# the-byte-bender/GraphAudio

Hardware: AMD Instinct MI355X
Metric: rendered frames/sec @48kHz, 1024-voice convolver graph (higher is better)
Workload: dtype f32

## Files before the change

graphaudio_amd/_capi.py:

```python
from __future__ import annotations

import ctypes as C
import os

_HERE = os.path.dirname(os.path.abspath(__file__))
LIB_NAME = "libgraphaudio_hip.so"


class GraphAudioLibraryError(ImportError):
    """The native HIP library could not be loaded."""


class ArgumentException(ValueError):
    """System.ArgumentException (OfflineAudioContext.cs:32-51)."""


class ArgumentOutOfRangeException(ArgumentException):
    """System.ArgumentOutOfRangeException (AudioBuffer.cs:18, AudioNodeInput.cs:43)."""


class InvalidOperationException(RuntimeError):
    """System.InvalidOperationException (ConvolverNode.cs:45-49, Nodes/AudioNode.cs:157-160)."""


class ObjectDisposedException(InvalidOperationException):
    """System.ObjectDisposedException (AudioContextBase.cs:54)."""


class NotSupportedException(RuntimeError):
    """The graph uses a feature outside the accelerated path (GA_ERR_UNSUPPORTED)."""


class DeviceException(RuntimeError):
    """HIP runtime / device failure (GA_ERR_DEVICE, GA_ERR_OUT_OF_MEMORY, GA_ERR_NO_DEVICE)."""


_CODE_TO_EXC = {
    -1: ArgumentException,
    -2: ArgumentOutOfRangeException,
    -3: InvalidOperationException,
    -4: ObjectDisposedException,
    -5: InvalidOperationException,
    -6: NotSupportedException,
    -7: DeviceException,
    -8: DeviceException,
    -9: DeviceException,
}


class Stats(C.Structure):
    _fields_ = [
        ("blocks_rendered", C.c_int64),
        ("chunks", C.c_int64),
        ("segments", C.c_int64),
        ("kernel_launches", C.c_int64),
        ("device_ms_total", C.c_double),
        ("mac_launches", C.c_int64),
        ("mac_ms_total", C.c_double),
        ("mac_flops_total", C.c_double),
        ("mac_bytes_total", C.c_double),
        ("fft_ms_total", C.c_double),
        ("other_ms_total", C.c_double),
        ("device_bytes_in_use", C.c_int64),
        ("n_nodes", C.c_int32),
        ("n_conv_rows", C.c_int32),
        ("stage_ms", C.c_double * 16),
        ("stage_launches", C.c_int64 * 16),
        ("stage_bytes", C.c_double * 16),
        ("profiled_chunks", C.c_int64),
        ("coarse_carried_outputs", C.c_int64),
        ("stage_flops", C.c_double * 16),
        ("stage_kernel", (C.c_char * 64) * 16),
        ("coarse_premixed_signals", C.c_int64),
        ("deferred_handovers", C.c_int64),
        ("biquad_split_cascades", C.c_int64),
        ("ref_order_rows", C.c_int64),
        ("sim_replays", C.c_int64),
        ("twin_rows", C.c_int64),
    ]
    STAGES = ("other", "mix", "rfft_fwd", "mac", "rfft_inv", "coarse_fwd", "coarse_mac", "coarse_inv", "coarse_hist", "coarse_section",
              "coarse_premix")

    def as_dict(self):
        d = {}
        for name, _ in self._fields_:
            v = getattr(self, name)
            if name == "stage_kernel":
                d[name] = [bytes(row.value).decode("ascii", "replace") for row in v]
            else:
                d[name] = list(v) if hasattr(v, "__len__") else v
        return d


NODE_SPATIAL_PANNER = 12
SPATIAL_PARAM_COUNT = 17
SPATIAL_DISTANCE_MODEL = 17
SPATIAL_HRIR_AZIMUTHS = 18
LISTENER_OPTIONS = tuple(f"listener_{v}_{a}" for v in ("origin", "right", "up", "ahead") for a in "xyz")

_vp, _i, _i64, _f, _d = C.c_void_p, C.c_int, C.c_int64, C.c_float, C.c_double
_pp = C.POINTER(C.c_void_p)

SIGNATURES = {
    "strerror": (C.c_char_p, [_i]),
    "version": (C.c_char_p, []),
    "device_count": (_i, []),
    "context_create": (_i, [_i, _i, C.POINTER(_vp)]),
    "context_destroy": (_i, [_vp]),
    "last_error": (C.c_char_p, [_vp]),
    "current_time": (_d, [_vp]),
    "current_block": (_i64, [_vp]),
    "set_option": (_i, [_vp, C.c_char_p, _d]),
    "get_stats": (_i, [_vp, C.POINTER(Stats)]),
    "buffer_create": (_i, [_vp, _pp, _i, _i64, _i, C.POINTER(_i)]),
    "buffer_release": (_i, [_vp, _i]),
    "node_create": (_i, [_vp, _i, C.POINTER(_i)]),
    "node_create_ex": (_i, [_vp, _i, _d, C.POINTER(_i)]),
    "node_dispose": (_i, [_vp, _i]),
    "node_connect": (_i, [_vp, _i, _i, _i, _i]),
    "node_disconnect": (_i, [_vp, _i, _i, _i, _i]),
    "node_connect_param": (_i, [_vp, _i, _i, _i, _i]),
    "node_disconnect_param": (_i, [_vp, _i, _i, _i, _i]),
    "node_has_ended": (_i, [_vp, _i]),
    "poll_ended": (_i, [_vp, C.POINTER(_i), _i]),
    "input_set_channel_count": (_i, [_vp, _i, _i, _i]),
    "input_set_channel_count_mode": (_i, [_vp, _i, _i, _i]),
    "input_set_channel_interpretation": (_i, [_vp, _i, _i, _i]),
    "destination_set_channel_count": (_i, [_vp, _i]),
    "destination_output_channels": (_i, [_vp]),
    "param_set_value": (_i, [_vp, _i, _i, _f]),
    "param_get_value": (_i, [_vp, _i, _i, C.POINTER(_f)]),
    "param_set_value_at_time": (_i, [_vp, _i, _i, _f, _d]),
    "param_linear_ramp_to_value_at_time": (_i, [_vp, _i, _i, _f, _d]),
    "param_exponential_ramp_to_value_at_time": (_i, [_vp, _i, _i, _f, _d]),
    "param_set_target_at_time": (_i, [_vp, _i, _i, _f, _d, _d]),
    "param_cancel_scheduled_values": (_i, [_vp, _i, _i, _d]),
    "source_set_buffer": (_i, [_vp, _i, _i]),
    "source_set_loop": (_i, [_vp, _i, _i, _d, _d]),
    "source_start": (_i, [_vp, _i, _d, _d, _d]),
    "source_stop": (_i, [_vp, _i, _d]),
    "oscillator_set_type": (_i, [_vp, _i, _i]),
    "biquad_set_type": (_i, [_vp, _i, _i]),
    "convolver_set_normalize": (_i, [_vp, _i, _i]),
    "convolver_set_enable_true_stereo": (_i, [_vp, _i, _i]),
    "convolver_set_buffer": (_i, [_vp, _i, _i]),
    "render": (_i, [_vp, _pp, _i, _i64, _i64]),
    "render_device": (_i, [_vp, _pp, _i, _i64, _i64]),
    "process_blocks": (_i, [_vp, _pp, _i, _i64, _i]),
    "process_blocks_interleaved": (_i, [_vp, C.POINTER(C.c_float), _i, _i64, _i]),
    "context_set_stream": (_i, [_vp, _vp]),
    "synchronize": (_i, [_vp]),
    "stream_queue_buffer": (_i, [_vp, _i, _i]),
    "stream_set_state": (_i, [_vp, _i, _i]),
    "stream_dequeue_processed": (_i, [_vp, _i, C.POINTER(_i)]),
    "stream_queued_count": (_i, [_vp, _i]),
    "stream_processed_count": (_i, [_vp, _i]),
    "comm_unique_id": (_i, [_vp]),
    "comm_init": (_i, [_vp, _vp, _i, _i]),
    "comm_destroy": (_i, [_vp]),
    "comm_info": (_i, [_vp, C.POINTER(_i), C.POINTER(_i), C.POINTER(_i)]),
    "shard_range": (_i, [_i64, _i, _i, C.POINTER(_i64), C.POINTER(_i64)]),
# ... 60 lines not shown
```

graphaudio_amd/csrc/ga_api.cpp:

```cpp
#include <algorithm>
#include <cstring>

#include <execinfo.h>
#include <signal.h>
#include <unistd.h>

#include "ga_engine.hpp"

using namespace ga;

static void ga_segv_handler(int sig) {
  void* frames[64];
  int n = backtrace(frames, 64);
  const char msg[] = "\n[graphaudio_hip] fatal signal, native backtrace:\n";
  (void)!write(2, msg, sizeof(msg) - 1);
  backtrace_symbols_fd(frames, n, 2);
  signal(sig, SIG_DFL);
  raise(sig);
}
__attribute__((constructor)) static void ga_install_handler() {
  const char* e = getenv("GA_BACKTRACE");
  if (e && e[0] == '1') signal(SIGSEGV, ga_segv_handler);
}

// ... 258 lines not shown
  stats.device_bytes_in_use = devBytes;
}

extern "C" {

const char* ga_strerror(int code) {
  switch (code) {
    case GA_OK: return "ok";
    case GA_ERR_INVALID_ARGUMENT: return "invalid argument";
    case GA_ERR_OUT_OF_RANGE: return "argument out of range";
    case GA_ERR_INVALID_OPERATION: return "invalid operation";
    case GA_ERR_DISPOSED: return "object disposed";
    case GA_ERR_CYCLE: return "audio graph cycle detected";
    case GA_ERR_UNSUPPORTED: return "unsupported on the device path";
    case GA_ERR_DEVICE: return "HIP device error";
    case GA_ERR_OUT_OF_MEMORY: return "out of memory";
    case GA_ERR_NO_DEVICE: return "no HIP device";
    default: return "unknown error code";
  }
}
const char* ga_version(void) { return "graphaudio-hip 0.1 (gfx950)"; }
int ga_device_count(void) {
  int n = 0;
  if (hipGetDeviceCount(&n) != hipSuccess) return 0;
  return n;
}

int ga_context_create(int sample_rate, int device_ordinal, ga_context** out) {
  if (!out) return GA_ERR_INVALID_ARGUMENT;
  if (sample_rate <= 0) return GA_ERR_OUT_OF_RANGE;
  ga_context* h = nullptr;
  try {
    h = new ga_context(sample_rate);
    h->c.init_device(device_ordinal);
    auto d = std::make_unique<NodeS>();
    d->id = 0;
    d->type = GA_NODE_DESTINATION;
    d->inputs.resize(1);
    d->inputs[0].channelCount = 2;
    h->c.nodes.push_back(std::move(d));
    *out = h;
    return GA_OK;
  } catch (const Err& e) {
    delete h;
    return e.code;
  } catch (...) {
    delete h;
    return GA_ERR_DEVICE;
  }
}
int ga_context_destroy(ga_context* ctx) {
  delete ctx;
  return GA_OK;
}
const char* ga_last_error(ga_context* ctx) { return ctx ? ctx->c.lastError.c_str() : ""; }
double ga_current_time(ga_context* ctx) { return ctx ? ctx->c.currentTime : 0.0; }
int64_t ga_current_block(ga_context* ctx) { return ctx ? ctx->c.currentBlock : 0; }
int ga_set_option(ga_context* ctx, const char* key, double value) {
  return guard(ctx, [&](Context& c) {
    std::string k = key ? key : "";
    if (k == "max_chunk_blocks") c.maxChunkBlocks = std::max<int64_t>(1, std::min<int64_t>(32768, (int64_t)value));
    else if (k == "profile") c.profile = value != 0;
    else if (k == "profile_every") c.profileEvery = (int)std::max<int64_t>(1, value);
    else if (k == "time_fft") c.useTimeFft = value != 0;
    else if (k == "fft64") c.fft64 = value != 0;
    else if (k == "tconv_radix16") c.useRadix16 = value != 0;
    else if (k == "async") {
      if (c.asyncMode && value == 0) c.synchronize();
      c.asyncMode = value != 0;
    }
    else if (k == "coarse") c.useCoarse = value != 0;
    else if (k == "coarse_overlap") c.coarseOverlap = value != 0;
    else if (k == "coarse_carry") c.coarseCarry = value != 0;
    else if (k == "coarse_tail") c.coarseTail = value != 0;
    else if (k == "coarse_tail_private") c.coarseTailPrivate = value != 0;
    else if (k == "sim_replay") c.simReplay = value != 0;
    else if (k == "twin_channels") c.twinChannels = value != 0;
    else if (k == "cycle_delay_split") c.cycleDelaySplit = value != 0;
    else if (k == "resample_fast") c.resampleFast = value != 0;
    else if (k == "rate_mod_walk") c.rateModWalk = value != 0;
    else if (k == "conv_reference_order") c.convRefOrder = (int)std::min(2.0, std::max(0.0, value));
    else if (k == "conv_ref_min_deviation") c.convRefMinDeviation = std::max(0.0, value);
    else if (k == "coarse_premix") c.coarsePremix = value != 0;
    else if (k == "coarse_long") c.coarseLong = value != 0;
    else if (k == "coarse_ext_history") c.coarseExtHist = value != 0;
    else if (k == "coarse_wide") c.coarseWide = value != 0;
    else if (k == "gain_pass_through") c.gainPassThrough = value != 0;
    else if (k == "gain_fold") c.gainFold = value != 0;
    else if (k == "coarse_mfma") c.coarseMfma = value != 0;
    else if (k == "biquad_time_split") c.biquadTimeSplit = (int)std::min(2.0, std::max(0.0, value));
    else if (k == "biquad_split_max_deviation") c.biquadSplitMaxDeviation = std::max(0.0, value);
    else if (k == "biquad_split_min_frames") c.biquadSplitMinFrames = std::max<int64_t>(2048, (int64_t)value);
    else if (k == "host_direct") c.hostDirect = value != 0;
    else if (k == "host_defer") c.hostDefer = value != 0;
    else if (k == "table_upload_kernel") c.tableUploadKernel = value != 0;
    else if (k == "comm_timeout_s") c.commTimeoutS = std::max(1.0, value);
    else if (k == "host_copy_stream") c.hostCopyStream = value != 0;
    else if (k == "coarse_min_blocks") c.coarseMinBlocks = std::max<int64_t>(1, (int64_t)value);
    else if (k == "debug_tconv_n2") c.debugTconvN2 = (int)value;
    else if (k == "mem_budget_fraction") c.memBudgetFraction = std::min(0.95, std::max(0.05, value));
    else if (k.rfind("listener_", 0) == 0) {
      static const char* const vec[4] = {"origin", "right", "up", "ahead"};
      int slot = -1;
      for (int v = 0; v < 4 && slot < 0; v++)
        for (int a = 0; a < 3 && slot < 0; a++)
          if (k == std::string("listener_") + vec[v] + "_" + "xyz"[a]) slot = v * 3 + a;
      if (slot < 0) fail(GA_ERR_INVALID_ARGUMENT, "unknown option " + k);
      c.listener[slot] = (float)value;
    }
    else fail(GA_ERR_INVALID_ARGUMENT, "unknown option " + k);
  });
}
int ga_get_stats(ga_context* ctx, ga_stats* out) {
  return guardRO(ctx, [&](Context& c) {
    if (!out) fail(GA_ERR_INVALID_ARGUMENT, "null pointer");
    c.harvestProfile(true);
    c.stats.device_bytes_in_use = c.devBytes;
    c.stats.n_nodes = (int)c.nodes.size();
    int rows = 0;
    for (auto& g : c.groups) rows += (int)g->rows.size();
    c.stats.n_conv_rows = rows;
    *out = c.stats;
  });
}
int ga_synchronize(ga_context* ctx) {
  return guardRO(ctx, [&](Context& c) { c.synchronize(); });
}
int ga_context_set_stream(ga_context* ctx, void* hip_stream) {
  return guard(ctx, [&](Context& c) {
    c.flushHandOver();
    GA_HIP(hipStreamSynchronize(c.stream));
    c.waitHostCopies();
    if (c.ownStream && c.stream) (void)hipStreamDestroy(c.stream);
    c.stream = (hipStream_t)hip_stream;
    c.ownStream = false;
  });
}

int ga_buffer_create(ga_context* ctx, const float* const* planar, int channels, int64_t frames, int sample_rate, int* out_id) {
  return guard(ctx, [&](Context& c) {
    if (!planar || !out_id) fail(GA_ERR_INVALID_ARGUMENT, "null pointer");
    if (channels < 1 || channels > 4096) fail(GA_ERR_OUT_OF_RANGE, "Channel count must be between 1 and 4096 (1 .. 32 for audio, more for an HRIR set)");
    if (frames < 0) fail(GA_ERR_OUT_OF_RANGE, "Length must be non-negative");
    if (sample_rate <= 0) fail(GA_ERR_OUT_OF_RANGE, "Sample rate must be positive");
    auto b = std::make_unique<PlayBuf>();
    b->channels = channels;
    b->length = frames;
    b->sampleRate = sample_rate;
    b->stride = (frames + 8 + 63) / 64 * 64;
    b->host.resize(channels);
    GA_HIP(hipSetDevice(c.device));
    size_t bytes = (size_t)b->stride * channels * sizeof(float);
    b->dev = c.dallocSkewed(bytes, &b->devBase, &b->devBytes);
    GA_HIP(hipMemsetAsync(b->dev, 0, bytes, c.stream));
    for (int i = 0; i < channels; i++) {
      if (!planar[i]) fail(GA_ERR_INVALID_ARGUMENT, "null channel pointer");
      b->host[i].assign(planar[i], planar[i] + frames);
      if (frames)
        GA_HIP(hipMemcpyAsync(b->dev + (size_t)i * b->stride, planar[i], sizeof(float) * frames, hipMemcpyHostToDevice, c.stream));
    }
    GA_HIP(hipStreamSynchronize(c.stream));
    c.buffers.push_back(std::move(b));
    c.bufVersion++;
    *out_id = (int)c.buffers.size() - 1;
  });
}
// ... 572 lines not shown
```

graphaudio_amd/csrc/ga_chunk.cpp:

```cpp
#include "ga_chunk_internal.hpp"

namespace ga {

float* getSlab(Context& c) {
  if (c.slabFree.empty()) {
    size_t slabBytes = (size_t)c.slabFrames * sizeof(float);
    size_t count = std::max<size_t>(8, std::min<size_t>(1024, ((size_t)1 << 30) / slabBytes));
    char* blk = (char*)c.dalloc(slabBytes * count);
    c.slabBlocks.push_back(blk);
    for (size_t i = 0; i < count; i++) {
      float* p = (float*)(blk + i * slabBytes);
      c.slabAll.push_back(p);
      c.slabFree.push_back(p);
    }
  }
  float* p = c.slabFree.back();
  c.slabFree.pop_back();
  return p;
}

void resetSlabs(Context& c, int64_t frames) {
  int64_t need = roundup(frames, 256);
  if (need > c.slabFrames) {
    GA_HIP(hipStreamSynchronize(c.stream));
// ... 573 lines not shown
    }
    nd.delayW.assign(rings, 0);
    nd.delayR.assign(rings, 0);
  }

  if (r.stage != 2) resetSlabs(*this, frames);
  if (zerosLen < frames) {
    if (zeros) {
      GA_HIP(hipStreamSynchronize(stream));
      dfree(zeros, (size_t)zerosLen * 4);
    }
    zerosLen = roundup(frames, 4096);
    zeros = (float*)dalloc((size_t)zerosLen * 4);
    GA_HIP(hipMemsetAsync(zeros, 0, (size_t)zerosLen * 4, stream));
  }
  if (busCapFrames < frames) {
    GA_HIP(hipStreamSynchronize(stream));
    for (float* p : busSlabs) dfree(p, (size_t)busCapFrames * 4);
    busSlabs.clear();
    busCapFrames = roundup(frames, 4096);
  }
  while ((int)busSlabs.size() < 32 && (int)busSlabs.size() < std::max(destOutCh, 2)) busSlabs.push_back((float*)dalloc((size_t)busCapFrames * 4));
  {
    int mx = 0;
    for (auto& sg : segs)
      if (r.stage != 1) mx = std::max(mx, sg.nodes.back().outCh);
    while ((int)busSlabs.size() < mx) busSlabs.push_back((float*)dalloc((size_t)busCapFrames * 4));
  }

}

void Context::chunkExecute(ChunkRun& r) {
  Context& c_ = *this; (void)c_;
  int& maxDepth = r.maxDepth; int& maxLevel = r.maxLevel; (void)maxDepth; (void)maxLevel;
  int64_t& n = r.n; (void)n;
  std::vector<double>& bt = r.bt; (void)bt;
  std::vector<int>& srcIds = r.srcIds; (void)srcIds;
  std::vector<SrcPlanOut>& srcPlans = r.srcPlans; (void)srcPlans;
  std::vector<Segment>& segs = r.segs; (void)segs;
  const int64_t frames = r.n * kBlock; (void)frames;
  int& bHistMax = r.bHistMax; (void)bHistMax;
  Exec& ex = *r.ex;
  r.tmPlan = nowMs();
  if (!pendingHandOver.empty()) {
    std::vector<HandOver> hv;
    hv.swap(pendingHandOver);
    hipStream_t st = stream;
    ex.plan.launches.insert(ex.plan.launches.begin(), Plan::L{[hv, st](uint8_t*) {
      for (const HandOver& h : hv) GA_HIP(hipMemcpyAsync(h.dst_host, h.src, sizeof(float) * (size_t)h.n, hipMemcpyDeviceToHost, st));
    }, LK_OTHER, 0.0, 0.0});
  }
  ex.trajOffFinal = ex.plan.putv(ex.traj);
  ex.spatialJobsOff = ex.plan.putv(ex.spatialJobs);
  size_t tbytes = ex.plan.host.size();
  const int slot = asyncMode ? (int)(chunkSeq & 1) : 0;
  void*& thost = slot ? tablesHostB : tablesHost;
  size_t& thostBytes = slot ? tablesHostBBytes : tablesHostBytes;
  if (asyncMode && chunkDone[slot]) GA_HIP(hipEventSynchronize(chunkDone[slot]));
  if (thostBytes < tbytes) {
    if (thost) {
      GA_HIP(hipStreamSynchronize(stream));
      (void)hipHostFree(thost);
    }
    thostBytes = (tbytes + tbytes / 4 + 4096 + 15) & ~(size_t)15;
    GA_HIP(hipHostMalloc(&thost, thostBytes, hipHostMallocDefault));
  }
  ensure(tables, std::max(tablesHostBytes, tablesHostBBytes));
  std::memcpy(thost, ex.plan.host.data(), tbytes);
  if (tableUploadKernel) launch_table_upload(stream, tables.p, thost, tbytes);
  else GA_HIP(hipMemcpyAsync(tables.p, thost, tbytes, hipMemcpyHostToDevice, stream));
  uint8_t* base = (uint8_t*)tables.p;

  std::vector<std::pair<hipEvent_t, hipEvent_t>> evs;
  std::vector<int> evKind;
  std::vector<double> evBytes;
  hipEvent_t evBegin = nullptr, evEnd = nullptr;
  const bool profile = profileNow;
  if (profile) {
    GA_HIP(hipEventCreate(&evBegin));
    GA_HIP(hipEventCreate(&evEnd));
    GA_HIP(hipEventRecord(evBegin, stream));
  }
  for (auto& l : ex.plan.launches) {
    hipEvent_t e0 = nullptr, e1 = nullptr;
    if (profile) {
      GA_HIP(hipEventCreate(&e0));
      GA_HIP(hipEventCreate(&e1));
      GA_HIP(hipEventRecord(e0, stream));
    }
    l.fn(base);
    if (profile) {
      GA_HIP(hipEventRecord(e1, stream));
      evs.push_back({e0, e1});
      evKind.push_back(l.kind);
      evBytes.push_back(l.bytes);
    }
    if (l.kind == GA_STAGE_COARSE_SECTION) continue;
    stats.kernel_launches++;
    if (l.kind >= 0 && l.kind < 16) {
      stats.stage_launches[l.kind]++;
      stats.stage_bytes[l.kind] += l.bytes;
      stats.stage_flops[l.kind] += l.flops;
    }
  }
  for (auto& x : extraProf) {
    evs.push_back({x.e0, x.e1});
    evKind.push_back(x.kind);
    evBytes.push_back(x.bytes);
  }
  extraProf.clear();
  if (profile) GA_HIP(hipEventRecord(evEnd, stream));
  GA_HIP(hipGetLastError());
  r.tmLaunch = nowMs();
  if (profileNow) pendingProf.push_back(ProfBatch{evBegin, evEnd, std::move(evs), std::move(evKind), std::move(evBytes)});
  if (asyncMode) {
    if (!chunkDone[slot]) GA_HIP(hipEventCreateWithFlags(&chunkDone[slot], hipEventDisableTiming));
    GA_HIP(hipEventRecord(chunkDone[slot], stream));
    harvestProfile(false);
  } else {
    GA_HIP(hipStreamSynchronize(stream));
    harvestProfile(true);
  }
  chunkSeq++;
  if (gaTiming)
    fprintf(stderr, "[ga]   host detail: topo %.2f, sources %.2f, sim %.2f | resources %.2f, params %.2f, exec %.2f ms\n", r.tmTopo - r.tm0,
            r.tmSrc - r.tmTopo, r.tmSim - r.tmSrc, r.tmRes - r.tmSim, r.tmPre - r.tmRes, r.tmPlan - r.tmPre);
  if (gaTiming)
    fprintf(stderr, "[ga] chunk %lld blocks: sim %.2f ms, plan %.2f ms, enqueue %.2f ms, wait %.2f ms\n", (long long)n, r.tmSim - r.tm0,
            r.tmPlan - r.tmSim, r.tmLaunch - r.tmPlan, nowMs() - r.tmLaunch);

}

void Context::chunkCommit(ChunkRun& r) {
  Context& c_ = *this; (void)c_;
  int& maxDepth = r.maxDepth; int& maxLevel = r.maxLevel; (void)maxDepth; (void)maxLevel;
  int64_t& n = r.n; (void)n;
  std::vector<double>& bt = r.bt; (void)bt;
  std::vector<int>& srcIds = r.srcIds; (void)srcIds;
  std::vector<SrcPlanOut>& srcPlans = r.srcPlans; (void)srcPlans;
  std::vector<Segment>& segs = r.segs; (void)segs;
  const int64_t frames = r.n * kBlock; (void)frames;
  int& bHistMax = r.bHistMax; (void)bHistMax;
  for (size_t i = 0; i < srcIds.size(); i++) {
    NodeS& s = *nodes[srcIds[i]];
    SrcPlanOut& po = srcPlans[i];
    if (s.type != GA_NODE_BUFFER_SOURCE) {
      if (po.gone && po.goneAt <= n) {
        if (!s.endedRaised) endedQueue.push_back(srcIds[i]);
        s.endedRaised = true;
        if (po.goneAt == n) pending.push_back([this, id = srcIds[i]]() { doDispose(id); });
      }
      continue;
    }
    if (s.spans.empty()) continue;
    int64_t firstPlay = -1;
    for (const SrcSpan& sp : s.spans)
      if ((sp.phase == SRC_PLAY || sp.phase == SRC_END) && firstPlay < 0) firstPlay = sp.b0;
    if (firstPlay < 0 || firstPlay >= n) continue;
    int64_t lastProcessed = n;
    if (po.gone && po.goneAt <= n) lastProcessed = po.goneAt;
    int64_t played = lastProcessed - firstPlay;
    PlayBuf* pb = s.bufId >= 0 ? buffers[s.bufId].get() : nullptr;
    bool rate1 = true;
    if (pb) rate1 = sourceGeom(*this, s, *pb).effectiveRate == 1.0;
    if (s.gsr && s.gsrWalked >= 0) {
      if (played == s.gsrWalked) {
        s.playbackPosition = s.gsrTail.pp;
        for (int k = 0; k < 4; k++) s.gsrW[k] = s.gsrTail.w[k];
        s.gsrPos = s.gsrTail.pos;
        s.gsrReady = s.gsrTail.ready;
      } else if (!(po.gone && po.goneAt <= n)) {
        fail(GA_ERR_DEVICE, "internal: a walked source ends its chunk at another block than its walk");
      }
    } else if (s.gsr) {
// ... 305 lines not shown
```

graphaudio_amd/csrc/ga_chunk_internal.hpp:

```cpp
#pragma once
#include <time.h>

#include <algorithm>
#include <array>
#include <cstdio>
#include <cstdlib>
#include <cstring>
#include <unordered_map>

#include "ga_engine.hpp"

namespace ga {

static inline uint64_t hmix(uint64_t h, uint64_t v) {
  h ^= v + 0x9e3779b97f4a7c15ull + (h << 6) + (h >> 2);
  return h;
}

static inline int64_t roundup(int64_t v, int64_t m) { return (v + m - 1) / m * m; }

struct Plan {
  std::vector<uint8_t> host;
  struct L {
    std::function<void(uint8_t*)> fn;
    int kind;
    double bytes;
    double flops;
  };
  std::vector<L> launches;
  size_t put(const void* p, size_t bytes) {
    size_t off = (host.size() + 15) & ~(size_t)15;
    host.resize(off + bytes);
    if (bytes) std::memcpy(&host[off], p, bytes);
    return off;
  }
  template <class T>
  size_t putv(const std::vector<T>& v) {
    return put(v.data(), v.size() * sizeof(T));
  }
  void add(int kind, std::function<void(uint8_t*)> fn, double bytes = 0.0, double flops = 0.0) {
    launches.push_back(L{std::move(fn), kind, bytes, flops});
  }
};

float* getSlab(Context& c);
void resetSlabs(Context& c, int64_t frames);

extern const bool gaTiming;
double nowMs();

struct SrcGeom {
  int64_t loopStartFrame, loopEndFrame, durationEndFrame;
  double effectiveRate;
};

SrcGeom sourceGeom(Context& c, NodeS& s, PlayBuf& b);
Resampler& resamplerFor(Context& c, double rate);

struct SrcPlanOut {
  int64_t playedBlocks = 0;
  bool reachedEnd = false;
  int64_t endBlock = -1;
  bool gone = false;
  int64_t goneAt = -1;
  int64_t partialBlock = -1;
  int partialProduced = 0;
};

struct RateModIn {
  const float* rates = nullptr;
  const GsrWalkOut* walk = nullptr;
  const GsrBlock* desc = nullptr;
  int64_t nrel = 0;
};

SrcPlanOut planSource(Context& c, NodeS& s, int64_t n, const std::vector<double>& bt, const RateModIn* rm = nullptr);
bool rateModWalkJob(Context& c, NodeS& s, int64_t n, const std::vector<double>& bt, GsrWalkJob& j);
SrcPlanOut planScheduled(Context& c, NodeS& s, int64_t n, const std::vector<double>& bt);

static const SrcSpan& spanAt(const NodeS& s, int64_t b) {
  size_t i = s.spans.size() - 1;
  while (i > 0 && s.spans[i].b0 > b) i--;
  return s.spans[i];
}

struct ChunkRun;

struct Sim {
  Context& c;
  int64_t n;
  int64_t blockNumber = 0;
  Segment* cur = nullptr;
  int64_t brel = 0;
  std::vector<int64_t>* extraBreaks = nullptr;
  const std::vector<double>* blockTimes = nullptr;
  const ChunkRun* pre = nullptr;

  bool restorePre(int id);

  void evalProbe(const std::vector<std::pair<int, int>>& mods, const std::vector<int>& roots) {
    for (int id : roots)
      if (!c.nodes[id]->disposed) evalNode(id);
    for (const auto& pm : mods) {
      InSeg is;
      is.bufCh = 1;
      is.silent = true;
      for (auto& m : c.nodes[pm.first]->params[pm.second].modulation) {
        evalNode(m.first);
        const NodeS& pn = *c.nodes[m.first];
        const OutputS& o = pn.outputs[m.second];
        if (o.bufCh != 0 && !o.silent) {
          is.terms.push_back(TermS{m.first, m.second, o.bufCh, pn.isProcessing});
          is.silent = false;
        }
      }
      cur->probe.push_back(std::move(is));
    }
  }

  int computeOutputChannelCount(InputS& in) {
    switch (in.mode) {
      case GA_COUNT_MODE_EXPLICIT: return in.channelCount;
      case GA_COUNT_MODE_CLAMPED_MAX: {
        int mx = 0;
// ... 961 lines not shown
```

graphaudio_amd/csrc/ga_coarse.hip:

```cpp
#include "ga_kernels.hpp"
#include "ga_fft16.hpp"

#include <hip/hip_runtime.h>

#include <algorithm>
#include <atomic>
#include <string>
#include <type_traits>
#include <utility>
#include <cstdio>
#include <cstdlib>

namespace ga {

struct LdsLimit {
  std::atomic<uint64_t> done{0};
  void raise(const void* kern, size_t need, const char* what) {
    int dev = 0;
    (void)hipGetDevice(&dev);
    const uint64_t bit = 1ull << (dev & 63);
    if (done.load(std::memory_order_relaxed) & bit) return;
    if (hipFuncSetAttribute(kern, hipFuncAttributeMaxDynamicSharedMemorySize, 160 * 1024) == hipSuccess) {
      done.fetch_or(bit);
      return;
    }
    (void)hipGetLastError();
    if (hipFuncSetAttribute(kern, hipFuncAttributeMaxDynamicSharedMemorySize, (int)std::max<size_t>(need, 65536)) != hipSuccess) launch_fail(what);
  }
};

constexpr int CM = 4096;
constexpr int CPAD = TC16_PADDED(CM);
__device__ __forceinline__ int cpad(int j) { return j + (j >> 5); }
__device__ __forceinline__ int cslot(int s) { return (s >> 12) * CPAD + cpad(s & (CM - 1)); }

__device__ __forceinline__ f2 cj(f2 a) { return f2{a.x, -a.y}; }
__device__ __forceinline__ f2 mul_mi(f2 a) { return f2{a.y, -a.x}; }
__device__ __forceinline__ f2 mul_pi(f2 a) { return f2{-a.y, a.x}; }
__device__ __forceinline__ f2 cmulc(f2 a, f2 b) { return cmulp(a, b); }

__device__ __forceinline__ f2 cfmap(f2 a, f2 b, f2 acc) {
#if defined(GA_EXPERIMENTS) && defined(GA_MAC_SCALAR_FMA)
  float re, im, re2, im2;
  asm("v_fma_f32 %0, %1, %2, %3" : "=v"(re) : "v"(a.x), "v"(b.x), "v"(acc.x));
  asm("v_fma_f32 %0, %1, %2, %3" : "=v"(im) : "v"(a.x), "v"(b.y), "v"(acc.y));
  asm("v_fma_f32 %0, -%1, %2, %3" : "=v"(re2) : "v"(a.y), "v"(b.y), "v"(re));
  asm("v_fma_f32 %0, %1, %2, %3" : "=v"(im2) : "v"(a.y), "v"(b.x), "v"(im));
  return f2{re2, im2};
#endif
  f2 t, r;
  asm("v_pk_fma_f32 %0, %1, %2, %3 op_sel_hi:[0,1,1]" : "=v"(t) : "v"(a), "v"(b), "v"(acc));
  asm("v_pk_fma_f32 %0, %1, %2, %3 op_sel:[1,1,0] op_sel_hi:[1,0,1] neg_lo:[0,1,0]" : "=v"(r) : "v"(a), "v"(b), "v"(t));
  return r;
}

template <int OFF>
__device__ __forceinline__ f2 lds_rd_b64(unsigned addr) {
  f2 r;
  asm volatile("ds_read_b64 %0, %1 offset:%2" : "=v"(r) : "v"(addr), "n"(OFF) : "memory");
  return r;
}
template <int STRIDE, int... Q>
__device__ __forceinline__ void lds_rd_seq(f2* dst, unsigned addr, std::integer_sequence<int, Q...>) {
  ((dst[Q] = lds_rd_b64<Q * STRIDE>(addr)), ...);
}
template <int N>
__device__ __forceinline__ void lds_pin(f2* v) {
#pragma unroll
  for (int i = 0; i < N; i++) asm volatile("" : "+v"(v[i]));
}
__device__ __forceinline__ void lds_wait_all() { asm volatile("s_waitcnt lgkmcnt(0)" ::: "memory"); }
__device__ __forceinline__ unsigned lds_addr(const f2* p) {
  return (unsigned)(uintptr_t)(const __attribute__((address_space(3))) f2*)p;
}

__device__ __forceinline__ void coarse_issue_half(const CoarseXRow& R, int hw, int t, v4f (&raw)[8]) {
  const float* src = nullptr;
  int64_t lim = 0;
  if (hw < 0) {
    const int64_t off = (int64_t)R.hist_len + (int64_t)hw * kCoarseBlock;
    if (R.hist && off >= 0) {
      src = R.hist + off;
      lim = kCoarseBlock;
    }
  } else if (R.in) {
    const int64_t off = (int64_t)hw * kCoarseBlock;
    src = R.in + off;
    lim = std::min<int64_t>(kCoarseBlock, R.nvalid - off);
  }
  const bool aligned = ((uintptr_t)src & 15) == 0;
#pragma unroll
  for (int q = 0; q < 8; q++) {
    const int o = 4 * (t + 256 * q);
    raw[q] = v4f{0.f, 0.f, 0.f, 0.f};
    if (src && o < lim) {
      if (aligned) raw[q] = ldg4(src + o);
      else raw[q] = v4f{ldg1(src + o), ldg1(src + o + 1), ldg1(src + o + 2), ldg1(src + o + 3)};
    }
  }
}

constexpr int kHandOverWgs = 8;
constexpr int kFwdPark = 4;
constexpr int kFwdTw3 = 4 * 256;
template <bool EXPERIMENT>
__global__ __launch_bounds__(256, 3) void coarse_fwd_kernel(const CoarseXRow* __restrict rows, int run, float2* __restrict X,
                                                            const float2* __restrict twg, const float2* __restrict twab, int exp_,
                                                            const CoarseHandOver* __restrict handover, int n_handover) {
  if ((int)blockIdx.y < n_handover) {
    const int nwg = min((int)gridDim.x, kHandOverWgs);
    if ((int)blockIdx.x >= nwg) return;
    const CoarseHandOver H = handover[blockIdx.y];
    const GA_GLOBAL v4f* src = (const GA_GLOBAL v4f*)H.src;
    GA_GLOBAL v4f* dst = (GA_GLOBAL v4f*)H.dst;
    const int64_t nw = H.n / 4, step = (int64_t)nwg * 512;
    for (int64_t i = (int64_t)blockIdx.x * 512 + threadIdx.x; i < nw; i += step) {
      const int64_t i2 = i + 256;
      const v4f a = src[i], b = i2 < nw ? src[i2] : a;
      dst[i] = a;
      if (i2 < nw) dst[i2] = b;
    }
    return;
  }
  const int exp = EXPERIMENT ? exp_ : 0;
  using PL = R16Plan<CM>;
  extern __shared__ f2 clds[];
  f2* tw2 = clds;
  f2* tw3 = clds + PL::T2;
  f2* buf = clds + PL::T2 + kFwdTw3;
  f2* park = buf + CPAD;
  const int t_ = threadIdx.x;
  for (int i = t_; i < PL::T2 + kFwdTw3; i += 256) clds[i] = f2{twg[i].x, twg[i].y};
  const CoarseXRow R = rows[blockIdx.y - n_handover];
  const int w0 = blockIdx.x * run;
  const int w1 = min(R.n_frames, w0 + run);
  if (w0 >= w1) return;
  const bool zero2 = (R.flags & 1) != 0;
  const float scale = R.scale;
  const int wave64 = __builtin_amdgcn_readfirstlane(t_ & ~63);
  v4f first[8], second[8];
  coarse_issue_half(R, R.u0 + w0 - 1, t_, first);
  if (zero2) {
#pragma unroll
    for (int q = 0; q < 8; q++) second[q] = v4f{0.f, 0.f, 0.f, 0.f};
  } else {
    coarse_issue_half(R, R.u0 + w0, t_, second);
  }
  __syncthreads();
  for (int w = w0; w < w1; w++) {
    int t = wave64 + (int)__builtin_amdgcn_mbcnt_hi(~0u, __builtin_amdgcn_mbcnt_lo(~0u, 0u));
    asm volatile("" : "+v"(t));
    const int u = R.u0 + w;
    const bool more = w + 1 < w1;
    f2 own[16];
    if (R.carry && u >= 0 && (int64_t)(u + 1) * kCoarseBlock > R.carry_from) {
#pragma unroll
      for (int q = 0; q < 8; q++) {
        const int64_t sidx = (int64_t)u * kCoarseBlock + 4 * (t + 256 * q);
        if (sidx >= R.carry_from && sidx < R.nvalid) stg4(R.carry + (sidx - R.carry_from), second[q]);
      }
    }
#pragma unroll
    for (int m = 0; m < 8; m++) {
      own[m] = f2{first[m].x * scale, first[m].y * scale};
      own[8 + m] = f2{second[m].x * scale, second[m].y * scale};
    }
    int go = 1;
    asm volatile("" : "+s"(go));
    if (go && !(exp & 4)) fft16_own<CM, true>(own, buf, tw2, tw3, t);
    f2 za[8], pa[8];
    const f2 za8 = own[8];
    __syncthreads();
    const int xw = cpad(t), xr = cpad(2048 - t) - 264 * 7;
#pragma unroll
    for (int m = 0; m < 8; m++) {
      za[m] = own[m];
      buf[xw + 264 * m] = own[8 + m];
    }
    __syncthreads();
#pragma unroll
    for (int m = 0; m < 8; m++) {
      const int k = t + 256 * m;
      pa[m] = k == 0 ? za[0] : buf[xr + 264 * (7 - m)];
      if (m >= 8 - kFwdPark) park[t + 256 * (m - (8 - kFwdPark))] = pa[m];
    }
    __syncthreads();
#pragma unroll
    for (int m = 0; m < 8; m++) {
      own[m] = f2{first[m].z * scale, first[m].w * scale};
      own[8 + m] = f2{second[m].z * scale, second[m].w * scale};
    }
    asm volatile("" : "+s"(go));
    if (go && !(exp & 4)) fft16_own<CM, true>(own, buf, tw2, tw3, t);
    f2 pb[8];
    const f2 zb8 = own[8];
    __syncthreads();
#pragma unroll
    for (int m = 0; m < 8; m++) buf[xw + 264 * m] = own[8 + m];
    __syncthreads();
#pragma unroll
    for (int m = 0; m < 8; m++) {
      const int k = t + 256 * m;
      pb[m] = k == 0 ? own[0] : buf[xr + 264 * (7 - m)];
    }
    const float2 tb0g = twab[2049 + t];
    const f2 tb0 = f2{tb0g.x, tb0g.y};
    if (more) {
      if (zero2) {
        if (!(exp & 8)) coarse_issue_half(R, u, t, first);
      } else {
#pragma unroll
        for (int q = 0; q < 8; q++) first[q] = second[q];
        if (!(exp & 8)) coarse_issue_half(R, u + 1, t, second);
      }
    }
    float2* __restrict F = X + (size_t)(R.frame0 + w) * kCoarseBins;
    auto quad = [&](int k, f2 Ak, f2 Am, f2 Bk, f2 Bm, f2 b) {
      const f2 a = cmulc(b, b);
      const f2 aB = cmulc(a, Bk), caBm = cmulc(cj(a), Bm);
      const f2 Wk = Ak + aB, Wp = Ak - aB;
      const f2 Wm = Am - caBm, Wn = Am + caBm;
      const f2 fe = Wk + cj(Wn), bfo = cmulc(b, mul_mi(Wk - cj(Wn)));
      const f2 Xk = fe + bfo, Xn = cj(fe - bfo);
      const f2 fe2 = Wm + cj(Wp), wfo2 = cmulc(mul_mi(cj(b)), mul_mi(Wm - cj(Wp)));
      const f2 Xm = fe2 + wfo2, Xp = cj(fe2 - wfo2);
      if (exp & 1) {
        if (Xk.x == 12345.f && Xn.x == 54321.f && Xm.x == 999.f && Xp.y == 777.f) F[0] = make_float2(0.f, 0.f);
      } else if (k == 0) {
        stg4(F, v4f{Xk.x, Xn.x, Xm.x, Xm.y});
      } else if (k == CM / 2) {
        stg4(F + 2 * k, v4f{Xk.x, Xk.y, Xn.x, Xn.y});
      } else {
        stg4(F + 2 * k, v4f{Xk.x, Xk.y, Xp.x, Xp.y});
        stg4(F + 2 * (CM - k), v4f{Xm.x, Xm.y, Xn.x, Xn.y});
      }
    };
    if (!(exp & 2)) {
      constexpr float w64[8][2] = {{1.f, 0.f},
                                   {0.99518472667219688624f, -0.09801714032956060199f},
                                   {0.98078528040323044913f, -0.19509032201612826785f},
                                   {0.95694033573220886494f, -0.29028467725446236764f},
                                   {0.92387953251128675613f, -0.38268343236508977173f},
                                   {0.88192126434835502971f, -0.47139673682599764856f},
                                   {0.83146961230254523708f, -0.55557023301960222474f},
                                   {0.77301045336273696081f, -0.63439328416364549822f}};
#pragma unroll
      for (int m = 0; m < 8; m++) {
        const f2 b = m == 0 ? tb0 : cmulc(tb0, f2{w64[m][0], w64[m][1]});
        quad(t + 256 * m, za[m], m >= 8 - kFwdPark ? park[t + 256 * (m - (8 - kFwdPark))] : pa[m], own[m], pb[m], b);
        __builtin_amdgcn_sched_barrier(0);
      }
      if (t == 0) quad(CM / 2, za8, za8, zb8, zb8, f2{twab[2049 + CM / 2].x, twab[2049 + CM / 2].y});
    }
    __syncthreads();
  }
}

const char* launch_coarse_fwd(hipStream_t s, const CoarseXRow* rows_dev, int nrows, int max_frames, int run, float2* X, const float2* tw16,
                              const float2* twab, const CoarseHandOver* handover_dev, int n_handover) {
  if (nrows <= 0 || max_frames <= 0) return "";
  using PL = R16Plan<CM>;
  const size_t lds = (size_t)(PL::T2 + kFwdTw3 + CPAD + kFwdPark * 256) * sizeof(float2);
  static const int exp = (expenv("GA_COARSE_EXP") ? atoi(expenv("GA_COARSE_EXP")) : 0) & 15;
  auto kern = exp ? coarse_fwd_kernel<true> : coarse_fwd_kernel<false>;
  static LdsLimit lim[2];
  lim[exp ? 1 : 0].raise((const void*)kern, lds, "cannot raise the dynamic LDS limit of the coarse forward transform");
  run = std::max(run, 1);
  for (int r0 = 0; r0 < nrows; r0 += 32768) {
    const int nh = r0 == 0 ? n_handover : 0;
    dim3 grid((max_frames + run - 1) / run, std::min(32768, nrows - r0) + nh);
    hipLaunchKernelGGL(kern, grid, dim3(256), lds, s, rows_dev + r0, run, X, tw16, twab, exp, handover_dev, nh);
  }
  return "coarse_fwd_kernel";
}

#ifndef GA_MAC_WAVES
#define GA_MAC_WAVES 8
#endif
#ifndef GA_MAC_TW
#define GA_MAC_TW 9
#endif
#ifndef GA_MAC_PB2
#define GA_MAC_PB2 4
#endif
constexpr int kMacWaves16 = 12;
constexpr int kMacTW16 = (kCoarseJobBlocks(16) + kMacWaves16 - 1) / kMacWaves16;
constexpr int kMacWaves = GA_MAC_WAVES;
constexpr int kMacWavesPerSimd(int cw) { return kMacWaves * (cw >= 4 ? 2 : 1) / 4; }
template <int CW, int TW, int PB, int WV>
__global__ __launch_bounds__(64 * WV, WV == 8 ? kMacWavesPerSimd(CW) : WV / 4) void coarse_mac_kernel(const CoarseJob* __restrict jobs, const CoarseTerm* __restrict terms,
                                                                    const float2* __restrict X, float2* __restrict Y, int y_frames, int NFA,
                                                                    int exp) {
  extern __shared__ f2 mlds[];
  const CoarseJob J = jobs[blockIdx.y];
  const int tile = blockIdx.x;
  const int tid = threadIdx.x, lane = tid & 63, wv = __builtin_amdgcn_readfirstlane(tid >> 6);
  const int P = J.P, nT = J.n_t;
  const int NF = nT + P - 1;
  const int fr_lo = max(0, J.u_lo - (J.t0 - (P - 1))), fr_hi = min(NF - 1, J.u_hi - (J.t0 - (P - 1)));
  f2* xs0 = mlds;
  f2* xs1 = mlds + (size_t)NFA * 64;
  f2* hs0 = mlds + (size_t)2 * NFA * 64;
  f2* hs1 = hs0 + (size_t)P * CW * 64;
  const int twr = (nT + WV - 1) / WV;
  const int t0w = wv * twr;
  const bool special = tile == 0;
  const bool lane0 = special && lane == 0;
  const size_t binoff = (size_t)tile * 64;

  typedef __attribute__((address_space(3))) void* lds_t;
  constexpr int XR = ((WV * TW + kCoarseMaxP) * 32 + (64 * WV) - 1) / (64 * WV);
  auto issue_x = [&](const CoarseTerm& T, f2* xs) {
#pragma unroll
    for (int r = 0; r < XR; r++) {
      const int fr0 = ((64 * WV) / 32) * r + 2 * wv;
      const int fr = fr0 + (lane >> 5), of = lane & 31;
      if (fr >= fr_lo && fr <= fr_hi)
        __builtin_amdgcn_global_load_lds(gptr(X + (size_t)(T.frame0 + J.t0 + fr) * kCoarseBins + binoff + 2 * of), (lds_t)(xs + fr0 * 64), 16, 0, 0);
    }
  };
  auto issue_h = [&](const CoarseTerm& T, f2* hs) {
    for (int pc0 = 2 * wv; pc0 < P * CW; pc0 += 2 * WV) {
      const int pc = pc0 + (lane >> 5), of = lane & 31;
      const int pA = pc0 / CW, cA = pc0 % CW, pB = (pc0 + 1) / CW, cB = (pc0 + 1) % CW;
      const float2* rowA = T.h[cA] + (size_t)pA * kCoarseBins;
      const float2* rowB = pc0 + 1 < P * CW ? T.h[cB] + (size_t)pB * kCoarseBins : rowA;
      if (pc < P * CW)
        __builtin_amdgcn_global_load_lds(gptr(((lane >> 5) ? rowB : rowA) + binoff + 2 * of), (lds_t)(hs + pc0 * 64), 16, 0, 0);
    }
  };

  f2 acc[TW][CW];
#pragma unroll
  for (int tt = 0; tt < TW; tt++)
#pragma unroll
    for (int c = 0; c < CW; c++) acc[tt][c] = f2{0.f, 0.f};

  const CoarseTerm* __restrict T = terms + J.term0;
  for (int idx = tid; idx < NF * 32; idx += (64 * WV)) {
    const int fr = idx >> 5;
    if (fr < fr_lo || fr > fr_hi) {
      *reinterpret_cast<v4f*>(xs0 + fr * 64 + 2 * (idx & 31)) = v4f{0.f, 0.f, 0.f, 0.f};
      *reinterpret_cast<v4f*>(xs1 + fr * 64 + 2 * (idx & 31)) = v4f{0.f, 0.f, 0.f, 0.f};
    }
  }
  issue_x(T[0], xs0);
  issue_h(T[0], hs0);
  __syncthreads();
  for (int i = 0; i < J.n_terms; i++) {
    const bool more = i + 1 < J.n_terms;
    f2* xs = (i & 1) ? xs1 : xs0;
    f2* hs = (J.shared_h || !(i & 1)) ? hs0 : hs1;
    if (more && !(exp & 2)) {
      if (!J.shared_h) issue_h(T[i + 1], (i & 1) ? hs0 : hs1);
// ... 150 lines not shown
      case 1: stream(std::integral_constant<int, 1>{}); break;
      case 2: stream(std::integral_constant<int, 2>{}); break;
      case 3: stream(std::integral_constant<int, XR >= 3 ? 3 : XR>{}); break;
      case 4: stream(std::integral_constant<int, XR >= 4 ? 4 : XR>{}); break;
      case 5: stream(std::integral_constant<int, XR >= 5 ? 5 : XR>{}); break;
      case 6: stream(std::integral_constant<int, XR >= 6 ? 6 : XR>{}); break;
      default: break;
    }
  }
  for (int idx = tid; idx < NF * 32; idx += kSumThreads) {
    const int fr = idx >> 5;
    if (fr < fr_lo || fr > fr_hi) *reinterpret_cast<v4f*>(S + fr * 64 + 2 * (idx & 31)) = v4f{0.f, 0.f, 0.f, 0.f};
  }
#pragma unroll
  for (int r = 0; r < XR; r++) {
    const int idx = tid + kSumThreads * r;
    const int fv = idx >> 5, of = idx & 31;
    if (fv < nvf) *reinterpret_cast<v4f*>(S + (fr_lo + fv) * 64 + 2 * of) = acc[r];
  }
  __syncthreads();
  f2 y[TW][CW], yS[TW][CW];
#pragma unroll
  for (int tt = 0; tt < TW; tt++)
#pragma unroll
    for (int c = 0; c < CW; c++) y[tt][c] = yS[tt][c] = f2{0.f, 0.f};
  if (t0w < nT && !(exp & 1)) {
    auto sweep = [&](auto sp) {
      constexpr bool SP = decltype(sp)::value;
      const f2* __restrict xb = S + (t0w + (P - 1)) * 64 + lane;
      f2 xv[TW];
#pragma unroll
      for (int q = 1; q < TW; q++) xv[q] = xb[q * 64];
      for (int p = 0; p < P; p++) {
#pragma unroll
        for (int q = TW - 1; q > 0; q--) xv[q] = p == 0 ? xv[q] : xv[q - 1];
        xv[0] = xb[-p * 64];
        f2 h[CW];
#pragma unroll
        for (int c = 0; c < CW; c++) h[c] = hs[(p * CW + c) * 64 + lane];
#pragma unroll
        for (int tt = 0; tt < TW; tt++)
#pragma unroll
          for (int c = 0; c < CW; c++) {
            y[tt][c] = cfmap(xv[tt], h[c], y[tt][c]);
            if constexpr (SP) yS[tt][c] = __builtin_elementwise_fma(xv[tt], h[c], yS[tt][c]);
          }
      }
    };
    if (special) sweep(std::true_type{});
    else sweep(std::false_type{});
  }
#pragma unroll
  for (int tt = 0; tt < TW; tt++) {
    const int t = t0w + tt;
    if (tt < twr && t < nT && !(exp & 4)) {
#pragma unroll
      for (int c = 0; c < CW; c++) {
        const f2 a = lane0 ? yS[tt][c] : y[tt][c];
        stg2(Y + ((size_t)(J.yrow0 + c) * y_frames + J.t0 + t) * kCoarseBins + binoff + lane, v2f{a.x, a.y});
      }
    }
  }
}

template <int CW>
static const char* launch_coarse_sum(hipStream_t s, const CoarseJob* jobs_dev, int njobs, const CoarseTerm* terms_dev, const float2* X, float2* Y,
                              int y_frames, int max_t, int maxP) {
  static const int exp = expenv("GA_COARSE_EXP") ? atoi(expenv("GA_COARSE_EXP")) : 0;
  constexpr int TW = kCoarseSumJobBlocks(CW) / kSumWaves;
  int NFA = 0;
  for (int nt = 1; nt <= max_t; nt++) {
    const int twr = (nt + kSumWaves - 1) / kSumWaves, wl = (nt + twr - 1) / twr - 1;
    NFA = std::max(NFA, wl * twr + TW + maxP - 1);
  }
  const size_t lds = ((size_t)NFA * 64 + (size_t)maxP * CW * 64) * sizeof(float2);
  if (lds > 160 * 1024) launch_fail("coarse multiply-accumulate: staging does not fit the LDS");
  static LdsLimit lim;
  lim.raise((const void*)coarse_sum_kernel<CW>, lds, "cannot raise the dynamic LDS limit of the coarse multiply-accumulate");
  if (expenv("GA_COARSE_EXP")) {
    int occ = -1;
    (void)hipOccupancyMaxActiveBlocksPerMultiprocessor(&occ, coarse_sum_kernel<CW>, kSumThreads, lds);
    fprintf(stderr, "[coarse_sum<%d>] lds %zu B, NFA %d, occupancy %d workgroups/CU, %d jobs\n", CW, lds, NFA, occ, njobs);
  }
  for (int j0 = 0; j0 < njobs; j0 += 32768)
    hipLaunchKernelGGL((coarse_sum_kernel<CW>), dim3(kCoarseBins / 64, std::min(32768, njobs - j0)), dim3(kSumThreads), lds, s, jobs_dev + j0, terms_dev, X,
                       Y, y_frames, NFA, exp >> 4);
  return CW == 1 ? "coarse_sum_kernel<1>" : (CW == 2 ? "coarse_sum_kernel<2>" : "coarse_sum_kernel<4>");
}

template <int CW, int TW, int PB, int WV>
__global__ __launch_bounds__(64 * WV, WV / 4) void coarse_mac_seg_kernel(const CoarseJob* __restrict jobs, const CoarseTerm* __restrict terms,
                                                                                      const float2* __restrict X, float2* __restrict Y, int y_frames, int NFA) {
  static_assert(CW <= 4, "segments: 1, 2 or 4 columns (16-column pieces are made for P' <= 4 only)");
  extern __shared__ f2 mlds[];
  const CoarseJob J = jobs[blockIdx.y];
  const int tile = blockIdx.x;
  const int tid = threadIdx.x, lane = tid & 63, wv = __builtin_amdgcn_readfirstlane(tid >> 6);
  constexpr int P = kCoarseMaxP;
  const int nT = J.n_t;
  const int NF = nT + P - 1;
  f2* xs0 = mlds;
  f2* xs1 = mlds + (size_t)NFA * 64;
  f2* hs0 = mlds + (size_t)2 * NFA * 64;
  f2* hs1 = hs0 + (size_t)P * CW * 64;
  const int twr = (nT + WV - 1) / WV;
  const int t0w = wv * twr;
  const bool special = tile == 0;
  const bool lane0 = special && lane == 0;
  const size_t binoff = (size_t)tile * 64;
  typedef __attribute__((address_space(3))) void* lds_t;
  constexpr int XR = ((WV * TW + kCoarseMaxP) * 32 + (64 * WV) - 1) / (64 * WV);
  auto zero_x = [&](const CoarseTerm& T, f2* xs) {
    const int w0 = J.t0 - (T.pad_ & 255) - (P - 1);
    const int fr_lo = max(0, J.u_lo - w0), fr_hi = min(NF - 1, J.u_hi - w0);
    for (int idx = tid; idx < NF * 32; idx += (64 * WV)) {
      const int fr = idx >> 5;
      if (fr < fr_lo || fr > fr_hi) *reinterpret_cast<v4f*>(xs + fr * 64 + 2 * (idx & 31)) = v4f{0.f, 0.f, 0.f, 0.f};
    }
  };
  auto issue_x = [&](const CoarseTerm& T, f2* xs) {
    const int w0 = J.t0 - (T.pad_ & 255) - (P - 1);
    const int fr_lo = max(0, J.u_lo - w0), fr_hi = min(NF - 1, J.u_hi - w0);
#pragma unroll
    for (int r = 0; r < XR; r++) {
      const int fr0 = ((64 * WV) / 32) * r + 2 * wv;
      const int fr = fr0 + (lane >> 5), of = lane & 31;
      if (fr >= fr_lo && fr <= fr_hi)
        __builtin_amdgcn_global_load_lds(gptr(X + (size_t)(T.frame0 + J.t0 + fr) * kCoarseBins + binoff + 2 * of), (lds_t)(xs + fr0 * 64), 16, 0, 0);
    }
  };
  auto issue_h = [&](const CoarseTerm& T, f2* hs) {
    const int np = T.pad_ >> 8;
    for (int pc0 = 2 * wv; pc0 < np * CW; pc0 += 2 * WV) {
      const int pc = pc0 + (lane >> 5), of = lane & 31;
      const int pA = pc0 / CW, cA = pc0 % CW, pB = (pc0 + 1) / CW, cB = (pc0 + 1) % CW;
      const float2* rowA = T.h[cA] + (size_t)pA * kCoarseBins;
      const float2* rowB = pc0 + 1 < np * CW ? T.h[cB] + (size_t)pB * kCoarseBins : rowA;
      if (pc < np * CW)
        __builtin_amdgcn_global_load_lds(gptr(((lane >> 5) ? rowB : rowA) + binoff + 2 * of), (lds_t)(hs + pc0 * 64), 16, 0, 0);
    }
  };

  f2 acc[TW][CW];
#pragma unroll
  for (int tt = 0; tt < TW; tt++)
#pragma unroll
    for (int c = 0; c < CW; c++) acc[tt][c] = f2{0.f, 0.f};

  const CoarseTerm* __restrict T = terms + J.term0;
  zero_x(T[0], xs0);
  issue_x(T[0], xs0);
  issue_h(T[0], hs0);
  __syncthreads();
  for (int i = 0; i < J.n_terms; i++) {
    f2* xs = (i & 1) ? xs1 : xs0;
    f2* hs = (i & 1) ? hs1 : hs0;
    if (i + 1 < J.n_terms) {
      zero_x(T[i + 1], (i & 1) ? xs0 : xs1);
      issue_h(T[i + 1], (i & 1) ? hs0 : hs1);
      issue_x(T[i + 1], (i & 1) ? xs0 : xs1);
    }
    if (t0w < nT) {
      const int off = T[i].pad_ & 255, np = T[i].pad_ >> 8;
      auto sweep = [&](auto sp) {
        constexpr bool SP = decltype(sp)::value;
        constexpr int PBX = PB, NX = TW + PBX - 1, NH = PBX * CW;
        auto fma1 = [&](int tt, int c, f2 x, f2 h) {
          if constexpr (!SP) {
            acc[tt][c] = cfmap(x, h, acc[tt][c]);
// ... 114 lines not shown
        }
#pragma unroll
        for (int u = 0; u < AH; u++)
#pragma unroll
          for (int r = 0; r < NW; r++) acc[r] += ld[u][r];
      }
      for (; i < nterms; i++) {
        const float2* __restrict Xt = X + (int64_t)__builtin_amdgcn_readlane(f0v, i) * kCoarseBins;
#pragma unroll
        for (int r = 0; r < NW; r++) acc[r] += ldg4(Xt + woff[r]);
      }
    };
    static_assert(XR <= 6, "one case per word count below");
    switch (nw) {
      case 1: stream(std::integral_constant<int, 1>{}); break;
      case 2: stream(std::integral_constant<int, 2>{}); break;
      case 3: stream(std::integral_constant<int, XR >= 3 ? 3 : XR>{}); break;
      case 4: stream(std::integral_constant<int, XR >= 4 ? 4 : XR>{}); break;
      case 5: stream(std::integral_constant<int, XR >= 5 ? 5 : XR>{}); break;
      case 6: stream(std::integral_constant<int, XR >= 6 ? 6 : XR>{}); break;
      default: break;
    }
    for (int idx = tid; idx < NF * 32; idx += kSumThreads) {
      const int fr = idx >> 5;
      if (fr < fr_lo || fr > fr_hi) *reinterpret_cast<v4f*>(S + fr * 64 + 2 * (idx & 31)) = v4f{0.f, 0.f, 0.f, 0.f};
    }
#pragma unroll
    for (int r = 0; r < XR; r++) {
      const int idx = tid + kSumThreads * r;
      const int fv = idx >> 5, of = idx & 31;
      if (fv < nvf) *reinterpret_cast<v4f*>(S + (fr_lo + fv) * 64 + 2 * of) = acc[r];
    }
    __syncthreads();
    if (t0w < nT) {
      const f2* __restrict xb = S + (t0w + (PS - 1)) * 64 + lane;
      f2 xv[TW];
#pragma unroll
      for (int q = 1; q < TW; q++) xv[q] = xb[q * 64];
      for (int p = 0; p < np; p++) {
#pragma unroll
        for (int q = TW - 1; q > 0; q--) xv[q] = p == 0 ? xv[q] : xv[q - 1];
        xv[0] = xb[-p * 64];
        f2 h[CW];
#pragma unroll
        for (int c = 0; c < CW; c++) h[c] = hs[(p * CW + c) * 64 + lane];
#pragma unroll
        for (int tt = 0; tt < TW; tt++)
#pragma unroll
          for (int c = 0; c < CW; c++) {
            const f2 gen = cfmap(xv[tt], h[c], y[tt][c]);
            const f2 pk = __builtin_elementwise_fma(xv[tt], h[c], y[tt][c]);
            y[tt][c] = lane0 ? pk : gen;
          }
      }
    }
  }
#pragma unroll
  for (int tt = 0; tt < TW; tt++) {
    const int t = t0w + tt;
    if (tt < twr && t < nT) {
#pragma unroll
      for (int c = 0; c < CW; c++)
        stg2(Y + ((size_t)(J.yrow0 + c) * y_frames + J.t0 + t) * kCoarseBins + binoff + lane, v2f{y[tt][c].x, y[tt][c].y});
    }
  }
}

static int coarse_seg_frames(int max_t, int waves, int tw) {
  int NFA = 0;
  for (int nt = 1; nt <= max_t; nt++) {
    const int twr = (nt + waves - 1) / waves, wl = (nt + twr - 1) / twr - 1;
    NFA = std::max(NFA, wl * twr + tw + kCoarseMaxP - 1);
  }
  return NFA;
}
template <int CW>
static const char* launch_coarse_sum_seg(hipStream_t s, const CoarseJob* jobs_dev, int njobs, const CoarseTerm* terms_dev, const float2* X, float2* Y,
                                         int y_frames, int max_t) {
  const int NFA = coarse_seg_frames(max_t, kSumWaves, kCoarseSumJobBlocks(CW) / kSumWaves);
  const size_t lds = ((size_t)NFA * 64 + (size_t)kCoarseMaxP * CW * 64) * sizeof(float2);
  if (lds > 160 * 1024) launch_fail("coarse multiply-accumulate: staging does not fit the LDS");
  static LdsLimit lim;
  lim.raise((const void*)coarse_sum_seg_kernel<CW>, lds, "cannot raise the dynamic LDS limit of the coarse multiply-accumulate");
  for (int j0 = 0; j0 < njobs; j0 += 32768)
    hipLaunchKernelGGL((coarse_sum_seg_kernel<CW>), dim3(kCoarseBins / 64, std::min(32768, njobs - j0)), dim3(kSumThreads), lds, s, jobs_dev + j0, terms_dev,
                       X, Y, y_frames, NFA);
  return CW == 1 ? "coarse_sum_seg_kernel<1>" : (CW == 2 ? "coarse_sum_seg_kernel<2>" : "coarse_sum_seg_kernel<4>");
}
template <int CW, int TW>
static const char* launch_coarse_mac_seg(hipStream_t s, const CoarseJob* jobs_dev, int njobs, const CoarseTerm* terms_dev, const float2* X, float2* Y,
                                         int y_frames, int max_t) {
  constexpr int PB = 4;
  const int NFA = coarse_seg_frames(max_t, kMacWaves, TW);
  const size_t lds = ((size_t)2 * NFA * 64 + (size_t)2 * kCoarseMaxP * CW * 64) * sizeof(float2);
  if (lds > 160 * 1024) launch_fail("coarse multiply-accumulate: staging does not fit the LDS");
  static LdsLimit lim;
  lim.raise((const void*)coarse_mac_seg_kernel<CW, TW, PB, kMacWaves>, lds, "cannot raise the dynamic LDS limit of the coarse multiply-accumulate");
  for (int j0 = 0; j0 < njobs; j0 += 32768)
    hipLaunchKernelGGL((coarse_mac_seg_kernel<CW, TW, PB, kMacWaves>), dim3(kCoarseBins / 64, std::min(32768, njobs - j0)), dim3(64 * kMacWaves), lds, s,
                       jobs_dev + j0, terms_dev, X, Y, y_frames, NFA);
  static const std::string name = "coarse_mac_seg_kernel<" + std::to_string(CW) + "," + std::to_string(TW) + "," + std::to_string(PB) + ">";
  return name.c_str();
}
template <int CW>
static const char* launch_coarse_seg_cw(hipStream_t s, const CoarseJob* jobs_dev, int njobs, const CoarseTerm* terms_dev, const float2* X, float2* Y,
                                        int y_frames, int max_t, bool any_private) {
  if (!any_private) return launch_coarse_sum_seg<CW>(s, jobs_dev, njobs, terms_dev, X, Y, y_frames, max_t);
  if (max_t <= 2 * kMacWaves) return launch_coarse_mac_seg<CW, 2>(s, jobs_dev, njobs, terms_dev, X, Y, y_frames, max_t);
  if constexpr (CW <= 2) {
    if (max_t <= 8 * kMacWaves) return launch_coarse_mac_seg<CW, 8>(s, jobs_dev, njobs, terms_dev, X, Y, y_frames, max_t);
    return launch_coarse_mac_seg<CW, GA_MAC_TW>(s, jobs_dev, njobs, terms_dev, X, Y, y_frames, max_t);
  } else {
    return launch_coarse_mac_seg<CW, GA_MAC_TW4>(s, jobs_dev, njobs, terms_dev, X, Y, y_frames, max_t);
  }
}

__global__ __launch_bounds__(256) void coarse_mac_bin0_kernel(const CoarseJob* __restrict jobs, const CoarseTerm* __restrict terms,
                                                             const float2* __restrict X, float2* __restrict Y, int y_frames) {
  const CoarseJob J = jobs[blockIdx.x];
  const CoarseTerm* __restrict T = terms + J.term0;
  const int P = J.P;
  const int idx = blockIdx.y * 256 + threadIdx.x;
  if (idx >= J.n_t * 16) return;
  const int t = idx >> 4, c = idx & 15;
  const int p_lo = max(0, J.t0 + t - J.u_hi), p_hi = min(P - 1, J.t0 + t - J.u_lo);
  f2 acc = f2{0.f, 0.f};
  for (int i = 0; i < J.n_terms; i++) {
    const float2* __restrict h = T[i].h[c];
    const float2* __restrict x = X + (size_t)(T[i].frame0 + J.t0 + t + (P - 1)) * kCoarseBins;
    int p = p_lo;
    for (; p + 3 <= p_hi; p += 4) {
      v2f xv[4], hv[4];
#pragma unroll
      for (int q = 0; q < 4; q++) {
        xv[q] = ldg2(x - (size_t)(p + q) * kCoarseBins);
        hv[q] = ldg2(h + (size_t)(p + q) * kCoarseBins);
      }
#pragma unroll
      for (int q = 0; q < 4; q++) acc = __builtin_elementwise_fma(f2{xv[q].x, xv[q].y}, f2{hv[q].x, hv[q].y}, acc);
    }
    for (; p <= p_hi; p++) {
      const v2f xv = ldg2(x - (size_t)p * kCoarseBins), hv = ldg2(h + (size_t)p * kCoarseBins);
      acc = __builtin_elementwise_fma(f2{xv.x, xv.y}, f2{hv.x, hv.y}, acc);
    }
  }
  stg2(Y + ((size_t)(J.yrow0 + c) * y_frames + J.t0 + t) * kCoarseBins, v2f{acc.x, acc.y});
}

typedef float f4v __attribute__((ext_vector_type(4)));
constexpr int kMfThreads = 512, kMfFrames = kCoarseJobBlocks(16) + 3, kMfRows = kMfFrames + 64, kMfPitch = 65;
constexpr size_t kMfLdsBytes = std::max<size_t>((size_t)2 * kMfRows * 64, (size_t)256 * kMfPitch) * sizeof(float2);
__device__ __forceinline__ int mf_slot(int row, int bin) { return row * 64 + ((((bin >> 1) ^ row) & 31) << 1) + (bin & 1); }
__global__ __launch_bounds__(kMfThreads, 2) void coarse_mfma16_kernel(const CoarseJob* __restrict jobs, const CoarseTerm* __restrict terms,
                                                                     const float2* __restrict X, float2* __restrict Y, int y_frames) {
  extern __shared__ f2 mlds[];
  typedef __attribute__((address_space(3))) void* lds_t;
  const CoarseJob J = jobs[blockIdx.y];
  const int tid = threadIdx.x, lane = tid & 63, wv = __builtin_amdgcn_readfirstlane(tid >> 6);
  const int P = J.P, nT = J.n_t;
  const size_t binoff = (size_t)blockIdx.x * 64;
  const CoarseTerm* __restrict T = terms + J.term0;
  auto live = [&](int row) {
    if (row < kMfFrames) {
      const int u = J.t0 + row - 3;
      return row < nT + 3 && u >= J.u_lo && u <= J.u_hi;
    }
    return row < kMfRows && ((row - kMfFrames) >> 4) < P;
  };
  f2* st0 = mlds;
  f2* st1 = mlds + (size_t)kMfRows * 64;
  for (int idx = tid; idx < kMfRows * 32; idx += kMfThreads) {
    const int row = idx >> 5;
    if (!live(row)) {
      *reinterpret_cast<v4f*>(st0 + row * 64 + 2 * (idx & 31)) = v4f{0.f, 0.f, 0.f, 0.f};
      *reinterpret_cast<v4f*>(st1 + row * 64 + 2 * (idx & 31)) = v4f{0.f, 0.f, 0.f, 0.f};
    }
  }
  auto issue = [&](int i, f2* stage) {
    const int frame0 = T[i].frame0;
    const float2* __restrict h0 = T[i].h[0];
#pragma unroll
    for (int k = 0; k < (kMfRows + 15) / 16; k++) {
      const int r0 = 16 * k + 2 * wv, row = r0 + (lane >> 5);
      const int sw = ((lane & 31) ^ row) & 31;
      const float2* src = row < kMfFrames ? X + (size_t)(frame0 + J.t0 + row - 3 + (P - 1)) * kCoarseBins
                                          : h0 + ((size_t)((row - kMfFrames) & 15) * P + ((row - kMfFrames) >> 4)) * kCoarseBins;
      if (live(row)) __builtin_amdgcn_global_load_lds(gptr(src + binoff + 2 * sw), (lds_t)(stage + r0 * 64), 16, 0, 0);
    }
  };
  f4v accr[8][2], acci[8][2];
#pragma unroll
  for (int b = 0; b < 8; b++)
#pragma unroll
    for (int q = 0; q < 2; q++) accr[b][q] = acci[b][q] = f4v{0.f, 0.f, 0.f, 0.f};
  issue(0, st0);
  __syncthreads();
  const int arow = kMfFrames + lane;
  const int brow = (lane & 15) - (lane >> 4) + 3;
  for (int i = 0; i < J.n_terms; i++) {
    const f2* __restrict st = (i & 1) ? st1 : st0;
    if (i + 1 < J.n_terms) issue(i + 1, (i & 1) ? st0 : st1);
#pragma unroll
    for (int b = 0; b < 8; b++) {
      const int bin = 8 * wv + b;
      const f2 a = st[mf_slot(arow, bin)];
      const f2 x0 = st[mf_slot(brow, bin)], x1 = st[mf_slot(brow + 16, bin)];
      const float nai = -a.y;
      accr[b][0] = __builtin_amdgcn_mfma_f32_16x16x4f32(a.x, x0.x, accr[b][0], 0, 0, 0);
      acci[b][0] = __builtin_amdgcn_mfma_f32_16x16x4f32(a.x, x0.y, acci[b][0], 0, 0, 0);
      accr[b][1] = __builtin_amdgcn_mfma_f32_16x16x4f32(a.x, x1.x, accr[b][1], 0, 0, 0);
      acci[b][1] = __builtin_amdgcn_mfma_f32_16x16x4f32(a.x, x1.y, acci[b][1], 0, 0, 0);
      accr[b][0] = __builtin_amdgcn_mfma_f32_16x16x4f32(nai, x0.y, accr[b][0], 0, 0, 0);
      acci[b][0] = __builtin_amdgcn_mfma_f32_16x16x4f32(a.y, x0.x, acci[b][0], 0, 0, 0);
      accr[b][1] = __builtin_amdgcn_mfma_f32_16x16x4f32(nai, x1.y, accr[b][1], 0, 0, 0);
      acci[b][1] = __builtin_amdgcn_mfma_f32_16x16x4f32(a.y, x1.x, acci[b][1], 0, 0, 0);
    }
    __syncthreads();
  }
#pragma unroll
  for (int q = 0; q < 2; q++) {
#pragma unroll
    for (int b = 0; b < 8; b++)
#pragma unroll
      for (int r = 0; r < 4; r++) mlds[((4 * (lane >> 4) + r) * 16 + (lane & 15)) * kMfPitch + 8 * wv + b] = f2{accr[b][q][r], acci[b][q][r]};
    __syncthreads();
    for (int idx = tid; idx < 256 * 32; idx += kMfThreads) {
      const int row = idx >> 5, of = idx & 31, c = row >> 4, t = 16 * q + (row & 15);
      if (t < nT) {
        const f2 v0 = mlds[row * kMfPitch + 2 * of], v1 = mlds[row * kMfPitch + 2 * of + 1];
        stg4(Y + ((size_t)(J.yrow0 + c) * y_frames + J.t0 + t) * kCoarseBins + binoff + 2 * of, v4f{v0.x, v0.y, v1.x, v1.y});
      }
    }
    __syncthreads();
  }
}

template <int CW, int TW, int PB, int WV = kMacWaves>
static const char* launch_coarse_mac_t(hipStream_t s, const CoarseJob* jobs_dev, int njobs, const CoarseTerm* terms_dev, const float2* X, float2* Y,
                                int y_frames, int max_t, int maxP, bool any_private) {
  static const int exp = expenv("GA_COARSE_EXP") ? atoi(expenv("GA_COARSE_EXP")) : 0;
  int NFA = 0;
  for (int nt = 1; nt <= max_t; nt++) {
    const int twr = (nt + WV - 1) / WV, wl = (nt + twr - 1) / twr - 1;
    NFA = std::max(NFA, wl * twr + TW + maxP - 1);
  }
  const size_t lds = ((size_t)2 * NFA * 64 + (size_t)(any_private ? 2 : 1) * maxP * CW * 64) * sizeof(float2);
  if (lds > 160 * 1024) launch_fail("coarse multiply-accumulate: staging does not fit the LDS");
  static LdsLimit lim;
  lim.raise((const void*)coarse_mac_kernel<CW, TW, PB, WV>, lds, "cannot raise the dynamic LDS limit of the coarse multiply-accumulate");
  if (expenv("GA_COARSE_EXP")) {
    int occ = -1;
    (void)hipOccupancyMaxActiveBlocksPerMultiprocessor(&occ, coarse_mac_kernel<CW, TW, PB, WV>, 64 * WV, lds);
    fprintf(stderr, "[coarse_mac<%d,%d,%d>] lds %zu B, NFA %d, occupancy %d workgroups/CU, %d jobs\n", CW, TW, PB, lds, NFA, occ, njobs);
  }
  for (int j0 = 0; j0 < njobs; j0 += 32768)
    hipLaunchKernelGGL((coarse_mac_kernel<CW, TW, PB, WV>), dim3(kCoarseBins / 64, std::min(32768, njobs - j0)), dim3(64 * WV), lds, s,
                       jobs_dev + j0, terms_dev, X, Y, y_frames, NFA, exp >> 4);
  static const std::string name = "coarse_mac_kernel<" + std::to_string(CW) + "," + std::to_string(TW) + "," + std::to_string(PB) + "," + std::to_string(WV) + ">";
  return name.c_str();
}
template <int CW, int TWL>
static const char* launch_coarse_mac_tw(hipStream_t s, const CoarseJob* jobs_dev, int njobs, const CoarseTerm* terms_dev, const float2* X, float2* Y,
                                 int y_frames, int max_t, int maxP, bool any_private, int pb) {
  if (pb >= 4 && (CW == 1 || (CW == 2 && GA_MAC_PB2 == 4))) return launch_coarse_mac_t<CW, TWL, 4>(s, jobs_dev, njobs, terms_dev, X, Y, y_frames, max_t, maxP, any_private);
  if (pb >= 2) return launch_coarse_mac_t<CW, TWL, 2>(s, jobs_dev, njobs, terms_dev, X, Y, y_frames, max_t, maxP, any_private);
  return launch_coarse_mac_t<CW, TWL, 1>(s, jobs_dev, njobs, terms_dev, X, Y, y_frames, max_t, maxP, any_private);
}
template <int CW>
static const char* launch_coarse_mac_cw(hipStream_t s, const CoarseJob* jobs_dev, int njobs, const CoarseTerm* terms_dev, const float2* X, float2* Y,
                                 int y_frames, int max_t, int maxP, bool any_private, int pb) {
  if (!any_private) return launch_coarse_sum<CW>(s, jobs_dev, njobs, terms_dev, X, Y, y_frames, max_t, maxP);
  if (max_t <= 2 * kMacWaves) return launch_coarse_mac_t<CW, 2, 1>(s, jobs_dev, njobs, terms_dev, X, Y, y_frames, max_t, maxP, any_private);
  if constexpr (CW <= 2) {
    if (max_t <= 8 * kMacWaves) return launch_coarse_mac_tw<CW, 8>(s, jobs_dev, njobs, terms_dev, X, Y, y_frames, max_t, maxP, any_private, pb);
    return launch_coarse_mac_tw<CW, GA_MAC_TW>(s, jobs_dev, njobs, terms_dev, X, Y, y_frames, max_t, maxP, any_private, pb);
  } else {
    return launch_coarse_mac_tw<CW, GA_MAC_TW4>(s, jobs_dev, njobs, terms_dev, X, Y, y_frames, max_t, maxP, any_private, pb);
  }
}
const char* launch_coarse_mac(hipStream_t s, const CoarseJob* jobs_dev, int njobs, const CoarseTerm* terms_dev, const float2* X, float2* Y,
                       int y_frames, int cw, int max_t, int maxP, bool any_private, int pb, bool matrix_cores) {
  if (njobs <= 0) return "";
  if (max_t > (any_private ? kCoarseJobBlocks(cw) : kCoarseSumJobBlocks(cw))) launch_fail("coarse multiply-accumulate: too many coarse blocks in a job");
  if (const char* e = expenv("GA_COARSE_PB")) pb = std::min(pb, std::max(1, atoi(e)));
  if (pb != 1 && pb != 2 && pb != 4 && pb != 8 && pb != 16) launch_fail("coarse multiply-accumulate: unsupported partition block");
  if (maxP > kCoarseMaxP) {
    if (maxP > kCoarseMaxParts) launch_fail("coarse multiply-accumulate: too many partitions");
    if (cw == 1) return launch_coarse_seg_cw<1>(s, jobs_dev, njobs, terms_dev, X, Y, y_frames, max_t, any_private);
    if (cw == 2) return launch_coarse_seg_cw<2>(s, jobs_dev, njobs, terms_dev, X, Y, y_frames, max_t, any_private);
    if (cw == 4) return launch_coarse_seg_cw<4>(s, jobs_dev, njobs, terms_dev, X, Y, y_frames, max_t, any_private);
    launch_fail("coarse multiply-accumulate: unsupported column count");
  }
  if (cw == 1) return launch_coarse_mac_cw<1>(s, jobs_dev, njobs, terms_dev, X, Y, y_frames, max_t, maxP, any_private, pb);
  if (cw == 2) return launch_coarse_mac_cw<2>(s, jobs_dev, njobs, terms_dev, X, Y, y_frames, max_t, maxP, any_private, pb);
  if (cw == 4) return launch_coarse_mac_cw<4>(s, jobs_dev, njobs, terms_dev, X, Y, y_frames, max_t, maxP, any_private, pb);
  if (cw == 16 && any_private) {
    const char* name;
    if (matrix_cores && maxP <= 4 && max_t <= kCoarseJobBlocks(16)) {
      static LdsLimit lim;
      lim.raise((const void*)coarse_mfma16_kernel, kMfLdsBytes, "cannot raise the dynamic LDS limit of the matrix-core multiply-accumulate");
      for (int j0 = 0; j0 < njobs; j0 += 32768)
        hipLaunchKernelGGL(coarse_mfma16_kernel, dim3(kCoarseBins / 64, std::min(32768, njobs - j0)), dim3(kMfThreads), kMfLdsBytes, s, jobs_dev + j0,
                           terms_dev, X, Y, y_frames);
      name = "coarse_mfma16_kernel";
    } else {
      name = launch_coarse_mac_t<16, kMacTW16, 1, kMacWaves16>(s, jobs_dev, njobs, terms_dev, X, Y, y_frames, max_t, maxP, true);
    }
    hipLaunchKernelGGL(coarse_mac_bin0_kernel, dim3(njobs, (kCoarseJobBlocks(16) * 16 + 255) / 256), dim3(256), 0, s, jobs_dev, terms_dev, X, Y, y_frames);
    return name;
  }
  launch_fail("coarse multiply-accumulate: unsupported column count");
}

__global__ __launch_bounds__(512) void coarse_inv_kernel(const CoarseOut* __restrict outs, const int* __restrict ylist,
                                                         const float2* __restrict Y, int y_frames, const float2* __restrict twg,
                                                         const float2* __restrict twab) {
  using PL = R16Plan<CM>;
  extern __shared__ f2 clds[];
  f2* tw2 = clds;
  f2* tw3 = clds + PL::T2;
  f2* zb0 = clds + PL::T2 + PL::T3;
  const int tid = threadIdx.x;
  const int g = __builtin_amdgcn_readfirstlane(tid >> 8), t = tid & 255;
  f2* buf = zb0 + g * CPAD;
  const CoarseOut O = outs[blockIdx.y];
  const int tb = blockIdx.x;
  const int64_t s0 = (int64_t)tb * kCoarseBlock;
  const int64_t send = O.nvalid + (O.tail_out ? O.tail_len : 0);
  if (s0 >= send || !O.out) return;
  float* st = reinterpret_cast<float*>(zb0);
  const bool have_y = tb < O.n_y;
  auto route = [&](bool zero) {
    __syncthreads();
    for (int i = tid; i < kCoarseBlock / 4; i += 512) {
      const int64_t si = s0 + 4 * i;
      if (si >= send) continue;
      v4f v = zero ? v4f{0.f, 0.f, 0.f, 0.f} : *reinterpret_cast<const v4f*>(st + 4 * i);
      if (O.tail_in && si < O.tail_len) v += ldg4(O.tail_in + si);
      float* __restrict dst = si < O.nvalid ? O.out + si : O.tail_out + (si - O.nvalid);
      if ((((uintptr_t)dst) & 15) == 0) stg4(dst, v);
      else { stg1(dst, v.x); stg1(dst + 1, v.y); stg1(dst + 2, v.z); stg1(dst + 3, v.w); }
    }
  };
  if (!have_y) {
    route(true);
    return;
  }
  for (int i = tid; i < PL::T2 + PL::T3; i += 512) clds[i] = f2{twg[i].x, twg[i].y};
  {
    float4 sum[8];
#pragma unroll
    for (int r = 0; r < 8; r++) sum[r] = make_float4(0.f, 0.f, 0.f, 0.f);
    for (int j = 0; j < O.ny; j++) {
      const float4* __restrict src = reinterpret_cast<const float4*>(Y + ((size_t)ylist[O.y0 + j] * y_frames + tb) * kCoarseBins);
      float4 v[8];
#pragma unroll
      for (int r = 0; r < 8; r++) v[r] = src[tid + 512 * r];
#pragma unroll
      for (int r = 0; r < 8; r++) {
        sum[r].x += v[r].x; sum[r].y += v[r].y; sum[r].z += v[r].z; sum[r].w += v[r].w;
      }
    }
#pragma unroll
    for (int r = 0; r < 8; r++) {
      const int b0 = tid + 512 * r;
      zb0[cslot(b0)] = f2{sum[r].x, sum[r].y};
      zb0[cslot(CM + b0)] = f2{sum[r].z, sum[r].w};
    }
  }
  __syncthreads();
  auto quad = [&](int k, f2 a, f2 b) {
    f2 xk, xn, xm, xp;
    if (k == 0) {
      const f2 p0 = zb0[cslot(0)];
      xk = f2{p0.x, 0.f};
      xn = f2{p0.y, 0.f};
      xm = zb0[cslot(CM)];
      xp = xm;
    } else {
      xk = zb0[cslot(k)];
      xn = zb0[cslot(2 * CM - k)];
      xm = zb0[cslot(CM - k)];
      xp = zb0[cslot(CM + k)];
    }
    const f2 Ek = xk + cj(xn), Ok = cmulc(xk - cj(xn), cj(b));
    const f2 Emk = xm + cj(xp), Omk = cmulc(xm - cj(xp), mul_pi(b));
    const f2 ca = cj(a);
    const f2 fea = Ek + cj(Emk), foa = cmulc(Ek - cj(Emk), ca);
    const f2 feb = Ok + cj(Omk), fob = cmulc(Ok - cj(Omk), ca);
    const f2 zak = fea + mul_pi(foa), zam = cj(fea) + mul_pi(cj(foa));
    const f2 zbk = feb + mul_pi(fob), zbm = cj(feb) + mul_pi(cj(fob));
    zb0[cslot(k)] = zak;
    zb0[cslot(CM + k)] = zbk;
    if (k != 0 && k != CM / 2) {
      zb0[cslot(CM - k)] = zam;
      zb0[cslot(2 * CM - k)] = zbm;
    }
  };
#pragma unroll
  for (int q = 0; q < 4; q++) {
    const int k = tid + 512 * q;
    quad(k, f2{twab[k].x, twab[k].y}, f2{twab[2049 + k].x, twab[2049 + k].y});
  }
  if (tid == 0) quad(CM / 2, f2{twab[CM / 2].x, twab[CM / 2].y}, f2{twab[2049 + CM / 2].x, twab[2049 + CM / 2].y});
  __syncthreads();
  f2 own[16];
#pragma unroll
  for (int m = 0; m < 16; m++) {
    const f2 z = buf[cpad(t + 256 * m)];
    own[m] = f2{z.y, z.x};
  }
  __syncthreads();
  fft16_own<CM>(own, buf, tw2, tw3, t);
  __syncthreads();
#pragma unroll
  for (int m = 8; m < 16; m++) {
    const int o = 4 * (t + 256 * (m - 8)) + g;
    st[o] = own[m].y;
    st[o + 2] = own[m].x;
  }
  route(false);
}

const char* launch_coarse_inv(hipStream_t s, const CoarseOut* outs_dev, int nouts, int n_blocks, const int* ylist_dev, const float2* Y, int y_frames,
                              const float2* tw16, const float2* twab) {
  const int n_t = n_blocks;
  if (nouts <= 0 || n_t <= 0) return "";
  using PL = R16Plan<CM>;
  const size_t lds = (size_t)(PL::T2 + PL::T3 + 2 * CPAD) * sizeof(float2);
  static LdsLimit lim;
  lim.raise((const void*)coarse_inv_kernel, lds, "cannot raise the dynamic LDS limit of the coarse inverse transform");
  for (int r0 = 0; r0 < nouts; r0 += 32768)
    hipLaunchKernelGGL(coarse_inv_kernel, dim3(n_t, std::min(32768, nouts - r0)), dim3(512), lds, s, outs_dev + r0, ylist_dev, Y, y_frames,
                       tw16, twab);
  return "coarse_inv_kernel";
}

__global__ __launch_bounds__(256) void coarse_hist_kernel(const CoarseHistJob* __restrict jobs) {
  const CoarseHistJob J = jobs[blockIdx.y];
  const bool wide = (((uintptr_t)J.old_hist | (uintptr_t)J.in | (uintptr_t)J.new_hist) & 15) == 0;
  if (wide) {
    for (int64_t i = 4 * ((int64_t)blockIdx.x * blockDim.x + threadIdx.x); i < J.hist_len; i += 4 * (int64_t)gridDim.x * blockDim.x) {
      const int64_t sidx = i + J.n;
      v4f v = v4f{0.f, 0.f, 0.f, 0.f};
      if (sidx < J.hist_len) {
        if (J.old_hist) v = ldg4(J.old_hist + sidx);
      } else if (J.in) {
        v = ldg4(J.in + (sidx - J.hist_len));
      }
      stg4(J.new_hist + i, v);
    }
    return;
  }
  for (int64_t i = (int64_t)blockIdx.x * blockDim.x + threadIdx.x; i < J.hist_len; i += (int64_t)gridDim.x * blockDim.x) {
    const int64_t sidx = i + J.n;
    float v = 0.f;
    if (sidx < J.hist_len) v = J.old_hist ? ldg1(J.old_hist + sidx) : 0.f;
    else if (J.in) v = ldg1(J.in + (sidx - J.hist_len));
    stg1(J.new_hist + i, v);
  }
}
#ifndef GA_PREMIX_AHEAD
#define GA_PREMIX_AHEAD 8
#endif
#ifndef GA_PREMIX_WAVES
#define GA_PREMIX_WAVES 4
#endif
#ifndef GA_PREMIX_NT
#define GA_PREMIX_NT 0
#endif
constexpr int kPremixAhead = GA_PREMIX_AHEAD, kPremixWaves = GA_PREMIX_WAVES;
#ifndef GA_PREMIX_WORDS
#define GA_PREMIX_WORDS 1
#endif
#ifndef GA_PREMIX_COPY_WGS
#define GA_PREMIX_COPY_WGS 8
#endif
constexpr int kPremixCopyWgs = GA_PREMIX_COPY_WGS;
constexpr int kPremixWords = GA_PREMIX_WORDS, kPremixTile = 256 * kPremixWords;
struct Kahan4 {
  v4f s, c;
  __device__ __forceinline__ void add(v4f x) {
#ifdef GA_PREMIX_PLAIN
    s += x;
    return;
#endif
    const v4f y = x - c, t = s + y;
    c = (t - s) - y;
    s = t;
  }
};
template <bool ALIGNED, bool CARRY>
__device__ __forceinline__ void premix_stream(const PremixJob& J, const PremixTerm* __restrict terms, int t0, int t1, int lane,
                                              const uint32_t (&off)[kPremixWords], const bool (&keep)[kPremixWords],
                                              const uint32_t (&coff)[kPremixWords], Kahan4 (&acc)[kPremixWords]) {
  typedef const GA_GLOBAL char* gcp;
  typedef GA_GLOBAL char* gp;
  auto fetch = [&](gcp in, uint32_t o) -> v4f {
    if (ALIGNED) return GA_PREMIX_NT ? __builtin_nontemporal_load((const GA_GLOBAL v4f*)(in + o)) : *(const GA_GLOBAL v4f*)(in + o);
    const GA_GLOBAL float* p = (const GA_GLOBAL float*)(in + o);
    return v4f{p[0], p[1], p[2], p[3]};
  };
  auto put = [&](gp car, uint32_t o, v4f x) {
    if (GA_PREMIX_NT >= 2) __builtin_nontemporal_store(x, (GA_GLOBAL v4f*)(car + o));
    else *(GA_GLOBAL v4f*)(car + o) = x;
  };
  for (int base = t0; base < t1; base += 64) {
    const int nb = min(64, t1 - base);
    uint64_t pin = 0, pcar = 0;
    if (lane < nb) {
      const GA_GLOBAL PremixTerm* T = (const GA_GLOBAL PremixTerm*)terms + (J.term0 + base + lane);
      pin = (uint64_t)(uintptr_t)T->in;
      if (CARRY) pcar = (uint64_t)(uintptr_t)T->carry;
    }
    const int pin_lo = (int)(uint32_t)pin, pin_hi = (int)(uint32_t)(pin >> 32), pc_lo = (int)(uint32_t)pcar, pc_hi = (int)(uint32_t)(pcar >> 32);
    auto in_of = [&](int j) {
      return (gcp)(uintptr_t)(((uint64_t)(uint32_t)__builtin_amdgcn_readlane(pin_hi, j) << 32) | (uint32_t)__builtin_amdgcn_readlane(pin_lo, j));
// ... 16 lines not shown
          gp car = carry_of(j + u);
#pragma unroll
          for (int w = 0; w < kPremixWords; w++)
            if (car && keep[w]) put(car, coff[w], x[u][w]);
        }
#pragma unroll
        for (int w = 0; w < kPremixWords; w++) acc[w].add(x[u][w]);
      }
    }
    for (; j < nb; j++) {
      gcp in = in_of(j);
      gp car = CARRY ? carry_of(j) : nullptr;
#pragma unroll
      for (int w = 0; w < kPremixWords; w++) {
        const v4f x = fetch(in, off[w]);
        if (CARRY && car && keep[w]) put(car, coff[w], x);
        acc[w].add(x);
      }
    }
  }
}
__global__ __launch_bounds__(64 * kPremixWaves) void coarse_premix_kernel(const PremixJob* __restrict jobs, const PremixTerm* __restrict terms) {
  __shared__ v4f part[kPremixWaves - 1][2][kPremixWords][64];
  const PremixJob J = jobs[blockIdx.y];
  if (J.flags & 4) {
    if (blockIdx.x >= (unsigned)kPremixCopyWgs) return;
    const GA_GLOBAL v4f* src = (const GA_GLOBAL v4f*)terms[J.term0].in;
    GA_GLOBAL v4f* dst = (GA_GLOBAL v4f*)J.out;
    const int64_t nw = J.n / 4, step = (int64_t)kPremixCopyWgs * blockDim.x * 2;
    for (int64_t i = (int64_t)blockIdx.x * blockDim.x * 2 + threadIdx.x; i < nw; i += step) {
      const int64_t i2 = i + blockDim.x;
      const v4f a = src[i], b = i2 < nw ? src[i2] : a;
      dst[i] = a;
      if (i2 < nw) dst[i2] = b;
    }
    return;
  }
  const int64_t tile0 = (int64_t)blockIdx.x * kPremixTile;
  if (tile0 >= J.n) return;
  const int lane = threadIdx.x & 63, wv = __builtin_amdgcn_readfirstlane(threadIdx.x >> 6);
  int64_t f[kPremixWords];
  bool live[kPremixWords], keep[kPremixWords];
  uint32_t off[kPremixWords], coff[kPremixWords];
  Kahan4 acc[kPremixWords];
#pragma unroll
  for (int w = 0; w < kPremixWords; w++) {
    f[w] = tile0 + (int64_t)(w * 64 + lane) * 4;
    live[w] = f[w] < J.n;
    keep[w] = live[w] && f[w] >= J.carry_from;
    off[w] = live[w] ? (uint32_t)(f[w] * 4) : 0u;
    coff[w] = (uint32_t)((f[w] - J.carry_from) * 4);
    acc[w] = Kahan4{v4f{0.f, 0.f, 0.f, 0.f}, v4f{0.f, 0.f, 0.f, 0.f}};
  }
  const int per = ((J.nterms + kPremixWaves - 1) / kPremixWaves + kPremixAhead - 1) / kPremixAhead * kPremixAhead;
  const int t0 = min(J.nterms, wv * per), t1 = min(J.nterms, t0 + per);
  const bool carry_here = (J.flags & 2) && tile0 + kPremixTile > J.carry_from;
  if (J.flags & 1) {
    if (carry_here) premix_stream<true, true>(J, terms, t0, t1, lane, off, keep, coff, acc);
    else premix_stream<true, false>(J, terms, t0, t1, lane, off, keep, coff, acc);
  } else {
    if (carry_here) premix_stream<false, true>(J, terms, t0, t1, lane, off, keep, coff, acc);
    else premix_stream<false, false>(J, terms, t0, t1, lane, off, keep, coff, acc);
  }
  if (wv > 0) {
#pragma unroll
    for (int w = 0; w < kPremixWords; w++) {
      part[wv - 1][0][w][lane] = acc[w].s;
      part[wv - 1][1][w][lane] = acc[w].c;
    }
  }
  __syncthreads();
  if (wv == 0) {
#pragma unroll
    for (int w = 0; w < kPremixWords; w++) {
#pragma unroll
      for (int q = 0; q < kPremixWaves - 1; q++) {
        acc[w].add(part[q][0][w][lane]);
        acc[w].add(-part[q][1][w][lane]);
      }
      if (live[w]) stg4(J.out + f[w], acc[w].s);
    }
  }
}
const char* launch_coarse_premix(hipStream_t s, const PremixJob* jobs_dev, int njobs, const PremixTerm* terms_dev, int64_t max_n) {
  if (njobs <= 0 || max_n <= 0) return "";
  const int64_t gx = (max_n + kPremixTile - 1) / kPremixTile;
  if (gx > 0x7fffffff || max_n >= ((int64_t)1 << 29)) launch_fail("coarse pre-mix: chunk too long");
  for (int j0 = 0; j0 < njobs; j0 += 32768)
    hipLaunchKernelGGL(coarse_premix_kernel, dim3((unsigned)gx, std::min(32768, njobs - j0)), dim3(64 * kPremixWaves), 0, s, jobs_dev + j0, terms_dev);
  return "coarse_premix_kernel";
}

void launch_coarse_hist(hipStream_t s, const CoarseHistJob* jobs_dev, int njobs, int64_t max_len) {
  if (njobs <= 0 || max_len <= 0) return;
  const int gx = (int)std::min<int64_t>((max_len / 4 + 255) / 256, 64);
  for (int j0 = 0; j0 < njobs; j0 += 32768)
    hipLaunchKernelGGL(coarse_hist_kernel, dim3(gx, std::min(32768, njobs - j0)), dim3(256), 0, s, jobs_dev + j0);
}

__global__ __launch_bounds__(256) void table_upload_kernel(v4f* __restrict dst, const v4f* __restrict src, size_t n16) {
  for (size_t i = (size_t)blockIdx.x * 256 + threadIdx.x; i < n16; i += (size_t)gridDim.x * 256) ((GA_GLOBAL v4f*)dst)[i] = ((const GA_GLOBAL v4f*)src)[i];
}
void launch_table_upload(hipStream_t s, void* dst, const void* src_pinned, size_t bytes) {
  const size_t n16 = (bytes + 15) / 16;
  if (!n16) return;
  const unsigned grid = (unsigned)std::min<size_t>((n16 + 255) / 256, 64);
  hipLaunchKernelGGL(table_upload_kernel, dim3(grid), dim3(256), 0, s, (v4f*)dst, (const v4f*)src_pinned, n16);
}

}
```

graphaudio_amd/csrc/ga_engine.cpp:

```cpp
#include "ga_engine.hpp"

#include <algorithm>
#include <cstdio>
#include <cstring>

namespace ga {

void launch_fail(const char* what) { fail(GA_ERR_INVALID_OPERATION, std::string("internal: ") + what); }

void* Context::dalloc(size_t bytes) {
  void* p = nullptr;
  if (bytes == 0) bytes = 256;
  GA_HIP(hipMalloc(&p, bytes));
  devBytes += (int64_t)bytes;
  return p;
}
float* Context::dallocSkewed(size_t bytes, void** base, size_t* total) {
  *total = bytes + 64 * 1024;
  *base = dalloc(*total);
  return (float*)((char*)*base + (size_t)(skewSeq++ % 64) * 1024);
}
double Context::biquadDeviation(const float* coefs, int nsec) {
  std::vector<float> key(coefs, coefs + 5 * nsec);
  uint64_t h = 1469598103934665603ull;
// ... 264 lines not shown
  if (latched && !inRender) cmd(); else pending.push_back(std::move(cmd));
}
void Context::post(std::function<void()> cmd) {
  if (disposed) fail(GA_ERR_DISPOSED, "context disposed");
  pending.push_back(std::move(cmd));
}
void Context::drain() {
  while (!pending.empty()) {
    auto cmd = std::move(pending.front());
    pending.pop_front();
    apiEpoch++;
    try {
      cmd();
    } catch (const Err&) {
    }
  }
}

NodeS* Context::node(int id) {
  if (id < 0 || id >= (int)nodes.size()) fail(GA_ERR_INVALID_ARGUMENT, "bad node id");
  return nodes[id].get();
}
ParamS* Context::param(int nid, int p) {
  NodeS* n = node(nid);
  if (p < 0 || p >= (int)n->params.size()) fail(GA_ERR_INVALID_ARGUMENT, "bad param index");
  return &n->params[p];
}
PlayBuf* Context::buffer(int id) {
  if (id < 0) return nullptr;
  if (id >= (int)buffers.size() || !buffers[id]) fail(GA_ERR_INVALID_ARGUMENT, "bad buffer id");
  return buffers[id].get();
}
void Context::collectGarbage() {
  chunksSinceGc = 0;
  if (!releasedPending.empty()) {
    std::vector<char> used(buffers.size(), 0);
    for (auto& np : nodes) {
      if (!np || np->disposed) continue;
      if (np->bufId >= 0 && np->bufId < (int)used.size()) used[np->bufId] = 1;
      if (np->irBuf >= 0 && np->irBuf < (int)used.size()) used[np->irBuf] = 1;
      for (auto& e : np->dHistExt)
        if (e.first && e.second >= 0 && e.second < (int)used.size()) used[e.second] = 1;
      if (np->type == GA_NODE_STREAM_SOURCE) {
        if (np->stCurrent >= 0 && np->stCurrent < (int)used.size()) used[np->stCurrent] = 1;
        for (int id : np->stQueued) if (id >= 0 && id < (int)used.size()) used[id] = 1;
        for (int id : np->stProcessed) if (id >= 0 && id < (int)used.size()) used[id] = 1;
      }
    }
    std::vector<int> keep;
    bool synced = false;
    for (int id : releasedPending) {
      if (id < 0 || id >= (int)buffers.size() || !buffers[id]) continue;
      if (used[id]) {
        keep.push_back(id);
        continue;
      }
      if (!synced && stream) {
        (void)hipStreamSynchronize(stream);
        synced = true;
      }
      PlayBuf& b = *buffers[id];
      if (b.devBase) dfree(b.devBase, b.devBytes);
      bufVersion++;
      for (auto it = irCache.begin(); it != irCache.end();)
        it = it->first.first == id ? irCache.erase(it) : std::next(it);
      buffers[id].reset();
    }
    releasedPending.swap(keep);
  }
  for (auto it = irCache.begin(); it != irCache.end();) {
    if (it->second.use_count() == 1) {
      if (stream) (void)hipStreamSynchronize(stream);
      it = irCache.erase(it);
    } else {
      ++it;
    }
  }
}

InputS* Context::inputOf(const InRef& r) {
  NodeS* n = nodes[r.node].get();
  if (r.input >= 0) return &n->inputs[r.input];
  return nullptr;
}

void Context::harvestProfile(bool wait) {
  while (!pendingProf.empty()) {
    ProfBatch& b = pendingProf.front();
    if (wait) GA_HIP(hipEventSynchronize(b.end));
    else if (hipEventQuery(b.end) != hipSuccess) { (void)hipGetLastError(); break; }
    float ms = 0;
    GA_HIP(hipEventElapsedTime(&ms, b.begin, b.end));
    stats.device_ms_total += ms;
    stats.profiled_chunks++;
    for (size_t i = 0; i < b.evs.size(); i++) {
      GA_HIP(hipEventElapsedTime(&ms, b.evs[i].first, b.evs[i].second));
      const int k = b.kinds[i];
      if (k == LK_MAC || k == LK_CMAC) stats.mac_ms_total += ms;
      else if (k == LK_FFT || k == LK_IFFT || k == LK_CFWD || k == LK_CINV || k == LK_CHIST) stats.fft_ms_total += ms;
      else if (k != GA_STAGE_COARSE_SECTION) stats.other_ms_total += ms;
      if (k >= 0 && k < 16) stats.stage_ms[k] += ms;
      (void)hipEventDestroy(b.evs[i].first);
      (void)hipEventDestroy(b.evs[i].second);
    }
    (void)hipEventDestroy(b.begin);
    (void)hipEventDestroy(b.end);
    pendingProf.pop_front();
  }
}
void Context::flushHandOver() {
  for (const HandOver& h : pendingHandOver)
    GA_HIP(hipMemcpyAsync(h.dst_host, h.src, sizeof(float) * (size_t)h.n, hipMemcpyDeviceToHost, stream));
  pendingHandOver.clear();
}
void Context::synchronize() {
  GA_HIP(hipSetDevice(device));
  flushHandOver();
  commWait();
  waitHostCopies();
  harvestProfile(true);
  freeRetired();
}
void Context::freeRetired() {
  for (auto& r : retired) dfree(r.first, r.second);
  retired.clear();
}
void Context::waitHostCopies() {
  if (!copyStream) return;
  GA_HIP(hipStreamSynchronize(copyStream));
  outPending[0] = outPending[1] = false;
}
void Context::handOverToHost(const float* const* src, float* const* out, int channels, int64_t offset, int64_t frames) {
  if (!copyStream) {
    GA_HIP(hipStreamCreateWithFlags(&copyStream, hipStreamNonBlocking));
    for (int k = 0; k < 2; k++) {
      GA_HIP(hipEventCreateWithFlags(&outReady[k], hipEventDisableTiming));
      GA_HIP(hipEventCreateWithFlags(&outCopied[k], hipEventDisableTiming));
    }
  }
  const int k = outCur;
  outCur ^= 1;
  const size_t need = (size_t)channels * (size_t)frames * sizeof(float);
  if (outStageBytes[k] < need) {
    if (outPending[k]) GA_HIP(hipEventSynchronize(outCopied[k]));
    outPending[k] = false;
    if (outStage[k]) {
      GA_HIP(hipStreamSynchronize(stream));
      dfree(outStage[k], outStageBytes[k]);
      outStage[k] = nullptr;
      outStageBytes[k] = 0;
    }
    outStage[k] = (float*)dalloc(need);
    outStageBytes[k] = need;
  }
  if (outPending[k]) GA_HIP(hipStreamWaitEvent(stream, outCopied[k], 0));
  for (int ch = 0; ch < channels; ch++)
    GA_HIP(hipMemcpyAsync(outStage[k] + (size_t)ch * frames, src[ch], sizeof(float) * (size_t)frames, hipMemcpyDeviceToDevice, stream));
  GA_HIP(hipEventRecord(outReady[k], stream));
  GA_HIP(hipStreamWaitEvent(copyStream, outReady[k], 0));
  for (int ch = 0; ch < channels; ch++)
    GA_HIP(hipMemcpyAsync(out[ch] + offset, outStage[k] + (size_t)ch * frames, sizeof(float) * (size_t)frames, hipMemcpyDeviceToHost, copyStream));
  GA_HIP(hipEventRecord(outCopied[k], copyStream));
  outPending[k] = true;
}

void Context::connectTo(int src, int out, InRef in) {
// ... 495 lines not shown
  dfree(xi, planeBytes);
  dfree(rowsDev, sizeof(ConvRowIO) * nch);
  irCache[key] = sp;
  return sp;
}

const float2* Context::twiddles16(int N2) {
  auto it = tw16.find(N2);
  if (it != tw16.end()) return it->second;
  const double pi = 3.14159265358979323846264338327950288;
  const int R3 = N2 / 256;
  std::vector<float2> t;
  for (int m = 1; m < 16; m++)
    for (int kk = 0; kk < 16; kk++) t.push_back(make_float2((float)std::cos(2.0 * pi * kk * m / 256), (float)-std::sin(2.0 * pi * kk * m / 256)));
  for (int m = 1; m < R3; m++)
    for (int j = 0; j < 256; j++) t.push_back(make_float2((float)std::cos(2.0 * pi * j * m / N2), (float)-std::sin(2.0 * pi * j * m / N2)));
  float2* d = (float2*)dalloc(sizeof(float2) * t.size());
  GA_HIP(hipMemcpy(d, t.data(), sizeof(float2) * t.size(), hipMemcpyHostToDevice));
  tw16[N2] = d;
  return d;
}

void Context::streamFlushToProcessed(NodeS& s) {
  if (s.stCurrent >= 0) s.stProcessed.push_back(s.stCurrent);
  s.stCurrent = -1;
  while (!s.stQueued.empty()) {
    s.stProcessed.push_back(s.stQueued.front());
    s.stQueued.pop_front();
  }
  if (s.stChannels >= 0) {
    s.stRsPos = 0.0;
    s.stRsReady = 0;
    s.stWinValid = false;
  }
  s.stPos = 0;
  s.stLastRate = 0;
}

void Context::ensureOverlapStream() {
  if (stream2) return;
  GA_HIP(hipStreamCreateWithFlags(&stream2, hipStreamNonBlocking));
  for (auto& e : dGroupEv) GA_HIP(hipEventCreateWithFlags(&e, hipEventDisableTiming));
  GA_HIP(hipEventCreateWithFlags(&dJoinEv, hipEventDisableTiming));
}
const float2* Context::coarseTwab() {
  if (coarseTw) return coarseTw;
  const double pi = 3.14159265358979323846264338327950288;
  std::vector<float2> t(2 * 2049);
  for (int k = 0; k <= 2048; k++) {
    t[k] = make_float2((float)std::cos(2.0 * pi * k / 8192), (float)-std::sin(2.0 * pi * k / 8192));
    t[2049 + k] = make_float2((float)std::cos(2.0 * pi * k / 16384), (float)-std::sin(2.0 * pi * k / 16384));
  }
  coarseTw = (float2*)dalloc(sizeof(float2) * t.size());
  GA_HIP(hipMemcpy(coarseTw, t.data(), sizeof(float2) * t.size(), hipMemcpyHostToDevice));
  return coarseTw;
}
void Context::ensureCoarseSpectra(IrSpectra& ir) {
  if (ir.coarse) return;
  if (!ir.taps) fail(GA_ERR_INVALID_OPERATION, "internal: impulse response without device taps");
  const int P = (int)((ir.tapsStride + kCoarseBlock - 1) / kCoarseBlock);
  ir.coarseP = P;
  const int PS = P > kCoarseMaxP ? (P + kCoarseMaxP - 1) / kCoarseMaxP * kCoarseMaxP : P;
  ir.coarseStride = PS;
  ir.coarseBytes = (size_t)ir.nch * PS * kCoarseBins * sizeof(float2);
  ir.coarse = (float2*)dalloc(ir.coarseBytes);
  if (PS != P) GA_HIP(hipMemsetAsync(ir.coarse, 0, ir.coarseBytes, stream));
  std::vector<CoarseXRow> rows(ir.nch);
  for (int c = 0; c < ir.nch; c++) {
    CoarseXRow& r = rows[c];
    r.hist = nullptr;
    r.in = ir.taps + (size_t)c * ir.tapsStride;
    r.nvalid = ir.tapsStride;
    r.frame0 = c * PS;
    r.n_frames = P;
    r.u0 = 1;
    r.hist_len = 0;
    r.flags = 1;
    r.scale = 1.0f / 65536.0f;
    r.carry = nullptr;
    r.carry_from = 0;
  }
  CoarseXRow* rd = (CoarseXRow*)dalloc(sizeof(CoarseXRow) * rows.size());
  GA_HIP(hipMemcpy(rd, rows.data(), sizeof(CoarseXRow) * rows.size(), hipMemcpyHostToDevice));
  launch_coarse_fwd(stream, rd, ir.nch, P, P, ir.coarse, twiddles16pw(), coarseTwab());
  GA_HIP(hipGetLastError());
  GA_HIP(hipStreamSynchronize(stream));
  dfree(rd, sizeof(CoarseXRow) * rows.size());
}

const float2* Context::twiddles16pw() {
  if (tw16pw) return tw16pw;
  const double pi = 3.14159265358979323846264338327950288;
  std::vector<float2> t;
  for (int m = 1; m < 16; m++)
    for (int kk = 0; kk < 16; kk++) t.push_back(make_float2((float)std::cos(2.0 * pi * kk * m / 256), (float)-std::sin(2.0 * pi * kk * m / 256)));
  for (int m : {1, 2, 4, 8})
    for (int j = 0; j < 256; j++) t.push_back(make_float2((float)std::cos(2.0 * pi * j * m / 4096), (float)-std::sin(2.0 * pi * j * m / 4096)));
  tw16pw = (float2*)dalloc(sizeof(float2) * t.size());
  GA_HIP(hipMemcpy(tw16pw, t.data(), sizeof(float2) * t.size(), hipMemcpyHostToDevice));
  return tw16pw;
}

const float2* Context::twiddlesC(int N2) {
  auto it = twC.find(N2);
  if (it != twC.end()) return it->second;
  const double pi = 3.14159265358979323846264338327950288;
  std::vector<float2> t(N2);
  for (int j = 0; j < N2; j++) t[j] = make_float2((float)std::cos(2.0 * pi * j / N2), (float)-std::sin(2.0 * pi * j / N2));
  float2* d = (float2*)dalloc(sizeof(float2) * N2);
  GA_HIP(hipMemcpy(d, t.data(), sizeof(float2) * N2, hipMemcpyHostToDevice));
  twC[N2] = d;
  return d;
}
const float2* Context::ensureTapSpectra(IrSpectra& ir, int N2) {
  if (N2 != 1024 && N2 != 2048 && N2 != 4096) fail(GA_ERR_INVALID_OPERATION, "internal: no block-axis FFT of " + std::to_string(N2) + " points");
  float2*& h = ir.hspecN[IrSpectra::n2Index(N2)];
  if (h) return h;
  size_t bytes = (size_t)ir.nch * kBins * N2 * sizeof(float2);
  ir.hspecBytes += bytes;
  h = (float2*)dalloc(bytes);
  launch_tap_spectra(stream, h, ir.hr, ir.hi, ir.nch, ir.P, N2, twiddlesC(N2));
  GA_HIP(hipGetLastError());
  return h;
}

std::vector<Context::TconvLaunch> Context::tconvPlan(int nblocks, int P) const {
  static const int sizes[3] = {1024, 2048, 4096};
  static const double perPoint[3] = {0.577, 0.583, 0.70};
  std::vector<double> best(nblocks + 1, 0.0);
  std::vector<int> pick(nblocks + 1, -1);
  for (int rem = 1; rem <= nblocks; rem++) {
    best[rem] = 1e300;
    for (int i = 0; i < 3; i++) {
      const int L = sizes[i] - (P - 1);
      if (L < sizes[i] / 4) continue;
      const double c = sizes[i] * perPoint[i] + best[std::max(0, rem - L)];
      if (c < best[rem]) { best[rem] = c; pick[rem] = i; }
    }
    if (pick[rem] < 0) {
      pick[rem] = 2;
      best[rem] = 0;
    }
  }
  int count[3] = {0, 0, 0};
  for (int rem = nblocks; rem > 0;) {
    const int i = pick[rem];
    count[i]++;
    rem -= std::min(rem, sizes[i] - (P - 1));
  }
  if (const char* e = expenv("GA_TCONV_PLAN")) {
    int c0 = 0, c1 = 0, c2 = 0;
    if (sscanf(e, "%d,%d,%d", &c0, &c1, &c2) == 3 &&
        (long long)c0 * (1024 - (P - 1)) + (long long)c1 * (2048 - (P - 1)) + (long long)c2 * (4096 - (P - 1)) >= nblocks) {
      count[0] = c0; count[1] = c1; count[2] = c2;
    }
  }
  std::vector<TconvLaunch> plan;
  int tbase = 0;
  for (int i = 2; i >= 0; i--)
    if (count[i] > 0) {
      plan.push_back(TconvLaunch{sizes[i], tbase, count[i]});
      tbase += count[i] * (sizes[i] - (P - 1));
    }
  return plan;
}

void Resampler::extend(int64_t nblocks) {
// ... 34 lines not shown
```

graphaudio_amd/csrc/ga_engine.hpp:

```cpp
#pragma once
#include <cstring>
#include <initializer_list>
#include <new>
#include <hip/hip_runtime.h>

#include <algorithm>
#include <cmath>
#include <cstdint>
#include <deque>
#include <functional>
#include <limits>
#include <map>
#include <tuple>
#include <memory>
#include <string>
#include <unordered_map>
#include <vector>

#include "../../include/graphaudio_hip.h"
#include "ga_kernels.hpp"
#include "ga_gsr.hpp"

namespace ga {

// ... 519 lines not shown
  explicit Context(int sr) : sampleRate(sr) {}
  ~Context();
  void init_device(int device);
  void* dalloc(size_t bytes);
  void dfree(void* p, size_t bytes);
  void ensure(DevArena& a, size_t bytes);
  float* dallocSkewed(size_t bytes, void** base, size_t* total);
  int persistentBuffer(const float* p, int64_t n);
  struct BufSpan { const float* lo; const float* hi; int id; };
  std::vector<BufSpan> bufSpans;
  uint64_t bufVersion = 1, bufSpansVersion = 0;
  bool coarseExtHist = true;
  bool coarseMfma = true;
  bool coarseWide = true;
  bool gainFold = true;
  bool gainPassThrough = true;
  int biquadTimeSplit = 1;
  int64_t biquadSplitMinFrames = 16384;
  struct BqTransition { std::vector<float> key; std::vector<float> M; };
  std::unordered_map<uint64_t, std::vector<std::pair<std::vector<float>, double>>> bqDeviations;
  double biquadDeviation(const float* coefs, int nsec);
  std::unordered_map<uint64_t, std::vector<BqTransition>> bqTransitions;
  const BqTransition& biquadTransition(const float* coefs, int nsec, int64_t K);
  double biquadSplitMaxDeviation = 2.5e-6;
  std::vector<float*> bqSplitBlocks;
  size_t bqSplitUsed = 0;
  static constexpr size_t kBqSplitBlock = (size_t)4 << 20;
  float* bqSplitAlloc(size_t floats);
  unsigned skewSeq = 0;

  void executeOrPost(std::function<void()> cmd);
  void post(std::function<void()> cmd);
  void drain();

  NodeS* node(int id);
  ParamS* param(int node, int p);
  PlayBuf* buffer(int id);
  std::vector<int> releasedPending;
  int64_t chunksSinceGc = 0;
  void collectGarbage();
  InputS* inputOf(const InRef& r);

  void connectTo(int src, int out, InRef in);
  void disconnectFrom(int src, int out, InRef in);
  void outputDisconnectAll(int src, int out);
  void inputDisconnectAll(InRef in);
  void doDispose(int id);

  std::shared_ptr<IrSpectra> irSpectra(int bufId, bool normalize);
  void releaseConvState(NodeS& n);
  void refOrderSensitivity(const std::vector<int>& topo);
  bool ensureResampleSamples(Exec& ex, Resampler& rs, int64_t upto);
  bool rateModWalk = true;
  bool resampleFast = true;
  void assignConvPaths(const std::vector<int>& topo, int64_t chunkBlocks);
  hipStream_t copyStream = nullptr;
  bool hostCopyStream = false;
  hipEvent_t outReady[2] = {nullptr, nullptr}, outCopied[2] = {nullptr, nullptr};
  float* outStage[2] = {nullptr, nullptr};
  size_t outStageBytes[2] = {0, 0};
  bool outPending[2] = {false, false};
  int outCur = 0;
  void handOverToHost(const float* const* src, float* const* out, int channels, int64_t offset, int64_t frames);
  void waitHostCopies();
  hipStream_t stream2 = nullptr;
  hipEvent_t dGroupEv[8] = {nullptr, nullptr, nullptr, nullptr, nullptr, nullptr, nullptr, nullptr};
  hipEvent_t dJoinEv = nullptr;
  bool coarseOverlap = false;
  bool coarseTail = true;
  int convRefOrder = 1;
  double convRefMinDeviation = 2.5e-6;
  std::vector<char> refSensScratch;
  bool coarseTailPrivate = false;
  bool coarseCarry = true;
  bool coarseLong = true;
  bool coarsePremix = true;
  void ensureOverlapStream();
  void noteKernel(int kind, const char* name) {
    if (kind < 0 || kind >= 16 || !name || !*name) return;
    std::strncpy(stats.stage_kernel[kind], name, sizeof(stats.stage_kernel[kind]) - 1);
  }
  struct ExtraProf { hipEvent_t e0, e1; int kind; double bytes; };
  std::vector<ExtraProf> extraProf;
  std::vector<std::vector<NodeSeg>> segNodePool;
  std::vector<std::vector<Views>> viewsPool;
  DevArena coarseM;
  DevArena coarseX, coarseY;
  float2* coarseTw = nullptr;
  const float2* coarseTwab();
  float2* tw16pw = nullptr;
  const float2* twiddles16pw();
  void ensureCoarseSpectra(IrSpectra& ir);
  void planCoarseFusion(const std::vector<int>& topo, const std::vector<Segment>& segs);
  uint64_t fusionKey = 0;
  bool fusionKeyValid = false;
  void aliasBusToLeader(ChunkRun& r);
  ConvRowRef addGroupRow(const std::shared_ptr<IrSpectra>& ir, int ch, int depth, int nodeId);
  void ensureGroupState(ConvGroup& g);
  const float2* twiddlesC(int N2);
  const float2* twiddles16(int N2);
  std::map<int, float2*> tw16;
  bool useRadix16 = true;
  bool useCoarse = true;
  int64_t coarseMinBlocks = 256;
  int debugTconvN2 = 0;
  const float2* ensureTapSpectra(IrSpectra& ir, int N2);
  struct TconvLaunch { int N2, tbase, nseg; };
  std::vector<TconvLaunch> tconvPlan(int nblocks, int P) const;
  bool fft64 = false;
  bool useTimeFft = true;
  void updateBiquadCoefficients(NodeS& n, float frequency, float q, float gain);

  void render(float* const* out, int channels, int64_t frames, int64_t start, bool deviceOut);
  void runChunk(int64_t nblocks, float* const* bus);
  void runChunkImpl(int64_t nblocks, float* const* bus);
  void chunkTopology(ChunkRun& r);
  void chunkSimulate(ChunkRun& r);
  void chunkResources(ChunkRun& r);
  void chunkParamCurves(ChunkRun& r);
  void chunkConvScratch(ChunkRun& r);
  void chunkPlanNodes(ChunkRun& r, int depth);
  void planConstantSource(NodePlanCtx& k);
  void planOscillator(NodePlanCtx& k);
  void planDelay(NodePlanCtx& k);
  void planStereoPanner(NodePlanCtx& k);
  void planSpatialPanner(NodePlanCtx& k);
  void spatialGeometry(const NodeS& nd, const float* pv, int D, NodeS::SpatialPrev& out) const;
  float spatialParamAt(const NodeS& nd, int p, double t) const;
  float listener[12] = {0, 0, 0, 1, 0, 0, 0, 1, 0, 0, 0, -1};
  bool topoHasSpatial = false;
  void planBufferSource(NodePlanCtx& k);
  void planStreamSource(NodePlanCtx& k);
  void planGain(NodePlanCtx& k);
  void planBiquad(NodePlanCtx& k);
  void chunkPlanConvolvers(ChunkRun& r, int depth);
  void planConvolversShared(ChunkRun& r, int depth, ConvPlanCtx& k);
  void planConvolversPrivate(ChunkRun& r, int depth, ConvPlanCtx& k, bool refOrder);
  void chunkDelayCommit(ChunkRun& r);
  void chunkStaleSeed(ChunkRun& r);
  void chunkStaleCommit(ChunkRun& r);
  void chunkExecute(ChunkRun& r);
  void chunkCommit(ChunkRun& r);
  void chunkRetire(ChunkRun& r);
  void runTwoStageChunk(ChunkRun& r);
  void chunkRateProbe(ChunkRun& r);
  std::vector<std::pair<int, int>> topoRateMods;
  std::vector<char> rateCone;
  uint64_t rateModsVersion = ~0ull;
  void* rateModDev = nullptr;
  size_t rateModDevBytes = 0;
  void* rateModHost = nullptr;
  size_t rateModHostBytes = 0;
  void ensureBiquadState(NodeS& bn);
  void streamReplay(NodeS& s, int64_t nblocks, const std::vector<double>& bt, bool commit);
  void streamFlushToProcessed(NodeS& s);
  bool faulted = false;
  std::string faultMsg;
  int chunkPhase = 0;

  void* comm = nullptr;
  int commRanks = 0, commRank = 0;
  float* reduceBuf = nullptr;
  size_t reduceBytes = 0;
  bool commDead = false;
  double commTimeoutS = 120.0;
  void commInit(const void* id, int nRanks, int rank);
// ... 67 lines not shown
```

graphaudio_amd/csrc/ga_kernels.hpp:

```cpp
#pragma once
#include <hip/hip_runtime.h>
#include <stdint.h>
#include <stdlib.h>

namespace ga {

[[noreturn]] void launch_fail(const char* what);

#ifdef GA_EXPERIMENTS
inline const char* expenv(const char* name) { return getenv(name); }
#else
inline const char* expenv(const char*) { return nullptr; }
#endif

constexpr int kBlock = 128;
constexpr int kBins = 129;

struct ConvPlanes {
  float* xr;
  float* xi;
  float* yr;
  float* yi;
  int tx;
  int ty;
// ... 57 lines not shown
  int x;
  int y0;
  int ncol;
  int P;
  const float2* hs[16];
};
void launch_tap_spectra(hipStream_t s, float2* hs, const float* hr, const float* hi, int nch, int P, int N2, const float2* tw);
void launch_tconv(hipStream_t s, const ConvSetC* sets_dev, int nsets, int nblocks, int hist, ConvPlanesB pl, int N2, const float2* tw,
                  int nseg);
void launch_tconv16(hipStream_t s, const ConvSetC* sets_dev, int nsets, int nblocks, int hist, ConvPlanesB pl, int N2, const float2* tw16,
                    int nseg, int tbase);

constexpr int kCoarseBlock = 8192;
constexpr int kCoarseMaxP = 16;
constexpr int kCoarseMaxParts = 128;
constexpr int kCoarseJobTerms = 32;
constexpr int kCoarseSumJobBlocks(int columns) { return columns <= 2 ? 72 : 40; }
#ifndef GA_MAC_TW4
#define GA_MAC_TW4 4
#endif
constexpr int kCoarseJobBlocks(int columns) { return columns <= 2 ? 72 : (columns == 16 ? 32 : 8 * GA_MAC_TW4); }
constexpr double kCoarseTransformFlops = 2.0 * 3.0 * 256.0 * 200.0 + 2048.0 * 60.0;
constexpr int kCoarseBins = 8192;
struct CoarseXRow {
  const float* hist;
  const float* in;
  int64_t nvalid;
  int frame0;
  int n_frames;
  int u0;
  int hist_len;
  int flags;
  float scale;
  float* carry;
  int64_t carry_from;
};
struct CoarseHandOver {
  const float* src;
  float* dst;
  int64_t n;
};
struct CoarseTerm {
  int frame0;
  int pad_;
  const float2* h[16];
};
struct CoarseJob {
  int term0, n_terms;
  int P;
  int t0, n_t;
  int yrow0;
  int shared_h;
  int u_lo, u_hi;
  int pad_;
};
struct CoarseOut {
  float* out;
  int64_t nvalid;
  int y0, ny;
  const float* tail_in;
  float* tail_out;
  int64_t tail_len;
  int n_y;
  int pad_;
};
struct CoarseHistJob {
  const float* old_hist;
  const float* in;
  float* new_hist;
  int64_t hist_len, n;
};
struct PremixTerm {
  const float* in;
  float* carry;
};
struct PremixJob {
  float* out;
  int term0, nterms;
  int64_t n;
  int64_t carry_from;
  int flags;
  int pad_;
};
const char* launch_coarse_premix(hipStream_t s, const PremixJob* jobs_dev, int njobs, const PremixTerm* terms_dev, int64_t max_n);
const char* launch_coarse_fwd(hipStream_t s, const CoarseXRow* rows_dev, int nrows, int max_frames, int run, float2* X, const float2* tw16,
                       const float2* twab, const CoarseHandOver* handover_dev = nullptr, int n_handover = 0);
const char* launch_coarse_mac(hipStream_t s, const CoarseJob* jobs_dev, int njobs, const CoarseTerm* terms_dev, const float2* X, float2* Y,
                       int y_frames, int cw, int max_t, int maxP, bool any_private, int pb, bool matrix_cores = false);
const char* launch_coarse_inv(hipStream_t s, const CoarseOut* outs_dev, int nouts, int n_t, const int* ylist_dev, const float2* Y, int y_frames,
                       const float2* tw16, const float2* twab);
void launch_coarse_hist(hipStream_t s, const CoarseHistJob* jobs_dev, int njobs, int64_t max_len);
void launch_table_upload(hipStream_t s, void* dst, const void* src_pinned, size_t bytes);

struct MixJob {
  float* out;
  int term0;
  int nterms;
  int64_t f0;
  int64_t n;
  float* out2 = nullptr;
};
void launch_mix(hipStream_t s, const MixJob* jobs_dev, int njobs, const float* const* terms_dev, int64_t max_n, bool vec4, const float* gains_dev = nullptr,
                const float* const* curves_dev = nullptr);

void launch_mix_wide(hipStream_t s, const MixJob* jobs_dev, int njobs, const float* const* terms_dev, int64_t max_n, const float* gains_dev = nullptr,
                     const float* const* curves_dev = nullptr);
constexpr int kMixWideMinTerms = 256;

struct DownmixJob {
  float* out;
  int term0;
  int nch;
  float scale;
  int64_t f0;
  int64_t n;
};
void launch_downmix(hipStream_t s, const DownmixJob* jobs_dev, int njobs, const float* const* terms_dev, int64_t max_n, const float* gains_dev = nullptr);

struct GainJob {
  const float* in;
  float* out;
  const float* curve;
  const float* mod;
  float gain;
  float vmin, vmax;
  int64_t f0;
  int64_t n;
};
void launch_gain(hipStream_t s, const GainJob* jobs_dev, int njobs, int64_t max_n);

constexpr int kMaxBiquadSections = 8;
struct BiquadSection {
  float b0, b1, b2, a1, a2;
  float pad_;
  float* state;
};
struct BiquadJob {
  const float* in;
  float* out;
  int sec0;
  int nsec;
  int64_t f0;
  int64_t n;
  float* state;
  int twins = 1;
  int pad_ = 0;
};
void launch_biquad(hipStream_t s, const BiquadJob* jobs_dev, int njobs, const BiquadSection* secs_dev, int nsec);

struct BiquadScanJob {
  const float* in;
  float* out;
  uint64_t m_off;
  float* scratch;
  int sec0, nsec;
  int64_t f0, n;
  int twins = 1;
  int pad_ = 0;
};
void launch_biquad_split_expand(hipStream_t s, const BiquadScanJob* casc_dev, int ncasc, int G, int64_t K, BiquadJob* passA, BiquadJob* passB);
void launch_biquad_lanes(hipStream_t s, const BiquadJob* jobs_dev, int njobs, const BiquadSection* secs_dev, int nsec, bool state_only = false);
void launch_biquad_scan(hipStream_t s, const BiquadScanJob* casc_dev, int ncasc, int G, const BiquadSection* secs_dev, const uint8_t* tables, int nsec = 0);

struct BiquadDynState {
  float b0, b1, b2, a1, a2;
  int dirty;
  float w[64];
};
struct BiquadDynJob {
  const float* in[32];
  float* out[32];
  const float* fcurve;
  const float* qcurve;
  const float* gcurve;
// ... 285 lines not shown
```

graphaudio_amd/csrc/ga_plan_conv.cpp:

```cpp
#include "ga_chunk_internal.hpp"

namespace ga {

void Context::ensureGroupState(ConvGroup& g) {
  Context& c = *this;
  int need = (int)roundup(std::max<size_t>(g.rows.size(), 1), 128);
  if (need <= g.rp) return;
  const int hist = g.P - 1;
  size_t hBytes = (size_t)kBins * std::max(hist, 1) * need * sizeof(float);
  size_t oBytes = (size_t)need * kBlock * sizeof(float);
  float* nr = (float*)c.dalloc(hBytes);
  float* ni = (float*)c.dalloc(hBytes);
  float* o0 = (float*)c.dalloc(oBytes);
  float* o1 = (float*)c.dalloc(oBytes);
  GA_HIP(hipMemsetAsync(nr, 0, hBytes, c.stream));
  GA_HIP(hipMemsetAsync(ni, 0, hBytes, c.stream));
  GA_HIP(hipMemsetAsync(o0, 0, oBytes, c.stream));
  GA_HIP(hipMemsetAsync(o1, 0, oBytes, c.stream));
  if (g.rp > 0) {
    if (hist > 0 && !g.histZero) {
      GA_HIP(hipMemcpy2DAsync(nr, (size_t)need * 4, g.histR, (size_t)g.rp * 4, (size_t)g.rp * 4, (size_t)kBins * hist,
                              hipMemcpyDeviceToDevice, c.stream));
      GA_HIP(hipMemcpy2DAsync(ni, (size_t)need * 4, g.histI, (size_t)g.rp * 4, (size_t)g.rp * 4, (size_t)kBins * hist,
                              hipMemcpyDeviceToDevice, c.stream));
// ... 65 lines not shown
    auto it = leaderOf.find(key);
    if (it == leaderOf.end()) leaderOf.emplace(key, id);
    else nd.dLeader = it->second;
  }
}

static const float* convChunkInput(Context& c, Exec& ex, const Exec::ConvInRow& ci, int ch) {
  const auto& segs = ex.segs;
  const float* stable = nullptr;
  bool same = true, first = true;
  for (size_t si = 0; si < segs.size(); si++) {
    const float* v = (ci[si].empty() || ch >= (int)ci[si].size()) ? nullptr : ci[si][ch];
    if (first) { stable = v; first = false; } else if (v != stable) same = false;
  }
  if (same) return stable;
  float* slab = getSlab(c);
  for (size_t si = 0; si < segs.size(); si++) {
    const float* v = (ci[si].empty() || ch >= (int)ci[si].size()) ? nullptr : ci[si][ch];
    MixJob mj;
    mj.out = slab;
    mj.term0 = (int)ex.terms.size();
    mj.nterms = v ? 1 : 0;
    mj.f0 = segs[si].b0 * kBlock;
    mj.n = (segs[si].b1 - segs[si].b0) * kBlock;
    if (v) {
      ex.terms.push_back(v);
      ex.noteAlign(v, mj.f0);
    }
    ex.mixJobs.push_back(mj);
  }
  return slab;
}

static const float* coarseHistory(const NodeS& nd, int ch) {
  if (ch < (int)nd.dHistExt.size() && nd.dHistExt[ch].first) return nd.dHistExt[ch].first;
  return nd.dHistZero ? nullptr : nd.dHist[nd.dHistCur] + (size_t)ch * nd.dHistLen;
}

static bool coarseHistoryStays(Context& c, NodeS& nd, int ch, const float* in, int64_t frames) {
  if ((int)nd.dHistExt.size() < nd.bInCh) nd.dHistExt.resize(nd.bInCh, {nullptr, -1});
  const int64_t hl = nd.dHistLen;
  int buf = -1;
  if (c.coarseExtHist && in && frames >= hl) buf = c.persistentBuffer(in + (frames - hl), hl);
  nd.dHistExt[ch] = buf >= 0 ? std::make_pair(in + (frames - hl), buf) : std::make_pair((const float*)nullptr, -1);
  return buf >= 0;
}

namespace {
struct CoarseStage {
  Context& c;
  Exec& ex;
  const std::vector<int>& dNodes;
  const int64_t n, frames;
  const int nT;
  static constexpr int kVoicesPerJob = kCoarseJobTerms;
  struct Piece {
    int frame0, P, xrow, u0;
    IrSpectra* ir;
    int leader;
    int ncol;
    int irCh[16], outCh[16];
  };
  struct GroupInfo {
    uint64_t sig = 1469598103934665603ull;
    int maxP = 0, nIn = 0, nOut = 0;
    const void* ir0 = nullptr;
    bool oneIr = true, tail = false, carried = false, fresh = true, noHist = false;
    bool uniform = true, premix = false;
    int members = 0, nxr = 0, bInCh0 = 0, bSlots0 = 0;
    bool ts0 = false;
    int64_t hl0 = 0;
    struct Terms { std::vector<PremixTerm> in[32], hist[32]; };
    std::unique_ptr<Terms> terms;
  };
  std::vector<Views> chInOf;
  bool wideStrided = true;
  std::vector<CoarseHandOver> fwdHandOver;
  std::vector<PremixJob> pmJobs;
  std::vector<PremixTerm> pmTerms;
  size_t pmUsed = 0;
  int64_t pmMaxN = 0;
  double pmBytes = 0;
  std::vector<CoarseXRow> xrows;
  std::vector<CoarseHistJob> hjobs;
  std::vector<Piece> pieces;
  std::map<int, GroupInfo> groups;
  const bool tails;
  int frameNext = 0;
  int64_t maxHist = 0;
  double histBytes = 0;
  std::map<int, double> carryBytes;
  int nxAll = 0, G = 1;
  int gBegin[9] = {};
  std::vector<CoarseTerm> terms;
  static constexpr int kCwOf[4] = {1, 2, 4, 16};
  std::vector<CoarseJob> jobs[16][8];
  int maxT[16] = {}, maxP[16] = {};
  int pbOf[16] = {4, 4, 4, 4, 4, 4, 4, 4, 4, 4, 4, 4, 4, 4, 4, 4};
  double macBytes[16][8] = {}, macFlops[16][8] = {};
  double pmFlops = 0, invFlops = 0;
  std::map<std::pair<int, int>, std::vector<int>> outRows;
  int yNext = 0;
  std::vector<CoarseOut> outs;
  std::vector<int> ylist;
  double invBytes = 0;
  int yFrames = 0, invBlocks = 0;

  CoarseStage(Context& c_, Exec& ex_, const std::vector<int>& d, int64_t n_)
      : c(c_), ex(ex_), dNodes(d), n(n_), frames(n_ * kBlock), nT((int)((n_ * kBlock + kCoarseBlock - 1) / kCoarseBlock)), tails(c_.coarseTail) {}
  void resolveInputs();
  void classifyGroups();
  void buildRows();
  void addPieces(NodeS& nd, int leader, int nxr, const int* xFrame, const int* xIndex);
  void buildJobs();
  void buildOutputs();
  void enqueue();
};

void CoarseStage::resolveInputs() {
  chInOf.resize(dNodes.size());
  for (size_t di = 0; di < dNodes.size(); di++) {
    const int id = dNodes[di];
    NodeS& nd = *c.nodes[id];
    const int64_t hl = nd.dHistLen;
    const Exec::ConvInRow ci = ex.convIn[id];
    Views& chIn = chInOf[di];
    chIn.assign(nd.bInCh, nullptr);
    auto viewOf = [&](size_t si, int ch) { return (ci[si].empty() || ch >= (int)ci[si].size()) ? (const float*)nullptr : ci[si][ch]; };
    for (int ch = 0; ch < nd.bInCh; ch++) {
      int same = -1;
      for (int e = 0; e < ch && same < 0; e++) {
        bool eq = true;
        for (size_t si = 0; si < ex.segs.size() && eq; si++) eq = viewOf(si, e) == viewOf(si, ch);
        if (eq) same = e;
      }
      chIn[ch] = same >= 0 ? chIn[same] : convChunkInput(c, ex, ci, ch);
    }
    bool allSame = true;
    for (int ch = 1; ch < nd.bInCh; ch++) allSame = allSame && (chIn[ch] == chIn[0]);
    if (nd.bShared && !allSame) {
      if (const float* h0 = coarseHistory(nd, 0))
        for (int ch = 1; ch < nd.bInCh; ch++) {
          float* dst = nd.dHist[nd.dHistCur] + (size_t)ch * hl;
          hipStream_t st = c.stream;
          ex.plan.add(LK_OTHER, [=](uint8_t*) { GA_HIP(hipMemcpyAsync(dst, h0, (size_t)hl * sizeof(float), hipMemcpyDeviceToDevice, st)); });
          if (ch < (int)nd.dHistExt.size()) nd.dHistExt[ch] = {nullptr, -1};
        }
      if (nd.dHistZero && coarseHistory(nd, 0)) nd.dHistZero = false;
      nd.bShared = false;
    }
  }
}

void CoarseStage::classifyGroups() {
  {
    auto mix = [](uint64_t& h, uint64_t v) { h = (h ^ v) * 1099511628211ull; };
    for (int id : dNodes) {
      NodeS& nd = *c.nodes[id];
      GroupInfo& g = groups[nd.dLeader >= 0 ? nd.dLeader : id];
      mix(g.sig, (uint64_t)id);
      mix(g.sig, (uint64_t)(uintptr_t)nd.ir.get());
      mix(g.sig, (uint64_t)nd.bInCh | ((uint64_t)nd.bSlots << 8) | ((uint64_t)nd.isTrueStereo << 16) | ((uint64_t)nd.bShared << 17) |
                     ((uint64_t)nd.ir->coarseP << 24));
      g.maxP = std::max(g.maxP, nd.ir->coarseP);
      g.fresh = g.fresh && nd.dHistZero;
      g.nIn += nd.bShared ? 1 : nd.bInCh;
// ... 43 lines not shown
      pc.frame0 = xFrame[xc];
      pc.xrow = xIndex[xc];
      pc.u0 = xrows[xIndex[xc]].u0;
      pc.P = ir.coarseP;
      pc.ir = &ir;
      pc.leader = leader;
      pc.ncol = w;
      for (int j = 0; j < w; j++) {
        pc.irCh[j] = cols[c0 + j][0];
        pc.outCh[j] = cols[c0 + j][1];
      }
      pieces.push_back(pc);
      c0 += w;
    }
  }
}

void CoarseStage::buildRows() {
  for (size_t di = 0; di < dNodes.size(); di++) {
    const int id = dNodes[di];
    NodeS& nd = *c.nodes[id];
    IrSpectra& ir = *nd.ir;
    const int P = ir.coarseP;
    if (P < 1 || P > kCoarseMaxParts) fail(GA_ERR_INVALID_OPERATION, "internal: coarse partition count out of range");
    const int64_t hl = nd.dHistLen;
    GroupInfo& gi0 = groups[nd.dLeader >= 0 ? nd.dLeader : id];
    const bool carried = gi0.noHist;
    const Views& chIn = chInOf[di];
    const int nxr = nd.bShared ? 1 : nd.bInCh;
    c.stats.mac_flops_total += 8.0 * ir.P * kBins * (double)nd.bSlots * (double)n;
    c.stats.mac_bytes_total += ((double)ir.P * kBins * 8.0 + kBins * 8.0 + 512.0) * nd.bSlots * (double)n;
    if (gi0.premix) {
      for (int ch = 0; ch < nxr; ch++) {
        const float* oldHist = coarseHistory(nd, ch);
        float* nextHist = nd.dHist[nd.dHistCur ^ 1] + (size_t)ch * hl;
        PremixTerm t{chIn[ch], nullptr};
        if (coarseHistoryStays(c, nd, ch, chIn[ch], frames)) {
        } else if (c.coarseCarry && chIn[ch] && frames >= hl && ((uintptr_t)nextHist & 15) == 0) {
          t.carry = nextHist;
          pmBytes += (double)hl * 4.0;
        } else {
          hjobs.push_back(CoarseHistJob{oldHist, chIn[ch], nextHist, hl, frames});
          maxHist = std::max(maxHist, hl);
          histBytes += 2.0 * (double)hl * 4.0;
        }
        if (!gi0.terms) gi0.terms = std::make_unique<GroupInfo::Terms>();
        gi0.terms->in[ch].push_back(t);
        if (!carried) gi0.terms->hist[ch].push_back(PremixTerm{oldHist, nullptr});
      }
      nd.dHistCur ^= 1;
      nd.dHistZero = false;
      continue;
    }
    int xFrame[32], xIndex[32];
    for (int ch = 0; ch < nxr; ch++) {
      CoarseXRow r;
      const float* oldHist = coarseHistory(nd, ch);
      r.hist = carried ? nullptr : oldHist;
      r.in = chIn[ch];
      r.nvalid = frames;
      r.frame0 = frameNext;
      r.u0 = carried ? 0 : -(P - 1);
      r.n_frames = (gi0.tail ? nT + 1 : nT) - r.u0;
      r.hist_len = (int)hl;
      r.flags = 0;
      r.scale = 1.0f;
      xFrame[ch] = frameNext;
      xIndex[ch] = (int)xrows.size();
      frameNext += r.n_frames;
      float* nextHist = nd.dHist[nd.dHistCur ^ 1] + (size_t)ch * hl;
      r.carry = nullptr;
      r.carry_from = 0;
      if (coarseHistoryStays(c, nd, ch, r.in, frames)) {
      } else if (c.coarseCarry && r.in && frames >= hl && (((uintptr_t)r.in | (uintptr_t)nextHist) & 15) == 0) {
        r.carry = nextHist;
        r.carry_from = frames - hl;
        carryBytes[(int)xrows.size()] = (double)hl * 4.0;
      } else {
        hjobs.push_back(CoarseHistJob{oldHist, r.in, nextHist, hl, frames});
        maxHist = std::max(maxHist, hl);
        histBytes += 2.0 * (double)hl * 4.0;
      }
      xrows.push_back(r);
    }
    nd.dHistCur ^= 1;
    nd.dHistZero = false;
    addPieces(nd, nd.dLeader >= 0 ? nd.dLeader : id, nxr, xFrame, xIndex);
  }
  for (auto& kv : groups) {
    GroupInfo& g = kv.second;
    if (!g.premix) continue;
    NodeS& ld = *c.nodes[kv.first];
    const int64_t hl = g.hl0;
    int xFrame[32], xIndex[32];
    for (int ch = 0; ch < g.nxr; ch++) {
      const size_t bytes = (size_t)(hl + frames) * sizeof(float);
      if (pmUsed + bytes > c.coarseM.bytes) fail(GA_ERR_INVALID_OPERATION, "internal: the pre-mix arena is too small for the plan");
      float* mixed = (float*)((char*)c.coarseM.p + pmUsed);
      pmUsed += (bytes + 255) & ~(size_t)255;
      auto job = [&](float* out, const std::vector<PremixTerm>& tv, int64_t len, int64_t carryFrom) {
        PremixJob j{out, (int)pmTerms.size(), 0, len, carryFrom, 1, 0};
        for (const PremixTerm& t : tv) {
          if (!t.in) continue;
          pmTerms.push_back(t);
          j.nterms++;
          if ((uintptr_t)t.in & 15) j.flags &= ~1;
          if (t.carry) j.flags |= 2;
          pmBytes += (double)len * 4.0;
          pmFlops += (double)len * 4.0;
        }
        pmJobs.push_back(j);
        pmMaxN = std::max(pmMaxN, len);
        pmBytes += (double)len * 4.0;
      };
      if (!g.terms) g.terms = std::make_unique<GroupInfo::Terms>();
      if (!g.noHist) job(mixed, g.terms->hist[ch], hl, hl);
      job(mixed + hl, g.terms->in[ch], frames, std::max<int64_t>(0, frames - hl));
      CoarseXRow r{};
      r.hist = g.noHist ? nullptr : mixed;
      r.in = mixed + hl;
      r.nvalid = frames;
      r.frame0 = frameNext;
      r.u0 = g.noHist ? 0 : -(g.maxP - 1);
      r.n_frames = (g.tail ? nT + 1 : nT) - r.u0;
      r.hist_len = (int)hl;
      r.flags = 0;
      r.scale = 1.0f;
      r.carry = nullptr;
      r.carry_from = 0;
      xFrame[ch] = frameNext;
      xIndex[ch] = (int)xrows.size();
      frameNext += r.n_frames;
      xrows.push_back(r);
    }
    addPieces(ld, kv.first, g.nxr, xFrame, xIndex);
    c.stats.coarse_premixed_signals += (int64_t)g.members * g.nxr;
  }
  if (!pmJobs.empty() && !c.pendingHandOver.empty()) {
    std::vector<PremixJob> head;
    for (const Context::HandOver& h : c.pendingHandOver) {
      head.push_back(PremixJob{h.dst_dev, (int)pmTerms.size(), 1, h.n, h.n, 1 | 4, 0});
      pmTerms.push_back(PremixTerm{h.src, nullptr});
      pmMaxN = std::max(pmMaxN, h.n);
      pmBytes += 2.0 * (double)h.n * 4.0;
    }
    pmJobs.insert(pmJobs.begin(), head.begin(), head.end());
    c.pendingHandOver.clear();
    c.stats.deferred_handovers++;
  } else if (!c.pendingHandOver.empty() && !xrows.empty()) {
    for (const Context::HandOver& h : c.pendingHandOver) fwdHandOver.push_back(CoarseHandOver{h.src, h.dst_dev, h.n});
    c.pendingHandOver.clear();
    c.stats.deferred_handovers++;
  }
  ex.flushLevel();
}

void CoarseStage::buildJobs() {
  struct Key {
    int leader, P, ncol;
    std::array<int, 16> out;
    bool operator<(const Key& o) const { return std::tie(leader, P, ncol, out) < std::tie(o.leader, o.P, o.ncol, o.out); }
  };
  std::map<Key, std::vector<const Piece*>> byKey;
  for (const Piece& pc : pieces) {
    Key k{pc.leader, pc.P, pc.ncol, {}};
    k.out.fill(-1);
// ... 109 lines not shown
    std::map<int, int> chOf;
    for (auto& kv : outRows) chOf[kv.first.first] = std::max(chOf[kv.first.first], kv.first.second + 1);
    for (auto& kv : groups) {
      if (!kv.second.tail) continue;
      NodeS& ld = *c.nodes[kv.first];
      const int64_t len = (int64_t)(kv.second.maxP + 1) * kCoarseBlock;
      const int nch = chOf.count(kv.first) ? chOf[kv.first] : 0;
      if (nch == 0) continue;
      if (!ld.dTail[0] || ld.dTailLen != len || ld.dTailCh != nch) {
        if (kv.second.carried) fail(GA_ERR_INVALID_OPERATION, "internal: a carried tail changed its shape");
        GA_HIP(hipStreamSynchronize(c.stream));
        for (int b = 0; b < 2; b++) {
          if (ld.dTail[b]) c.dfree(ld.dTail[b], (size_t)ld.dTailLen * ld.dTailCh * sizeof(float));
          ld.dTail[b] = (float*)c.dalloc((size_t)len * nch * sizeof(float));
        }
        ld.dTailLen = len;
        ld.dTailCh = nch;
        ld.dTailCur = 0;
      }
    }
  }
  for (auto& kv : outRows) {
    CoarseOut o{};
    o.out = ex.nodeOut(kv.first.first, kv.first.second);
    o.nvalid = frames;
    o.y0 = (int)ylist.size();
    o.ny = (int)kv.second.size();
    o.n_y = nT;
    if (groups[kv.first.first].tail) {
      NodeS& ld = *c.nodes[kv.first.first];
      const GroupInfo& gi = groups[kv.first.first];
      o.n_y = nT + gi.maxP;
      o.tail_len = ld.dTailLen;
      o.tail_in = gi.carried ? ld.dTail[ld.dTailCur] + (size_t)kv.first.second * ld.dTailLen : nullptr;
      o.tail_out = ld.dTail[ld.dTailCur ^ 1] + (size_t)kv.first.second * ld.dTailLen;
      invBlocks = std::max(invBlocks, (int)((frames + o.tail_len + kCoarseBlock - 1) / kCoarseBlock));
      invBytes += (double)o.tail_len * 4.0 * (gi.carried ? 2.0 : 1.0);
      if (gi.carried) c.stats.coarse_carried_outputs++;
    }
    ylist.insert(ylist.end(), kv.second.begin(), kv.second.end());
    outs.push_back(o);
    invBytes += (double)o.ny * o.n_y * kCoarseBins * 8.0 + (double)frames * 4.0;
    invFlops += (double)o.n_y * (kCoarseTransformFlops + (double)o.ny * 2.0 * kCoarseBins);
  }
  if (tails)
    for (auto& kv : groups) {
      NodeS& ld = *c.nodes[kv.first];
      if (!kv.second.tail || !ld.dTail[0]) continue;
      ld.dTailCur ^= 1;
      ld.dTailSig = kv.second.sig;
      ld.dTailSeq = c.chunkSeq;
    }
  if ((size_t)frameNext * kCoarseBins * sizeof(float2) > c.coarseX.bytes || (size_t)yNext * yFrames * kCoarseBins * sizeof(float2) > c.coarseY.bytes)
    fail(GA_ERR_INVALID_OPERATION, "internal: coarse spectra arenas are too small for the plan");

}

void CoarseStage::enqueue() {
  const int G = this->G, yFrames = this->yFrames, invBlocks = this->invBlocks, nxAll = this->nxAll;
  const double invBytes = this->invBytes, histBytes = this->histBytes;
  const size_t xo = ex.plan.putv(xrows), ho = ex.plan.putv(hjobs), to = ex.plan.putv(terms), oo = ex.plan.putv(outs), yo = ex.plan.putv(ylist);
  const size_t pjo = ex.plan.putv(pmJobs), pto = ex.plan.putv(pmTerms), fho = ex.plan.putv(fwdHandOver);
  const int nfh = (int)fwdHandOver.size();
  const int npm = (int)pmJobs.size();
  const int64_t pmMaxN = this->pmMaxN;
  const double pmBytes = this->pmBytes, pmFlops = this->pmFlops, invFlops = this->invFlops;
  struct MacLaunch { size_t off; int nj, cw, mt, mp, pb, grp; bool ap; double bytes, flops; };
  const bool matrixCores = c.coarseMfma && wideStrided;
  std::vector<MacLaunch> macs;
  for (int g = 0; g < G; g++)
    for (int i = 0; i < 16; i++) {
      if (jobs[i][g].empty()) continue;
      macs.push_back(MacLaunch{ex.plan.putv(jobs[i][g]), (int)jobs[i][g].size(), kCwOf[(i & 7) >> 1], maxT[i], maxP[i], pbOf[i], g, (i & 1) == 0,
                               macBytes[i][g], macFlops[i][g]});
      c.stats.mac_launches += 1;
    }
  hipStream_t st = c.stream;
  float2* X = (float2*)c.coarseX.p;
  float2* Y = (float2*)c.coarseY.p;
  const float2* tw16 = c.twiddles16(4096);
  const float2* twFwd = c.twiddles16pw();
  const float2* twab = c.coarseTwab();
  const int nh = (int)hjobs.size(), no = (int)outs.size();
  struct FwdLaunch { int x0, nx, maxFrames, run; double bytes, flops; };
  std::vector<FwdLaunch> fwds;
  for (int g = 0; g < G; g++) {
    FwdLaunch f{this->gBegin[g], this->gBegin[g + 1] - this->gBegin[g], 0, 1, 0.0, 0.0};
    for (int x = f.x0; x < f.x0 + f.nx; x++) {
      f.maxFrames = std::max(f.maxFrames, xrows[x].n_frames);
      f.bytes += (double)(xrows[x].n_frames + 1) * kCoarseBlock * 4.0 + (double)xrows[x].n_frames * kCoarseBins * 8.0;
      f.flops += (double)xrows[x].n_frames * kCoarseTransformFlops;
      if (auto it = carryBytes.find(x); it != carryBytes.end()) f.bytes += it->second;
    }
    while (f.run < 16 && (int64_t)nxAll * ((f.maxFrames + 2 * f.run - 1) / (2 * f.run)) >= 1024) f.run *= 2;
    if (f.run >= 8) {
      const int k = (f.maxFrames + 11) / 12;
      f.run = (f.maxFrames + k - 1) / k;
    }
    if (const char* e = expenv("GA_COARSE_RUN")) f.run = std::max(1, atoi(e));
    fwds.push_back(f);
  }
  if (G > 1) c.ensureOverlapStream();
  Context* cp = &c;
  ex.plan.add(GA_STAGE_COARSE_SECTION, [=](uint8_t* base) {
    auto timed = [&](hipStream_t sx, int kind, double bytes, double flops, const std::function<const char*()>& launch) {
      hipEvent_t e0 = nullptr, e1 = nullptr;
      if (cp->profileNow) {
        GA_HIP(hipEventCreate(&e0));
        GA_HIP(hipEventCreate(&e1));
        GA_HIP(hipEventRecord(e0, sx));
      }
      cp->noteKernel(kind, launch());
      if (cp->profileNow) {
        GA_HIP(hipEventRecord(e1, sx));
        cp->extraProf.push_back(Context::ExtraProf{e0, e1, kind, bytes});
      }
      cp->stats.kernel_launches++;
      cp->stats.stage_launches[kind]++;
      cp->stats.stage_bytes[kind] += bytes;
      cp->stats.stage_flops[kind] += flops;
    };
    hipStream_t s2 = G > 1 ? cp->stream2 : st;
    if (npm > 0)
      timed(st, LK_CPREMIX, pmBytes, pmFlops, [&] { return launch_coarse_premix(st, (const PremixJob*)(base + pjo), npm, (const PremixTerm*)(base + pto), pmMaxN); });
    for (int g = 0; g < G; g++) {
      const FwdLaunch& f = fwds[g];
      if (f.nx > 0)
        timed(st, LK_CFWD, f.bytes, f.flops, [&] {
          return launch_coarse_fwd(st, (const CoarseXRow*)(base + xo) + f.x0, f.nx, f.maxFrames, f.run, X, twFwd, twab,
                                   (const CoarseHandOver*)(base + fho), g == 0 ? nfh : 0);
        });
      if (G > 1) {
        GA_HIP(hipEventRecord(cp->dGroupEv[g], st));
        GA_HIP(hipStreamWaitEvent(s2, cp->dGroupEv[g], 0));
      }
      for (const MacLaunch& m : macs)
        if (m.grp == g)
          timed(s2, LK_CMAC, m.bytes, m.flops, [&] {
            return launch_coarse_mac(s2, (const CoarseJob*)(base + m.off), m.nj, (const CoarseTerm*)(base + to), X, Y, yFrames, m.cw, m.mt, m.mp, m.ap, m.pb,
                                     matrixCores);
          });
    }
    if (G > 1) {
      GA_HIP(hipEventRecord(cp->dJoinEv, s2));
      GA_HIP(hipStreamWaitEvent(st, cp->dJoinEv, 0));
    }
  });
  ex.plan.add(LK_CINV, [=](uint8_t* base) {
    cp->noteKernel(LK_CINV, launch_coarse_inv(st, (const CoarseOut*)(base + oo), no, invBlocks, (const int*)(base + yo), Y, yFrames, tw16, twab));
  }, invBytes, invFlops);
  const int64_t mh = maxHist;
  if (nh > 0) ex.plan.add(LK_CHIST, [=](uint8_t* base) { launch_coarse_hist(st, (const CoarseHistJob*)(base + ho), nh, mh); }, histBytes);
}
}

static void planCoarseStage(Context& c, Exec& ex, const std::vector<int>& dNodes, int64_t n) {
  CoarseStage s(c, ex, dNodes, n);
  s.resolveInputs();
  s.classifyGroups();
  s.buildRows();
  s.buildJobs();
  s.buildOutputs();
  s.enqueue();
}

void Context::aliasBusToLeader(ChunkRun& r) {
  Exec& ex = *r.ex;
  int leader = -1, nch = 0;
  for (const Segment& sg : r.segs) {
    if (sg.nodes.empty() || sg.nodes.back().id != 0 || sg.nodes.back().ins.empty()) return;
    const InSeg& is = sg.nodes.back().ins[0];
    for (const TermS& t : is.terms) {
      const NodeS& nd = *nodes[t.node];
      if (nd.type != GA_NODE_CONVOLVER || !nd.ir || nd.convPath != 4 || nd.dLeader < 0 || t.out != 0 || t.ch != is.bufCh) return;
      if (leader < 0) {
        leader = nd.dLeader;
        nch = is.bufCh;
      } else if (leader != nd.dLeader || nch != is.bufCh) {
        return;
      }
    }
  }
  if (leader < 0 || nch < 1 || nch > (int)busSlabs.size()) return;
  const NodeS& ld = *nodes[leader];
  if (ld.outputs.empty() || ld.outputs[0].connectedInputs.size() != 1) return;
  const InRef& to = ld.outputs[0].connectedInputs[0];
  if (to.node != 0 || to.input != 0) return;
  for (int ch = 0; ch < nch; ch++) ex.setNodeOut(leader, ch, busTarget[ch] ? busTarget[ch] : busSlabs[ch]);
}

void Context::chunkConvScratch(ChunkRun& r) {
  Context& c_ = *this; (void)c_;
  std::vector<int>& topo = r.topo;
  int& maxDepth = r.maxDepth; int& maxLevel = r.maxLevel; (void)maxDepth; (void)maxLevel;
  int64_t& n = r.n; (void)n;
  std::vector<double>& bt = r.bt; (void)bt;
  std::vector<int>& srcIds = r.srcIds; (void)srcIds;
  std::vector<SrcPlanOut>& srcPlans = r.srcPlans; (void)srcPlans;
  std::vector<Segment>& segs = r.segs; (void)segs;
  const int64_t frames = r.n * kBlock; (void)frames;
  int& bHistMax = r.bHistMax; (void)bHistMax;
  for (auto& kv : resamplers) kv.second->devOffset = -1;

  if (topoHasConvolvers && r.stage != 1) {
    refOrderSensitivity(topo);
    assignConvPaths(topo, n);
    for (int id : topo) {
      NodeS& nd = *nodes[id];
      if (nd.type == GA_NODE_CONVOLVER) nd.refOrder = nd.refSens && nd.ir && (nd.convPath == 2 || nd.convPath == 3);
    }
    planCoarseFusion(topo, segs);
    for (int id : topo)
      if (nodes[id]->type == GA_NODE_CONVOLVER) nodes[id]->dGroupSize = 0;
    for (int id : topo) {
      const NodeS& nd = *nodes[id];
      if (nd.type == GA_NODE_CONVOLVER && nd.ir && nd.convPath == 4 && nd.dLeader >= 0) nodes[nd.dLeader]->dGroupSize++;
    }
    aliasBusToLeader(r);
  }
  bHistMax = 0;
  if (topoHasConvolvers) {
    size_t xMax = 0, yMax = 0;
    size_t bx = 0, by = 0;
    for (int id : topo) {
      NodeS& nd = *nodes[id];
      if (nd.type != GA_NODE_CONVOLVER || !nd.ir) continue;
      if (nd.convPath == 2 || nd.convPath == 3) {
        bx += nd.bInCh;
        by += nd.bSlots;
        bHistMax = std::max(bHistMax, nd.ir->P - 1);
      }
      for (auto& rr : nd.convRows) {
        ConvGroup& g = *rr.group;
        ensureGroupState(g);
        const int ty_ = (int)roundup(n, 64), tx_ = ty_ + g.P + 128;
// ... 498 lines not shown
```

include/graphaudio_hip.h:

```cpp
#ifndef GRAPHAUDIO_HIP_H
#define GRAPHAUDIO_HIP_H

#include <stdint.h>

#ifdef __cplusplus
extern "C" {
#endif

#ifndef GA_FN
#define GA_FN(name) ga_##name
#endif

#if defined(__GNUC__)
#define GA_EXPORT __attribute__((visibility("default")))
#else
#define GA_EXPORT
#endif

#define GA_OK 0
#define GA_ERR_INVALID_ARGUMENT (-1)
#define GA_ERR_OUT_OF_RANGE (-2)
#define GA_ERR_INVALID_OPERATION (-3)
#define GA_ERR_DISPOSED (-4)
#define GA_ERR_CYCLE (-5)
#define GA_ERR_UNSUPPORTED (-6)
#define GA_ERR_DEVICE (-7)
#define GA_ERR_OUT_OF_MEMORY (-8)
#define GA_ERR_NO_DEVICE (-9)

enum {
  GA_NODE_DESTINATION = 0,
  GA_NODE_BUFFER_SOURCE = 1,
  GA_NODE_GAIN = 2,
  GA_NODE_BIQUAD = 3,
  GA_NODE_CONVOLVER = 4,
  GA_NODE_CHANNEL_SPLITTER = 5,
  GA_NODE_CHANNEL_MERGER = 6,
  GA_NODE_CONSTANT_SOURCE = 7,
  GA_NODE_STEREO_PANNER = 8,
  GA_NODE_OSCILLATOR = 9,
  GA_NODE_DELAY = 10,
  GA_NODE_STREAM_SOURCE = 11,
  GA_NODE_SPATIAL_PANNER = 12
};
enum { GA_DISTANCE_LINEAR = 0, GA_DISTANCE_INVERSE = 1, GA_DISTANCE_EXPONENTIAL = 2 };
enum { GA_SPATIAL_PARAM_COUNT = 17, GA_SPATIAL_DISTANCE_MODEL = 17, GA_SPATIAL_HRIR_AZIMUTHS = 18 };
enum { GA_STREAM_PLAYING = 0, GA_STREAM_PAUSED = 1, GA_STREAM_STOPPED = 2 };
enum { GA_FILTER_LOWPASS = 0, GA_FILTER_HIGHPASS, GA_FILTER_BANDPASS, GA_FILTER_NOTCH, GA_FILTER_ALLPASS,
       GA_FILTER_PEAKING, GA_FILTER_LOWSHELF, GA_FILTER_HIGHSHELF };
enum { GA_OSC_SINE = 0, GA_OSC_SQUARE, GA_OSC_SAWTOOTH, GA_OSC_TRIANGLE };
enum { GA_COUNT_MODE_MAX = 0, GA_COUNT_MODE_CLAMPED_MAX = 1, GA_COUNT_MODE_EXPLICIT = 2 };
enum { GA_INTERP_SPEAKERS = 0, GA_INTERP_DISCRETE = 1 };

typedef struct ga_context ga_context;

typedef struct ga_stats {
  int64_t blocks_rendered;
  int64_t chunks;
  int64_t segments;
  int64_t kernel_launches;
  double  device_ms_total;
  int64_t mac_launches;
  double  mac_ms_total;
  double  mac_flops_total;
  double  mac_bytes_total;
  double  fft_ms_total;
  double  other_ms_total;
  int64_t device_bytes_in_use;
  int32_t n_nodes;
  int32_t n_conv_rows;
  double  stage_ms[16];
  int64_t stage_launches[16];
  double  stage_bytes[16];
  int64_t profiled_chunks;
  int64_t coarse_carried_outputs;
  double  stage_flops[16];
  char    stage_kernel[16][64];
  int64_t coarse_premixed_signals;
  int64_t deferred_handovers;
  int64_t biquad_split_cascades;
  int64_t ref_order_rows;
  int64_t sim_replays;
  int64_t twin_rows;
} ga_stats;
enum {
  GA_STAGE_OTHER = 0,
  GA_STAGE_MIX = 1,
  GA_STAGE_RFFT_FWD = 2,
  GA_STAGE_MAC = 3,
  GA_STAGE_RFFT_INV = 4,
  GA_STAGE_COARSE_FWD = 5,
  GA_STAGE_COARSE_MAC = 6,
  GA_STAGE_COARSE_INV = 7,
  GA_STAGE_COARSE_HIST = 8,
  GA_STAGE_COARSE_SECTION = 9,
  GA_STAGE_COARSE_PREMIX = 10,
  GA_STAGE_COUNT = 11
};

GA_EXPORT const char* GA_FN(strerror)(int code);
GA_EXPORT const char* GA_FN(version)(void);
GA_EXPORT int GA_FN(device_count)(void);

GA_EXPORT int GA_FN(context_create)(int sample_rate, int device_ordinal, ga_context** out);
GA_EXPORT int GA_FN(context_destroy)(ga_context* ctx);
GA_EXPORT const char* GA_FN(last_error)(ga_context* ctx);
GA_EXPORT double GA_FN(current_time)(ga_context* ctx);
GA_EXPORT int64_t GA_FN(current_block)(ga_context* ctx);
GA_EXPORT int GA_FN(set_option)(ga_context* ctx, const char* key, double value);
GA_EXPORT int GA_FN(get_stats)(ga_context* ctx, ga_stats* out);

GA_EXPORT int GA_FN(buffer_create)(ga_context* ctx, const float* const* planar, int channels, int64_t frames,
                                   int sample_rate, int* out_buffer_id);
GA_EXPORT int GA_FN(buffer_release)(ga_context* ctx, int buffer_id);

GA_EXPORT int GA_FN(node_create)(ga_context* ctx, int node_type, int* out_node_id);
GA_EXPORT int GA_FN(node_create_ex)(ga_context* ctx, int node_type, double arg, int* out_node_id);
GA_EXPORT int GA_FN(node_dispose)(ga_context* ctx, int node);
GA_EXPORT int GA_FN(node_connect)(ga_context* ctx, int src, int dst, int output_index, int input_index);
GA_EXPORT int GA_FN(node_disconnect)(ga_context* ctx, int src, int dst, int output_index, int input_index);
GA_EXPORT int GA_FN(node_connect_param)(ga_context* ctx, int src, int dst_node, int dst_param, int output_index);
GA_EXPORT int GA_FN(node_disconnect_param)(ga_context* ctx, int src, int dst_node, int dst_param, int output_index);
GA_EXPORT int GA_FN(node_has_ended)(ga_context* ctx, int node);
GA_EXPORT int GA_FN(poll_ended)(ga_context* ctx, int* out_node_ids, int capacity);

GA_EXPORT int GA_FN(input_set_channel_count)(ga_context* ctx, int node, int input_index, int count);
GA_EXPORT int GA_FN(input_set_channel_count_mode)(ga_context* ctx, int node, int input_index, int mode);
GA_EXPORT int GA_FN(input_set_channel_interpretation)(ga_context* ctx, int node, int input_index, int interpretation);
GA_EXPORT int GA_FN(destination_set_channel_count)(ga_context* ctx, int channels);
GA_EXPORT int GA_FN(destination_output_channels)(ga_context* ctx);

GA_EXPORT int GA_FN(param_set_value)(ga_context* ctx, int node, int param, float value);
GA_EXPORT int GA_FN(param_get_value)(ga_context* ctx, int node, int param, float* out);
GA_EXPORT int GA_FN(param_set_value_at_time)(ga_context* ctx, int node, int param, float value, double start_time);
GA_EXPORT int GA_FN(param_linear_ramp_to_value_at_time)(ga_context* ctx, int node, int param, float value, double end_time);
GA_EXPORT int GA_FN(param_exponential_ramp_to_value_at_time)(ga_context* ctx, int node, int param, float value, double end_time);
GA_EXPORT int GA_FN(param_set_target_at_time)(ga_context* ctx, int node, int param, float target, double start_time,
                                              double time_constant);
GA_EXPORT int GA_FN(param_cancel_scheduled_values)(ga_context* ctx, int node, int param, double cancel_time);

GA_EXPORT int GA_FN(source_set_buffer)(ga_context* ctx, int node, int buffer_id);
GA_EXPORT int GA_FN(source_set_loop)(ga_context* ctx, int node, int loop, double loop_start, double loop_end);
GA_EXPORT int GA_FN(source_start)(ga_context* ctx, int node, double when, double offset, double duration);
GA_EXPORT int GA_FN(source_stop)(ga_context* ctx, int node, double when);

GA_EXPORT int GA_FN(oscillator_set_type)(ga_context* ctx, int node, int oscillator_type);

GA_EXPORT int GA_FN(biquad_set_type)(ga_context* ctx, int node, int filter_type);

GA_EXPORT int GA_FN(convolver_set_normalize)(ga_context* ctx, int node, int normalize);
GA_EXPORT int GA_FN(convolver_set_enable_true_stereo)(ga_context* ctx, int node, int enable);
GA_EXPORT int GA_FN(convolver_set_buffer)(ga_context* ctx, int node, int buffer_id);

GA_EXPORT int GA_FN(stream_queue_buffer)(ga_context* ctx, int node, int buffer_id);
GA_EXPORT int GA_FN(stream_set_state)(ga_context* ctx, int node, int state);
GA_EXPORT int GA_FN(stream_dequeue_processed)(ga_context* ctx, int node, int* buffer_id_out);
GA_EXPORT int GA_FN(stream_queued_count)(ga_context* ctx, int node);
GA_EXPORT int GA_FN(stream_processed_count)(ga_context* ctx, int node);

GA_EXPORT int GA_FN(render)(ga_context* ctx, float* const* out_planar, int out_channels, int64_t frame_count,
                            int64_t start_index);
GA_EXPORT int GA_FN(render_device)(ga_context* ctx, float* const* out_planar_dev, int out_channels, int64_t frame_count,
                                   int64_t start_index);
GA_EXPORT int GA_FN(process_blocks)(ga_context* ctx, float* const* out_planar, int out_channels, int64_t block_count,
                                    int out_on_device);
GA_EXPORT int GA_FN(process_blocks_interleaved)(ga_context* ctx, float* interleaved, int channels, int64_t block_count,
// ... 20 lines not shown
```

Measured before the change: 1.225 billion.

## Add 512-thread one-window-per-workgroup coarse forward FFT for small grids

Adds a wide variant of the coarse forward transform. Each 512-thread workgroup handles a single window, and two half-groups split the input columns and the post-processing quads. It is picked automatically when run length is 1, there are no hand-over rows, all rows come from premix, and the total window count fits within the CU count, so more of the GPU works in parallel when there are few windows. Profiling is also reworked: kernels now record their own events through hipExtLaunchKernelGGL instead of being wrapped in separate event records. The wide path needs more LDS and allows only one block per CU.

```diff
diff --git a/graphaudio_amd/_capi.py b/graphaudio_amd/_capi.py
--- a/graphaudio_amd/_capi.py
+++ b/graphaudio_amd/_capi.py
@@ -77,6 +77,7 @@
         ("ref_order_rows", C.c_int64),
         ("sim_replays", C.c_int64),
         ("twin_rows", C.c_int64),
+        ("coarse_fwd_wide_launches", C.c_int64),
     ]
     STAGES = ("other", "mix", "rfft_fwd", "mac", "rfft_inv", "coarse_fwd", "coarse_mac", "coarse_inv", "coarse_hist", "coarse_section",
               "coarse_premix")
diff --git a/graphaudio_amd/csrc/ga_api.cpp b/graphaudio_amd/csrc/ga_api.cpp
--- a/graphaudio_amd/csrc/ga_api.cpp
+++ b/graphaudio_amd/csrc/ga_api.cpp
@@ -364,6 +364,7 @@
     else if (k == "conv_reference_order") c.convRefOrder = (int)std::min(2.0, std::max(0.0, value));
     else if (k == "conv_ref_min_deviation") c.convRefMinDeviation = std::max(0.0, value);
     else if (k == "coarse_premix") c.coarsePremix = value != 0;
+    else if (k == "coarse_fwd_wide") c.coarseFwdWide = value != 0;
     else if (k == "coarse_long") c.coarseLong = value != 0;
     else if (k == "coarse_ext_history") c.coarseExtHist = value != 0;
     else if (k == "coarse_wide") c.coarseWide = value != 0;
diff --git a/graphaudio_amd/csrc/ga_chunk.cpp b/graphaudio_amd/csrc/ga_chunk.cpp
--- a/graphaudio_amd/csrc/ga_chunk.cpp
+++ b/graphaudio_amd/csrc/ga_chunk.cpp
@@ -679,14 +679,15 @@
     GA_HIP(hipEventRecord(evBegin, stream));
   }
   for (auto& l : ex.plan.launches) {
+    const bool wrap = profile && !l.selfTimed && l.kind != GA_STAGE_COARSE_SECTION;
     hipEvent_t e0 = nullptr, e1 = nullptr;
-    if (profile) {
+    if (wrap) {
       GA_HIP(hipEventCreate(&e0));
       GA_HIP(hipEventCreate(&e1));
       GA_HIP(hipEventRecord(e0, stream));
     }
     l.fn(base);
-    if (profile) {
+    if (wrap) {
       GA_HIP(hipEventRecord(e1, stream));
       evs.push_back({e0, e1});
       evKind.push_back(l.kind);
diff --git a/graphaudio_amd/csrc/ga_chunk_internal.hpp b/graphaudio_amd/csrc/ga_chunk_internal.hpp
--- a/graphaudio_amd/csrc/ga_chunk_internal.hpp
+++ b/graphaudio_amd/csrc/ga_chunk_internal.hpp
@@ -26,6 +26,7 @@
     int kind;
     double bytes;
     double flops;
+    bool selfTimed = false;
   };
   std::vector<L> launches;
   size_t put(const void* p, size_t bytes) {
@@ -40,6 +41,9 @@
   }
   void add(int kind, std::function<void(uint8_t*)> fn, double bytes = 0.0, double flops = 0.0) {
     launches.push_back(L{std::move(fn), kind, bytes, flops});
+  }
+  void addSelfTimed(int kind, std::function<void(uint8_t*)> fn, double bytes = 0.0, double flops = 0.0) {
+    launches.push_back(L{std::move(fn), kind, bytes, flops, true});
   }
 };
 
diff --git a/graphaudio_amd/csrc/ga_coarse.hip b/graphaudio_amd/csrc/ga_coarse.hip
--- a/graphaudio_amd/csrc/ga_coarse.hip
+++ b/graphaudio_amd/csrc/ga_coarse.hip
@@ -2,6 +2,7 @@
 #include "ga_fft16.hpp"
 
 #include <hip/hip_runtime.h>
+#include <hip/hip_ext.h>
 
 #include <algorithm>
 #include <atomic>
@@ -28,6 +29,27 @@
     if (hipFuncSetAttribute(kern, hipFuncAttributeMaxDynamicSharedMemorySize, (int)std::max<size_t>(need, 65536)) != hipSuccess) launch_fail(what);
   }
 };
+
+static thread_local LaunchEvents* tl_events = nullptr;
+struct EventScope {
+  explicit EventScope(LaunchEvents* ev) { tl_events = ev; }
+  ~EventScope() { tl_events = nullptr; }
+};
+template <class T>
+struct arg_of { using type = T; };
+template <typename... KA>
+static void coarse_launch(bool first, bool last, void (*kern)(KA...), dim3 grid, dim3 block, size_t lds, hipStream_t s, typename arg_of<KA>::type... args) {
+  LaunchEvents* ev = tl_events;
+  hipEvent_t e0 = ev && first ? ev->start : nullptr, e1 = ev && last ? ev->stop : nullptr;
+  if (e0 || e1) {
+    hipExtLaunchKernelGGL(kern, grid, block, (uint32_t)lds, s, e0, e1, 0u, args...);
+    ev->used = true;
+  } else {
+    hipLaunchKernelGGL(kern, grid, block, (uint32_t)lds, s, args...);
+  }
+}
+constexpr int kLaunchRows = 32768;
+static bool last_piece(int r0, int n) { return r0 + kLaunchRows >= n; }
 
 constexpr int CM = 4096;
 constexpr int CPAD = TC16_PADDED(CM);
@@ -74,7 +96,9 @@
   return (unsigned)(uintptr_t)(const __attribute__((address_space(3))) f2*)p;
 }
 
-__device__ __forceinline__ void coarse_issue_half(const CoarseXRow& R, int hw, int t, v4f (&raw)[8]) {
+template <class V>
+__device__ __forceinline__ void coarse_issue_half(const CoarseXRow& R, int hw, int t, int sub, V (&raw)[8]) {
+  static_assert(sizeof(V) == 16 || sizeof(V) == 8, "whole words or half words");
   const float* src = nullptr;
   int64_t lim = 0;
   if (hw < 0) {
@@ -92,21 +116,121 @@
 #pragma unroll
   for (int q = 0; q < 8; q++) {
     const int o = 4 * (t + 256 * q);
-    raw[q] = v4f{0.f, 0.f, 0.f, 0.f};
+    raw[q] = V(0.f);
     if (src && o < lim) {
-      if (aligned) raw[q] = ldg4(src + o);
-      else raw[q] = v4f{ldg1(src + o), ldg1(src + o + 1), ldg1(src + o + 2), ldg1(src + o + 3)};
-    }
-  }
-}
+      if constexpr (sizeof(V) == 16) {
+        if (aligned) raw[q] = ldg4(src + o);
+        else raw[q] = v4f{ldg1(src + o), ldg1(src + o + 1), ldg1(src + o + 2), ldg1(src + o + 3)};
+      } else {
+        if (aligned) raw[q] = ldg2(src + o + sub);
+        else raw[q] = v2f{ldg1(src + o + sub), ldg1(src + o + sub + 1)};
+      }
+    }
+  }
+}
+template <class V>
+__device__ __forceinline__ void coarse_carry_half(const CoarseXRow& R, int u, int t, int sub, const V (&second)[8]) {
+  if (R.carry && u >= 0 && (int64_t)(u + 1) * kCoarseBlock > R.carry_from) {
+#pragma unroll
+    for (int q = 0; q < 8; q++) {
+      const int64_t sidx = (int64_t)u * kCoarseBlock + 4 * (t + 256 * q);
+      if (sidx >= R.carry_from && sidx < R.nvalid) *(GA_GLOBAL V*)(R.carry + (sidx - R.carry_from) + sub) = second[q];
+    }
+  }
+}
+__device__ __forceinline__ void coarse_fwd_quad(float2* __restrict F, int k, f2 Ak, f2 Am, f2 Bk, f2 Bm, f2 b, int exp) {
+  const f2 a = cmulc(b, b);
+  const f2 aB = cmulc(a, Bk), caBm = cmulc(cj(a), Bm);
+  const f2 Wk = Ak + aB, Wp = Ak - aB;
+  const f2 Wm = Am - caBm, Wn = Am + caBm;
+  const f2 fe = Wk + cj(Wn), bfo = cmulc(b, mul_mi(Wk - cj(Wn)));
+  const f2 Xk = fe + bfo, Xn = cj(fe - bfo);
+  const f2 fe2 = Wm + cj(Wp), wfo2 = cmulc(mul_mi(cj(b)), mul_mi(Wm - cj(Wp)));
+  const f2 Xm = fe2 + wfo2, Xp = cj(fe2 - wfo2);
+  if (exp & 1) {
+    if (Xk.x == 12345.f && Xn.x == 54321.f && Xm.x == 999.f && Xp.y == 777.f) F[0] = make_float2(0.f, 0.f);
+  } else if (k == 0) {
+    stg4(F, v4f{Xk.x, Xn.x, Xm.x, Xm.y});
+  } else if (k == CM / 2) {
+    stg4(F + 2 * k, v4f{Xk.x, Xk.y, Xn.x, Xn.y});
+  } else {
+    stg4(F + 2 * k, v4f{Xk.x, Xk.y, Xp.x, Xp.y});
+    stg4(F + 2 * (CM - k), v4f{Xm.x, Xm.y, Xn.x, Xn.y});
+  }
+}
+__device__ constexpr float kW64[8][2] = {{1.f, 0.f},
+                                         {0.99518472667219688624f, -0.09801714032956060199f},
+                                         {0.98078528040323044913f, -0.19509032201612826785f},
+                                         {0.95694033573220886494f, -0.29028467725446236764f},
+                                         {0.92387953251128675613f, -0.38268343236508977173f},
+                                         {0.88192126434835502971f, -0.47139673682599764856f},
+                                         {0.83146961230254523708f, -0.55557023301960222474f},
+                                         {0.77301045336273696081f, -0.63439328416364549822f}};
 
 constexpr int kHandOverWgs = 8;
 constexpr int kFwdPark = 4;
 constexpr int kFwdTw3 = 4 * 256;
-template <bool EXPERIMENT>
-__global__ __launch_bounds__(256, 3) void coarse_fwd_kernel(const CoarseXRow* __restrict rows, int run, float2* __restrict X,
+__device__ __forceinline__ void coarse_fwd_window_wide(const CoarseXRow& R, int w, float2* __restrict X, const float2* __restrict twg,
+                                                       const float2* __restrict twab) {
+  using PL = R16Plan<CM>;
+  extern __shared__ f2 clds[];
+  f2* tw2 = clds;
+  f2* tw3 = clds + PL::T2;
+  f2* zb0 = clds + PL::T2 + kFwdTw3;
+  if (w >= R.n_frames) return;
+  const int tid = threadIdx.x;
+  const int g = __builtin_amdgcn_readfirstlane(tid >> 8), t = tid & 255;
+  f2* buf = zb0 + g * CPAD;
+  const float2 tb0g = twab[2049 + t];
+  const float2 tbhg = twab[2049 + (tid == 0 ? CM / 2 : t)];
+  for (int i = tid; i < PL::T2 + kFwdTw3; i += 512) clds[i] = f2{twg[i].x, twg[i].y};
+  const int u = R.u0 + w;
+  const float scale = R.scale;
+  v2f first[8], second[8];
+  coarse_issue_half(R, u - 1, t, 2 * g, first);
+  if (R.flags & 1) {
+#pragma unroll
+    for (int q = 0; q < 8; q++) second[q] = v2f(0.f);
+  } else {
+    coarse_issue_half(R, u, t, 2 * g, second);
+  }
+  coarse_carry_half(R, u, t, 2 * g, second);
+  f2 own[16];
+#pragma unroll
+  for (int m = 0; m < 8; m++) {
+    own[m] = f2{first[m].x * scale, first[m].y * scale};
+    own[8 + m] = f2{second[m].x * scale, second[m].y * scale};
+  }
+  __syncthreads();
+  fft16_own<CM, true>(own, buf, tw2, tw3, t);
+  __syncthreads();
+  const int xw = cpad(t);
+#pragma unroll
+  for (int m = 0; m < 16; m++) buf[xw + 264 * m] = own[m];
+  __syncthreads();
+  const f2* __restrict za = zb0;
+  const f2* __restrict zb = zb0 + CPAD;
+  float2* __restrict F = X + (size_t)(R.frame0 + w) * kCoarseBins;
+  const f2 tb0 = f2{tb0g.x, tb0g.y};
+#pragma unroll
+  for (int q = 0; q < 4; q++) {
+    const int k = tid + 512 * q;
+    const int km = k == 0 ? 0 : CM - k;
+    const f2 w64 = g ? f2{kW64[2 * q + 1][0], kW64[2 * q + 1][1]} : f2{kW64[2 * q][0], kW64[2 * q][1]};
+    const f2 b = (q == 0 && g == 0) ? tb0 : cmulc(tb0, w64);
+    coarse_fwd_quad(F, k, za[cpad(k)], za[cpad(km)], zb[cpad(k)], zb[cpad(km)], b, 0);
+  }
+  if (tid == 0) coarse_fwd_quad(F, CM / 2, za[cpad(CM / 2)], za[cpad(CM / 2)], zb[cpad(CM / 2)], zb[cpad(CM / 2)], f2{tbhg.x, tbhg.y}, 0);
+}
+
+template <bool EXPERIMENT, bool WIDE>
+__global__ __launch_bounds__(WIDE ? 512 : 256, WIDE ? 1 : 3) void coarse_fwd_kernel(const CoarseXRow* __restrict rows, int run, float2* __restrict X,
                                                             const float2* __restrict twg, const float2* __restrict twab, int exp_,
                                                             const CoarseHandOver* __restrict handover, int n_handover) {
+  if constexpr (WIDE) {
+    coarse_fwd_window_wide(rows[blockIdx.y], blockIdx.x, X, twg, twab);
+    return;
+  }
   if ((int)blockIdx.y < n_handover) {
     const int nwg = min((int)gridDim.x, kHandOverWgs);
     if ((int)blockIdx.x >= nwg) return;
@@ -139,12 +263,12 @@
   const float scale = R.scale;
   const int wave64 = __builtin_amdgcn_readfirstlane(t_ & ~63);
   v4f first[8], second[8];
-  coarse_issue_half(R, R.u0 + w0 - 1, t_, first);
+  coarse_issue_half(R, R.u0 + w0 - 1, t_, 0, first);
   if (zero2) {
 #pragma unroll
     for (int q = 0; q < 8; q++) second[q] = v4f{0.f, 0.f, 0.f, 0.f};
   } else {
-    coarse_issue_half(R, R.u0 + w0, t_, second);
+    coarse_issue_half(R, R.u0 + w0, t_, 0, second);
   }
   __syncthreads();
   for (int w = w0; w < w1; w++) {
@@ -153,13 +277,7 @@
     const int u = R.u0 + w;
     const bool more = w + 1 < w1;
     f2 own[16];
-    if (R.carry && u >= 0 && (int64_t)(u + 1) * kCoarseBlock > R.carry_from) {
-#pragma unroll
-      for (int q = 0; q < 8; q++) {
-        const int64_t sidx = (int64_t)u * kCoarseBlock + 4 * (t + 256 * q);
-        if (sidx >= R.carry_from && sidx < R.nvalid) stg4(R.carry + (sidx - R.carry_from), second[q]);
-      }
-    }
+    coarse_carry_half(R, u, t, 0, second);
 #pragma unroll
     for (int m = 0; m < 8; m++) {
       own[m] = f2{first[m].x * scale, first[m].y * scale};
@@ -207,69 +325,50 @@
     const f2 tb0 = f2{tb0g.x, tb0g.y};
     if (more) {
       if (zero2) {
-        if (!(exp & 8)) coarse_issue_half(R, u, t, first);
+        if (!(exp & 8)) coarse_issue_half(R, u, t, 0, first);
       } else {
 #pragma unroll
         for (int q = 0; q < 8; q++) first[q] = second[q];
-        if (!(exp & 8)) coarse_issue_half(R, u + 1, t, second);
+        if (!(exp & 8)) coarse_issue_half(R, u + 1, t, 0, second);
       }
     }
     float2* __restrict F = X + (size_t)(R.frame0 + w) * kCoarseBins;
-    auto quad = [&](int k, f2 Ak, f2 Am, f2 Bk, f2 Bm, f2 b) {
-      const f2 a = cmulc(b, b);
-      const f2 aB = cmulc(a, Bk), caBm = cmulc(cj(a), Bm);
-      const f2 Wk = Ak + aB, Wp = Ak - aB;
-      const f2 Wm = Am - caBm, Wn = Am + caBm;
-      const f2 fe = Wk + cj(Wn), bfo = cmulc(b, mul_mi(Wk - cj(Wn)));
-      const f2 Xk = fe + bfo, Xn = cj(fe - bfo);
-      const f2 fe2 = Wm + cj(Wp), wfo2 = cmulc(mul_mi(cj(b)), mul_mi(Wm - cj(Wp)));
-      const f2 Xm = fe2 + wfo2, Xp = cj(fe2 - wfo2);
-      if (exp & 1) {
-        if (Xk.x == 12345.f && Xn.x == 54321.f && Xm.x == 999.f && Xp.y == 777.f) F[0] = make_float2(0.f, 0.f);
-      } else if (k == 0) {
-        stg4(F, v4f{Xk.x, Xn.x, Xm.x, Xm.y});
-      } else if (k == CM / 2) {
-        stg4(F + 2 * k, v4f{Xk.x, Xk.y, Xn.x, Xn.y});
-      } else {
-        stg4(F + 2 * k, v4f{Xk.x, Xk.y, Xp.x, Xp.y});
-        stg4(F + 2 * (CM - k), v4f{Xm.x, Xm.y, Xn.x, Xn.y});
-      }
-    };
     if (!(exp & 2)) {
-      constexpr float w64[8][2] = {{1.f, 0.f},
-                                   {0.99518472667219688624f, -0.09801714032956060199f},
-                                   {0.98078528040323044913f, -0.19509032201612826785f},
-                                   {0.95694033573220886494f, -0.29028467725446236764f},
-                                   {0.92387953251128675613f, -0.38268343236508977173f},
-                                   {0.88192126434835502971f, -0.47139673682599764856f},
-                                   {0.83146961230254523708f, -0.55557023301960222474f},
-                                   {0.77301045336273696081f, -0.63439328416364549822f}};
 #pragma unroll
       for (int m = 0; m < 8; m++) {
-        const f2 b = m == 0 ? tb0 : cmulc(tb0, f2{w64[m][0], w64[m][1]});
-        quad(t + 256 * m, za[m], m >= 8 - kFwdPark ? park[t + 256 * (m - (8 - kFwdPark))] : pa[m], own[m], pb[m], b);
+        const f2 b = m == 0 ? tb0 : cmulc(tb0, f2{kW64[m][0], kW64[m][1]});
+        coarse_fwd_quad(F, t + 256 * m, za[m], m >= 8 - kFwdPark ? park[t + 256 * (m - (8 - kFwdPark))] : pa[m], own[m], pb[m], b, exp);
         __builtin_amdgcn_sched_barrier(0);
       }
-      if (t == 0) quad(CM / 2, za8, za8, zb8, zb8, f2{twab[2049 + CM / 2].x, twab[2049 + CM / 2].y});
+      if (t == 0) coarse_fwd_quad(F, CM / 2, za8, za8, zb8, zb8, f2{twab[2049 + CM / 2].x, twab[2049 + CM / 2].y}, exp);
     }
     __syncthreads();
   }
 }
 
 const char* launch_coarse_fwd(hipStream_t s, const CoarseXRow* rows_dev, int nrows, int max_frames, int run, float2* X, const float2* tw16,
-                              const float2* twab, const CoarseHandOver* handover_dev, int n_handover) {
+                              const float2* twab, const CoarseHandOver* handover_dev, int n_handover, bool wide, LaunchEvents* ev) {
   if (nrows <= 0 || max_frames <= 0) return "";
+  EventScope scope(ev);
   using PL = R16Plan<CM>;
+  static const int exp = (expenv("GA_COARSE_EXP") ? atoi(expenv("GA_COARSE_EXP")) : 0) & 15;
+  run = std::max(run, 1);
+  if (wide && !exp) {
+    if (run != 1 || n_handover > 0 || nrows > kLaunchRows) launch_fail("coarse forward transform: the 512-thread instance takes one window per workgroup and no hand-over rows");
+    const size_t lds = (size_t)(PL::T2 + kFwdTw3 + 2 * CPAD) * sizeof(float2);
+    static LdsLimit lim;
+    lim.raise((const void*)coarse_fwd_kernel<false, true>, lds, "cannot raise the dynamic LDS limit of the coarse forward transform");
+    coarse_launch(true, true, coarse_fwd_kernel<false, true>, dim3(max_frames, nrows), dim3(512), lds, s, rows_dev, 1, X, tw16, twab, 0, handover_dev, 0);
+    return "coarse_fwd_kernel";
+  }
   const size_t lds = (size_t)(PL::T2 + kFwdTw3 + CPAD + kFwdPark * 256) * sizeof(float2);
-  static const int exp = (expenv("GA_COARSE_EXP") ? atoi(expenv("GA_COARSE_EXP")) : 0) & 15;
-  auto kern = exp ? coarse_fwd_kernel<true> : coarse_fwd_kernel<false>;
+  auto kern = exp ? coarse_fwd_kernel<true, false> : coarse_fwd_kernel<false, false>;
   static LdsLimit lim[2];
   lim[exp ? 1 : 0].raise((const void*)kern, lds, "cannot raise the dynamic LDS limit of the coarse forward transform");
-  run = std::max(run, 1);
-  for (int r0 = 0; r0 < nrows; r0 += 32768) {
+  for (int r0 = 0; r0 < nrows; r0 += kLaunchRows) {
     const int nh = r0 == 0 ? n_handover : 0;
-    dim3 grid((max_frames + run - 1) / run, std::min(32768, nrows - r0) + nh);
-    hipLaunchKernelGGL(kern, grid, dim3(256), lds, s, rows_dev + r0, run, X, tw16, twab, exp, handover_dev, nh);
+    dim3 grid((max_frames + run - 1) / run, std::min(kLaunchRows, nrows - r0) + nh);
+    coarse_launch(r0 == 0, last_piece(r0, nrows), kern, grid, dim3(256), lds, s, rows_dev + r0, run, X, tw16, twab, exp, handover_dev, nh);
   }
   return "coarse_fwd_kernel";
 }
@@ -586,9 +685,9 @@
     (void)hipOccupancyMaxActiveBlocksPerMultiprocessor(&occ, coarse_sum_kernel<CW>, kSumThreads, lds);
     fprintf(stderr, "[coarse_sum<%d>] lds %zu B, NFA %d, occupancy %d workgroups/CU, %d jobs\n", CW, lds, NFA, occ, njobs);
   }
-  for (int j0 = 0; j0 < njobs; j0 += 32768)
-    hipLaunchKernelGGL((coarse_sum_kernel<CW>), dim3(kCoarseBins / 64, std::min(32768, njobs - j0)), dim3(kSumThreads), lds, s, jobs_dev + j0, terms_dev, X,
-                       Y, y_frames, NFA, exp >> 4);
+  for (int j0 = 0; j0 < njobs; j0 += kLaunchRows)
+    coarse_launch(j0 == 0, last_piece(j0, njobs), coarse_sum_kernel<CW>, dim3(kCoarseBins / 64, std::min(kLaunchRows, njobs - j0)), dim3(kSumThreads), lds, s,
+                  jobs_dev + j0, terms_dev, X, Y, y_frames, NFA, exp >> 4);
   return CW == 1 ? "coarse_sum_kernel<1>" : (CW == 2 ? "coarse_sum_kernel<2>" : "coarse_sum_kernel<4>");
 }
 
@@ -869,9 +968,9 @@
   if (lds > 160 * 1024) launch_fail("coarse multiply-accumulate: staging does not fit the LDS");
   static LdsLimit lim;
   lim.raise((const void*)coarse_sum_seg_kernel<CW>, lds, "cannot raise the dynamic LDS limit of the coarse multiply-accumulate");
-  for (int j0 = 0; j0 < njobs; j0 += 32768)
-    hipLaunchKernelGGL((coarse_sum_seg_kernel<CW>), dim3(kCoarseBins / 64, std::min(32768, njobs - j0)), dim3(kSumThreads), lds, s, jobs_dev + j0, terms_dev,
-                       X, Y, y_frames, NFA);
+  for (int j0 = 0; j0 < njobs; j0 += kLaunchRows)
+    coarse_launch(j0 == 0, last_piece(j0, njobs), coarse_sum_seg_kernel<CW>, dim3(kCoarseBins / 64, std::min(kLaunchRows, njobs - j0)), dim3(kSumThreads), lds, s,
+                  jobs_dev + j0, terms_dev, X, Y, y_frames, NFA);
   return CW == 1 ? "coarse_sum_seg_kernel<1>" : (CW == 2 ? "coarse_sum_seg_kernel<2>" : "coarse_sum_seg_kernel<4>");
 }
 template <int CW, int TW>
@@ -883,9 +982,9 @@
   if (lds > 160 * 1024) launch_fail("coarse multiply-accumulate: staging does not fit the LDS");
   static LdsLimit lim;
   lim.raise((const void*)coarse_mac_seg_kernel<CW, TW, PB, kMacWaves>, lds, "cannot raise the dynamic LDS limit of the coarse multiply-accumulate");
-  for (int j0 = 0; j0 < njobs; j0 += 32768)
-    hipLaunchKernelGGL((coarse_mac_seg_kernel<CW, TW, PB, kMacWaves>), dim3(kCoarseBins / 64, std::min(32768, njobs - j0)), dim3(64 * kMacWaves), lds, s,
-                       jobs_dev + j0, terms_dev, X, Y, y_frames, NFA);
+  for (int j0 = 0; j0 < njobs; j0 += kLaunchRows)
+    coarse_launch(j0 == 0, last_piece(j0, njobs), coarse_mac_seg_kernel<CW, TW, PB, kMacWaves>, dim3(kCoarseBins / 64, std::min(kLaunchRows, njobs - j0)),
+                  dim3(64 * kMacWaves), lds, s, jobs_dev + j0, terms_dev, X, Y, y_frames, NFA);
   static const std::string name = "coarse_mac_seg_kernel<" + std::to_string(CW) + "," + std::to_string(TW) + "," + std::to_string(PB) + ">";
   return name.c_str();
 }
@@ -1040,9 +1139,9 @@
     (void)hipOccupancyMaxActiveBlocksPerMultiprocessor(&occ, coarse_mac_kernel<CW, TW, PB, WV>, 64 * WV, lds);
     fprintf(stderr, "[coarse_mac<%d,%d,%d>] lds %zu B, NFA %d, occupancy %d workgroups/CU, %d jobs\n", CW, TW, PB, lds, NFA, occ, njobs);
   }
-  for (int j0 = 0; j0 < njobs; j0 += 32768)
-    hipLaunchKernelGGL((coarse_mac_kernel<CW, TW, PB, WV>), dim3(kCoarseBins / 64, std::min(32768, njobs - j0)), dim3(64 * WV), lds, s,
-                       jobs_dev + j0, terms_dev, X, Y, y_frames, NFA, exp >> 4);
+  for (int j0 = 0; j0 < njobs; j0 += kLaunchRows)
+    coarse_launch(j0 == 0, last_piece(j0, njobs), coarse_mac_kernel<CW, TW, PB, WV>, dim3(kCoarseBins / 64, std::min(kLaunchRows, njobs - j0)), dim3(64 * WV), lds, s,
+                  jobs_dev + j0, terms_dev, X, Y, y_frames, NFA, exp >> 4);
   static const std::string name = "coarse_mac_kernel<" + std::to_string(CW) + "," + std::to_string(TW) + "," + std::to_string(PB) + "," + std::to_string(WV) + ">";
   return name.c_str();
 }
@@ -1066,8 +1165,9 @@
   }
 }
 const char* launch_coarse_mac(hipStream_t s, const CoarseJob* jobs_dev, int njobs, const CoarseTerm* terms_dev, const float2* X, float2* Y,
-                       int y_frames, int cw, int max_t, int maxP, bool any_private, int pb, bool matrix_cores) {
+                       int y_frames, int cw, int max_t, int maxP, bool any_private, int pb, bool matrix_cores, LaunchEvents* ev) {
   if (njobs <= 0) return "";
+  EventScope scope(ev);
   if (max_t > (any_private ? kCoarseJobBlocks(cw) : kCoarseSumJobBlocks(cw))) launch_fail("coarse multiply-accumulate: too many coarse blocks in a job");
   if (const char* e = expenv("GA_COARSE_PB")) pb = std::min(pb, std::max(1, atoi(e)));
   if (pb != 1 && pb != 2 && pb != 4 && pb != 8 && pb != 16) launch_fail("coarse multiply-accumulate: unsupported partition block");
@@ -1086,14 +1186,14 @@
     if (matrix_cores && maxP <= 4 && max_t <= kCoarseJobBlocks(16)) {
       static LdsLimit lim;
       lim.raise((const void*)coarse_mfma16_kernel, kMfLdsBytes, "cannot raise the dynamic LDS limit of the matrix-core multiply-accumulate");
-      for (int j0 = 0; j0 < njobs; j0 += 32768)
-        hipLaunchKernelGGL(coarse_mfma16_kernel, dim3(kCoarseBins / 64, std::min(32768, njobs - j0)), dim3(kMfThreads), kMfLdsBytes, s, jobs_dev + j0,
-                           terms_dev, X, Y, y_frames);
+      for (int j0 = 0; j0 < njobs; j0 += kLaunchRows)
+        coarse_launch(j0 == 0, false, coarse_mfma16_kernel, dim3(kCoarseBins / 64, std::min(kLaunchRows, njobs - j0)), dim3(kMfThreads), kMfLdsBytes, s,
+                      jobs_dev + j0, terms_dev, X, Y, y_frames);
       name = "coarse_mfma16_kernel";
     } else {
       name = launch_coarse_mac_t<16, kMacTW16, 1, kMacWaves16>(s, jobs_dev, njobs, terms_dev, X, Y, y_frames, max_t, maxP, true);
     }
-    hipLaunchKernelGGL(coarse_mac_bin0_kernel, dim3(njobs, (kCoarseJobBlocks(16) * 16 + 255) / 256), dim3(256), 0, s, jobs_dev, terms_dev, X, Y, y_frames);
+    coarse_launch(false, true, coarse_mac_bin0_kernel, dim3(njobs, (kCoarseJobBlocks(16) * 16 + 255) / 256), dim3(256), 0, s, jobs_dev, terms_dev, X, Y, y_frames);
     return name;
   }
   launch_fail("coarse multiply-accumulate: unsupported column count");
@@ -1117,13 +1217,23 @@
   if (s0 >= send || !O.out) return;
   float* st = reinterpret_cast<float*>(zb0);
   const bool have_y = tb < O.n_y;
+  constexpr int kRouteWords = kCoarseBlock / 4 / 512;
+  v4f tin[kRouteWords];
+#pragma unroll
+  for (int r = 0; r < kRouteWords; r++) {
+    const int64_t si = s0 + 4 * (tid + 512 * r);
+    tin[r] = v4f{0.f, 0.f, 0.f, 0.f};
+    if (O.tail_in && si < send && si < O.tail_len) tin[r] = ldg4(O.tail_in + si);
+  }
   auto route = [&](bool zero) {
     __syncthreads();
-    for (int i = tid; i < kCoarseBlock / 4; i += 512) {
+#pragma unroll
+    for (int r = 0; r < kRouteWords; r++) {
+      const int i = tid + 512 * r;
       const int64_t si = s0 + 4 * i;
       if (si >= send) continue;
       v4f v = zero ? v4f{0.f, 0.f, 0.f, 0.f} : *reinterpret_cast<const v4f*>(st + 4 * i);
-      if (O.tail_in && si < O.tail_len) v += ldg4(O.tail_in + si);
+      if (O.tail_in && si < O.tail_len) v += tin[r];
       float* __restrict dst = si < O.nvalid ? O.out + si : O.tail_out + (si - O.nvalid);
       if ((((uintptr_t)dst) & 15) == 0) stg4(dst, v);
       else { stg1(dst, v.x); stg1(dst + 1, v.y); stg1(dst + 2, v.z); stg1(dst + 3, v.w); }
@@ -1133,6 +1243,13 @@
     route(true);
     return;
   }
+  float2 qa[4], qb[4];
+#pragma unroll
+  for (int q = 0; q < 4; q++) {
+    qa[q] = twab[tid + 512 * q];
+    qb[q] = twab[2049 + tid + 512 * q];
+  }
+  const float2 qah = twab[CM / 2], qbh = twab[2049 + CM / 2];
   for (int i = tid; i < PL::T2 + PL::T3; i += 512) clds[i] = f2{twg[i].x, twg[i].y};
   {
     float4 sum[8];
@@ -1186,10 +1303,9 @@
   };
 #pragma unroll
   for (int q = 0; q < 4; q++) {
-    const int k = tid + 512 * q;
-    quad(k, f2{twab[k].x, twab[k].y}, f2{twab[2049 + k].x, twab[2049 + k].y});
-  }
-  if (tid == 0) quad(CM / 2, f2{twab[CM / 2].x, twab[CM / 2].y}, f2{twab[2049 + CM / 2].x, twab[2049 + CM / 2].y});
+    quad(tid + 512 * q, f2{qa[q].x, qa[q].y}, f2{qb[q].x, qb[q].y});
+  }
+  if (tid == 0) quad(CM / 2, f2{qah.x, qah.y}, f2{qbh.x, qbh.y});
   __syncthreads();
   f2 own[16];
 #pragma unroll
@@ -1210,16 +1326,17 @@
 }
 
 const char* launch_coarse_inv(hipStream_t s, const CoarseOut* outs_dev, int nouts, int n_blocks, const int* ylist_dev, const float2* Y, int y_frames,
-                              const float2* tw16, const float2* twab) {
+                              const float2* tw16, const float2* twab, LaunchEvents* ev) {
   const int n_t = n_blocks;
   if (nouts <= 0 || n_t <= 0) return "";
+  EventScope scope(ev);
   using PL = R16Plan<CM>;
   const size_t lds = (size_t)(PL::T2 + PL::T3 + 2 * CPAD) * sizeof(float2);
   static LdsLimit lim;
   lim.raise((const void*)coarse_inv_kernel, lds, "cannot raise the dynamic LDS limit of the coarse inverse transform");
-  for (int r0 = 0; r0 < nouts; r0 += 32768)
-    hipLaunchKernelGGL(coarse_inv_kernel, dim3(n_t, std::min(32768, nouts - r0)), dim3(512), lds, s, outs_dev + r0, ylist_dev, Y, y_frames,
-                       tw16, twab);
+  for (int r0 = 0; r0 < nouts; r0 += kLaunchRows)
+    coarse_launch(r0 == 0, last_piece(r0, nouts), coarse_inv_kernel, dim3(n_t, std::min(kLaunchRows, nouts - r0)), dim3(512), lds, s, outs_dev + r0, ylist_dev, Y,
+                  y_frames, tw16, twab);
   return "coarse_inv_kernel";
 }
 
@@ -1402,20 +1519,23 @@
     }
   }
 }
-const char* launch_coarse_premix(hipStream_t s, const PremixJob* jobs_dev, int njobs, const PremixTerm* terms_dev, int64_t max_n) {
+const char* launch_coarse_premix(hipStream_t s, const PremixJob* jobs_dev, int njobs, const PremixTerm* terms_dev, int64_t max_n, LaunchEvents* ev) {
   if (njobs <= 0 || max_n <= 0) return "";
+  EventScope scope(ev);
   const int64_t gx = (max_n + kPremixTile - 1) / kPremixTile;
   if (gx > 0x7fffffff || max_n >= ((int64_t)1 << 29)) launch_fail("coarse pre-mix: chunk too long");
-  for (int j0 = 0; j0 < njobs; j0 += 32768)
-    hipLaunchKernelGGL(coarse_premix_kernel, dim3((unsigned)gx, std::min(32768, njobs - j0)), dim3(64 * kPremixWaves), 0, s, jobs_dev + j0, terms_dev);
+  for (int j0 = 0; j0 < njobs; j0 += kLaunchRows)
+    coarse_launch(j0 == 0, last_piece(j0, njobs), coarse_premix_kernel, dim3((unsigned)gx, std::min(kLaunchRows, njobs - j0)), dim3(64 * kPremixWaves), 0, s,
+                  jobs_dev + j0, terms_dev);
   return "coarse_premix_kernel";
 }
 
-void launch_coarse_hist(hipStream_t s, const CoarseHistJob* jobs_dev, int njobs, int64_t max_len) {
+void launch_coarse_hist(hipStream_t s, const CoarseHistJob* jobs_dev, int njobs, int64_t max_len, LaunchEvents* ev) {
   if (njobs <= 0 || max_len <= 0) return;
+  EventScope scope(ev);
   const int gx = (int)std::min<int64_t>((max_len / 4 + 255) / 256, 64);
-  for (int j0 = 0; j0 < njobs; j0 += 32768)
-    hipLaunchKernelGGL(coarse_hist_kernel, dim3(gx, std::min(32768, njobs - j0)), dim3(256), 0, s, jobs_dev + j0);
+  for (int j0 = 0; j0 < njobs; j0 += kLaunchRows)
+    coarse_launch(j0 == 0, last_piece(j0, njobs), coarse_hist_kernel, dim3(gx, std::min(kLaunchRows, njobs - j0)), dim3(256), 0, s, jobs_dev + j0);
 }
 
 __global__ __launch_bounds__(256) void table_upload_kernel(v4f* __restrict dst, const v4f* __restrict src, size_t n16) {
diff --git a/graphaudio_amd/csrc/ga_engine.cpp b/graphaudio_amd/csrc/ga_engine.cpp
--- a/graphaudio_amd/csrc/ga_engine.cpp
+++ b/graphaudio_amd/csrc/ga_engine.cpp
@@ -370,6 +370,25 @@
   NodeS* n = nodes[r.node].get();
   if (r.input >= 0) return &n->inputs[r.input];
   return nullptr;
+}
+
+Context::TimedLaunch::TimedLaunch(Context& c_, int kind_, double bytes_) : c(c_), kind(kind_), bytes(bytes_) {
+  if (!c.profileNow) return;
+  GA_HIP(hipEventCreate(&ev.start));
+  GA_HIP(hipEventCreate(&ev.stop));
+}
+Context::TimedLaunch::~TimedLaunch() {
+  if (!ev.start) return;
+  if (ev.used) {
+    c.extraProf.push_back(ExtraProf{ev.start, ev.stop, kind, bytes});
+  } else {
+    (void)hipEventDestroy(ev.start);
+    (void)hipEventDestroy(ev.stop);
+  }
+}
+int Context::cuCount() {
+  if (cuCountCached <= 0) GA_HIP(hipDeviceGetAttribute(&cuCountCached, hipDeviceAttributeMultiprocessorCount, device));
+  return cuCountCached;
 }
 
 void Context::harvestProfile(bool wait) {
@@ -1031,7 +1050,8 @@
   }
   CoarseXRow* rd = (CoarseXRow*)dalloc(sizeof(CoarseXRow) * rows.size());
   GA_HIP(hipMemcpy(rd, rows.data(), sizeof(CoarseXRow) * rows.size(), hipMemcpyHostToDevice));
-  launch_coarse_fwd(stream, rd, ir.nch, P, P, ir.coarse, twiddles16pw(), coarseTwab());
+  const bool wide = coarseFwdWide && (int64_t)ir.nch * P <= cuCount();
+  launch_coarse_fwd(stream, rd, ir.nch, P, wide ? 1 : P, ir.coarse, twiddles16pw(), coarseTwab(), nullptr, 0, wide);
   GA_HIP(hipGetLastError());
   GA_HIP(hipStreamSynchronize(stream));
   dfree(rd, sizeof(CoarseXRow) * rows.size());
diff --git a/graphaudio_amd/csrc/ga_engine.hpp b/graphaudio_amd/csrc/ga_engine.hpp
--- a/graphaudio_amd/csrc/ga_engine.hpp
+++ b/graphaudio_amd/csrc/ga_engine.hpp
@@ -625,6 +625,18 @@
   }
   struct ExtraProf { hipEvent_t e0, e1; int kind; double bytes; };
   std::vector<ExtraProf> extraProf;
+  struct TimedLaunch {
+    Context& c;
+    int kind;
+    double bytes;
+    LaunchEvents ev;
+    TimedLaunch(Context& c_, int kind_, double bytes_);
+    ~TimedLaunch();
+    LaunchEvents* events() { return ev.start ? &ev : nullptr; }
+  };
+  bool coarseFwdWide = true;
+  int cuCountCached = 0;
+  int cuCount();
   std::vector<std::vector<NodeSeg>> segNodePool;
   std::vector<std::vector<Views>> viewsPool;
   DevArena coarseM;
diff --git a/graphaudio_amd/csrc/ga_kernels.hpp b/graphaudio_amd/csrc/ga_kernels.hpp
--- a/graphaudio_amd/csrc/ga_kernels.hpp
+++ b/graphaudio_amd/csrc/ga_kernels.hpp
@@ -163,14 +163,20 @@
   int flags;
   int pad_;
 };
-const char* launch_coarse_premix(hipStream_t s, const PremixJob* jobs_dev, int njobs, const PremixTerm* terms_dev, int64_t max_n);
+struct LaunchEvents {
+  hipEvent_t start = nullptr, stop = nullptr;
+  bool used = false;
+};
+const char* launch_coarse_premix(hipStream_t s, const PremixJob* jobs_dev, int njobs, const PremixTerm* terms_dev, int64_t max_n,
+                                 LaunchEvents* ev = nullptr);
 const char* launch_coarse_fwd(hipStream_t s, const CoarseXRow* rows_dev, int nrows, int max_frames, int run, float2* X, const float2* tw16,
-                       const float2* twab, const CoarseHandOver* handover_dev = nullptr, int n_handover = 0);
+                       const float2* twab, const CoarseHandOver* handover_dev = nullptr, int n_handover = 0, bool wide = false,
+                       LaunchEvents* ev = nullptr);
 const char* launch_coarse_mac(hipStream_t s, const CoarseJob* jobs_dev, int njobs, const CoarseTerm* terms_dev, const float2* X, float2* Y,
-                       int y_frames, int cw, int max_t, int maxP, bool any_private, int pb, bool matrix_cores = false);
+                       int y_frames, int cw, int max_t, int maxP, bool any_private, int pb, bool matrix_cores = false, LaunchEvents* ev = nullptr);
 const char* launch_coarse_inv(hipStream_t s, const CoarseOut* outs_dev, int nouts, int n_t, const int* ylist_dev, const float2* Y, int y_frames,
-                       const float2* tw16, const float2* twab);
-void launch_coarse_hist(hipStream_t s, const CoarseHistJob* jobs_dev, int njobs, int64_t max_len);
+                       const float2* tw16, const float2* twab, LaunchEvents* ev = nullptr);
+void launch_coarse_hist(hipStream_t s, const CoarseHistJob* jobs_dev, int njobs, int64_t max_len, LaunchEvents* ev = nullptr);
 void launch_table_upload(hipStream_t s, void* dst, const void* src_pinned, size_t bytes);
 
 struct MixJob {
diff --git a/graphaudio_amd/csrc/ga_plan_conv.cpp b/graphaudio_amd/csrc/ga_plan_conv.cpp
--- a/graphaudio_amd/csrc/ga_plan_conv.cpp
+++ b/graphaudio_amd/csrc/ga_plan_conv.cpp
@@ -171,6 +171,7 @@
   int64_t pmMaxN = 0;
   double pmBytes = 0;
   std::vector<CoarseXRow> xrows;
+  bool premixRowsOnly = true;
   std::vector<CoarseHistJob> hjobs;
   std::vector<Piece> pieces;
   std::map<int, GroupInfo> groups;
@@ -380,6 +381,7 @@
         histBytes += 2.0 * (double)hl * 4.0;
       }
       xrows.push_back(r);
+      premixRowsOnly = false;
     }
     nd.dHistCur ^= 1;
     nd.dHistZero = false;
@@ -655,10 +657,10 @@
   const float2* twFwd = c.twiddles16pw();
   const float2* twab = c.coarseTwab();
   const int nh = (int)hjobs.size(), no = (int)outs.size();
-  struct FwdLaunch { int x0, nx, maxFrames, run; double bytes, flops; };
+  struct FwdLaunch { int x0, nx, maxFrames, run; double bytes, flops; bool wide; };
   std::vector<FwdLaunch> fwds;
   for (int g = 0; g < G; g++) {
-    FwdLaunch f{this->gBegin[g], this->gBegin[g + 1] - this->gBegin[g], 0, 1, 0.0, 0.0};
+    FwdLaunch f{this->gBegin[g], this->gBegin[g + 1] - this->gBegin[g], 0, 1, 0.0, 0.0, false};
     for (int x = f.x0; x < f.x0 + f.nx; x++) {
       f.maxFrames = std::max(f.maxFrames, xrows[x].n_frames);
       f.bytes += (double)(xrows[x].n_frames + 1) * kCoarseBlock * 4.0 + (double)xrows[x].n_frames * kCoarseBins * 8.0;
@@ -671,59 +673,70 @@
       f.run = (f.maxFrames + k - 1) / k;
     }
     if (const char* e = expenv("GA_COARSE_RUN")) f.run = std::max(1, atoi(e));
+    f.wide = c.coarseFwdWide && f.run == 1 && nfh == 0 && this->premixRowsOnly && (int64_t)f.nx * f.maxFrames <= c.cuCount();
     fwds.push_back(f);
   }
   if (G > 1) c.ensureOverlapStream();
   Context* cp = &c;
   ex.plan.add(GA_STAGE_COARSE_SECTION, [=](uint8_t* base) {
-    auto timed = [&](hipStream_t sx, int kind, double bytes, double flops, const std::function<const char*()>& launch) {
-      hipEvent_t e0 = nullptr, e1 = nullptr;
-      if (cp->profileNow) {
-        GA_HIP(hipEventCreate(&e0));
-        GA_HIP(hipEventCreate(&e1));
-        GA_HIP(hipEventRecord(e0, sx));
-      }
-      cp->noteKernel(kind, launch());
-      if (cp->profileNow) {
-        GA_HIP(hipEventRecord(e1, sx));
-        cp->extraProf.push_back(Context::ExtraProf{e0, e1, kind, bytes});
-      }
+    auto timed = [&](int kind, double bytes, double flops, const std::function<const char*(LaunchEvents*)>& launch) {
+      Context::TimedLaunch tl(*cp, kind, bytes);
+      cp->noteKernel(kind, launch(tl.events()));
       cp->stats.kernel_launches++;
       cp->stats.stage_launches[kind]++;
       cp->stats.stage_bytes[kind] += bytes;
       cp->stats.stage_flops[kind] += flops;
     };
     hipStream_t s2 = G > 1 ? cp->stream2 : st;
+    hipEvent_t sec0 = nullptr, sec1 = nullptr;
+    if (cp->profileNow && G > 1) {
+      GA_HIP(hipEventCreate(&sec0));
+      GA_HIP(hipEventCreate(&sec1));
+      GA_HIP(hipEventRecord(sec0, st));
+    }
     if (npm > 0)
-      timed(st, LK_CPREMIX, pmBytes, pmFlops, [&] { return launch_coarse_premix(st, (const PremixJob*)(base + pjo), npm, (const PremixTerm*)(base + pto), pmMaxN); });
+      timed(LK_CPREMIX, pmBytes, pmFlops, [&](LaunchEvents* ev) {
+        return launch_coarse_premix(st, (const PremixJob*)(base + pjo), npm, (const PremixTerm*)(base + pto), pmMaxN, ev);
+      });
     for (int g = 0; g < G; g++) {
       const FwdLaunch& f = fwds[g];
-      if (f.nx > 0)
-        timed(st, LK_CFWD, f.bytes, f.flops, [&] {
+      if (f.nx > 0) {
+        timed(LK_CFWD, f.bytes, f.flops, [&](LaunchEvents* ev) {
           return launch_coarse_fwd(st, (const CoarseXRow*)(base + xo) + f.x0, f.nx, f.maxFrames, f.run, X, twFwd, twab,
-                                   (const CoarseHandOver*)(base + fho), g == 0 ? nfh : 0);
+                                   (const CoarseHandOver*)(base + fho), g == 0 ? nfh : 0, f.wide, ev);
         });
+        if (f.wide) cp->stats.coarse_fwd_wide_launches++;
+      }
       if (G > 1) {
         GA_HIP(hipEventRecord(cp->dGroupEv[g], st));
         GA_HIP(hipStreamWaitEvent(s2, cp->dGroupEv[g], 0));
       }
       for (const MacLaunch& m : macs)
         if (m.grp == g)
-          timed(s2, LK_CMAC, m.bytes, m.flops, [&] {
+          timed(LK_CMAC, m.bytes, m.flops, [&](LaunchEvents* ev) {
             return launch_coarse_mac(s2, (const CoarseJob*)(base + m.off), m.nj, (const CoarseTerm*)(base + to), X, Y, yFrames, m.cw, m.mt, m.mp, m.ap, m.pb,
-                                     matrixCores);
+                                     matrixCores, ev);
           });
     }
     if (G > 1) {
       GA_HIP(hipEventRecord(cp->dJoinEv, s2));
       GA_HIP(hipStreamWaitEvent(st, cp->dJoinEv, 0));
     }
+    if (sec0) {
+      GA_HIP(hipEventRecord(sec1, st));
+      cp->extraProf.push_back(Context::ExtraProf{sec0, sec1, GA_STAGE_COARSE_SECTION, 0.0});
+    }
   });
-  ex.plan.add(LK_CINV, [=](uint8_t* base) {
-    cp->noteKernel(LK_CINV, launch_coarse_inv(st, (const CoarseOut*)(base + oo), no, invBlocks, (const int*)(base + yo), Y, yFrames, tw16, twab));
+  ex.plan.addSelfTimed(LK_CINV, [=](uint8_t* base) {
+    Context::TimedLaunch tl(*cp, LK_CINV, invBytes);
+    cp->noteKernel(LK_CINV, launch_coarse_inv(st, (const CoarseOut*)(base + oo), no, invBlocks, (const int*)(base + yo), Y, yFrames, tw16, twab, tl.events()));
   }, invBytes, invFlops);
   const int64_t mh = maxHist;
-  if (nh > 0) ex.plan.add(LK_CHIST, [=](uint8_t* base) { launch_coarse_hist(st, (const CoarseHistJob*)(base + ho), nh, mh); }, histBytes);
+  if (nh > 0)
+    ex.plan.addSelfTimed(LK_CHIST, [=](uint8_t* base) {
+      Context::TimedLaunch tl(*cp, LK_CHIST, histBytes);
+      launch_coarse_hist(st, (const CoarseHistJob*)(base + ho), nh, mh, tl.events());
+    }, histBytes);
 }
 }
 
diff --git a/include/graphaudio_hip.h b/include/graphaudio_hip.h
--- a/include/graphaudio_hip.h
+++ b/include/graphaudio_hip.h
@@ -82,6 +82,7 @@
   int64_t ref_order_rows;
   int64_t sim_replays;
   int64_t twin_rows;
+  int64_t coarse_fwd_wide_launches;
 } ga_stats;
 enum {
   GA_STAGE_OTHER = 0,
```

Result: faster. 1.247 billion (median of 5 runs) (+1.8%).
